# Youncy-Hu/MAGE

Hardware: AMD Instinct MI355X
Metric: generated frames/sec (64x64, 16-frame clips) (higher is better)
Workload: dtype bf16

## Files before the change

include/mage_hip_ext.h:

```cpp
#ifndef MAGE_HIP_EXT_H
#define MAGE_HIP_EXT_H

#include "mage_hip.h"

#ifdef __cplusplus
extern "C" {
#endif

int mage_token_stats(const float* logits, int64_t rows, int32_t K, int64_t ld, int64_t group, int64_t in_group_stride, int64_t in_off,
                     const int64_t* tokens, int64_t tok_group_stride, int64_t tok_off, float temperature, int32_t top_k, float top_p,
                     float* policy_logprob, float* policy_entropy, int32_t* kept, float* entropy, void* stream);

int mage_policy_loss(const float* logits, int64_t rows, int32_t K, int64_t ld, const int64_t* tokens, const float* advantage, int64_t adv_div,
                     const float* behaviour_logprob, float temperature, int32_t top_k, float top_p, float clip_lo, float clip_hi,
                     float entropy_coef, float* row_loss, float* logprob, float* entropy, uint32_t* cut, float* summary, void* stream);
int mage_policy_loss_bwd(const float* logits, int64_t rows, int32_t K, int64_t ld, const int64_t* tokens, const float* advantage,
                         int64_t adv_div, const float* behaviour_logprob, const uint32_t* cut, float temperature, float clip_lo,
                         float clip_hi, float entropy_coef, const float* grad_out, void* dlogits, int32_t dl_dtype, void* stream);

int mage_policy_loss_anchored(const float* logits, int64_t rows, int32_t K, int64_t ld, const int64_t* tokens, const float* advantage,
                              int64_t adv_div, const float* behaviour_logprob, const float* reference_logprob, float temperature,
                              int32_t top_k, float top_p, float clip_lo, float clip_hi, float entropy_coef, float kl_coef, float* row_loss,
                              float* logprob, float* entropy, uint32_t* cut, float* kl, float* summary, void* stream);
int mage_policy_loss_anchored_bwd(const float* logits, int64_t rows, int32_t K, int64_t ld, const int64_t* tokens, const float* advantage,
                                  int64_t adv_div, const float* behaviour_logprob, const float* reference_logprob, const uint32_t* cut,
                                  float temperature, float clip_lo, float clip_hi, float entropy_coef, float kl_coef, const float* grad_out,
                                  void* dlogits, int32_t dl_dtype, void* stream);

int mage_sumsq(const float* g, int64_t n, double* out, void* stream);
int mage_adam_clipped(float* p, const float* g, float* m, float* v, int64_t n, float lr, float beta1, float beta2, float eps, int32_t step,
                      float grad_scale, const double* sumsq, float max_norm, float* norm_out, void* stream);

int mage_video_metrics(const float* video, int64_t video_clip_stride, const float* target, int64_t target_clip_stride, int64_t clips, int32_t T,
                       int32_t C, int32_t H, int32_t W, int64_t tgt_div, float data_range, float* mse, float* psnr, float* ssim, void* stream);

int mage_group_advantages(const float* frame_reward, int64_t groups, int32_t N, int32_t T, int32_t mode, float eps, float* reward,
                          float* advantage, void* stream);

int mage_video_noise(const int64_t* seeds, int64_t B, int32_t C, int64_t hw, float* nchw, float* rows, void* stream);

int mage_guide_logits(const float* cond, const float* uncond, float* out, int64_t rows, int32_t K, int64_t ld, int64_t group,
                      int64_t in_group_stride, int64_t in_off, const float* scale, int64_t scale_div, void* stream);

int mage_preference_loss(const float* clip_logprob, const float* reference_logprob, int64_t clips, const int64_t* pairs, int64_t n_pairs,
                         float beta, float label_smoothing, int32_t mode, float* pair_loss, float* pair_margin, float* clip_coef,
                         float* summary, void* stream);

int mage_token_logprob_bwd(const float* logits, int64_t rows, int32_t K, int64_t ld, const int64_t* tokens, const float* weight,
                           int64_t weight_div, const float* grad_out, void* dlogits, int32_t dl_dtype, void* stream);

#ifdef __cplusplus
}
#endif
#endif
```

mage_amd/_lib.py:

```python
from __future__ import annotations

import ctypes as C
import os
from typing import Optional

_HERE = os.path.dirname(os.path.abspath(__file__))
LIB_PATH = os.environ.get("MAGE_HIP_LIB", os.path.join(_HERE, "lib", "libmage_hip.so"))

F32, BF16, BF16X3, F16X3, F16 = 0, 1, 2, 3, 4
ACT_NONE, ACT_RELU, ACT_QUICKGELU, ACT_GELU_ERF, ACT_TANH, ACT_QUICKGELU_GRAD = 0, 1, 2, 3, 4, 5
ABI_VERSION = 10

i32, i64, f32, vp = C.c_int32, C.c_int64, C.c_float, C.c_void_p


class GemmDesc(C.Structure):
    _fields_ = [
        ("dtype", i32), ("M", i32), ("N", i32), ("K", i32),
        ("A", vp), ("W", vp), ("Y", vp),
        ("lda", i32), ("ldy", i32), ("y_dtype", i32),
        ("out_h", i32), ("out_w", i32), ("in_h", i32), ("in_w", i32),
        ("a_img_stride", i32), ("a_off", i32),
        ("taps_h", i32), ("taps_w", i32), ("cin", i32), ("stride", i32),
        ("dy0", i32), ("dx0", i32), ("dys", i32), ("dxs", i32),
        ("y_img_stride", i32), ("y_mul_y", i32), ("y_mul_x", i32), ("y_off", i32),
        ("bias", vp), ("scale", vp), ("shift", vp),
        ("act", i32),
        ("rowadd", vp), ("rowadd_div", i32), ("rowadd_mod", i32),
        ("residual", vp), ("ldr", i32), ("res_dtype", i32),
        ("post_relu", i32), ("ldw", i32), ("n_split", i32),
        ("a_split_stride", i64), ("w_split_stride", i64), ("y_split_stride", i64),
        ("y2", vp), ("ldy2", i32), ("res_half", i32), ("ln_part", vp), ("ln_stats", vp), ("ln_colsum", vp), ("a_half", i32), ("ln_eps", C.c_float),
        ("head_w", vp), ("head_phases", i32), ("a_relu", i32), ("ln_part_rows", i64),
    ]


class AttnDesc(C.Structure):
    _fields_ = [
        ("dtype", i32), ("q", vp), ("k", vp), ("v", vp), ("out", vp),
        ("ldq", i32), ("ldk", i32), ("ldv", i32), ("ldo", i32),
        ("n_seq", i32), ("inner", i32), ("nq", i32), ("nk", i32), ("n_head", i32),
        ("q_outer_stride", i32), ("q_axis_stride", i32), ("kv_outer_stride", i32), ("kv_axis_stride", i32),
        ("causal", i32), ("kv_len", vp), ("kv_len_div", i32), ("scale", f32), ("out_split", i32), ("drop_p", f32), ("drop_seed", C.c_uint64),
        ("o_outer_stride", i32), ("o_axis_stride", i32),
    ]


SIGNATURES = {
    "mage_abi_version": (C.c_int, []),
    "mage_last_error": (C.c_char_p, []),
    "mage_init": (C.c_int, [C.c_int]),
    "mage_check_device_errors": (C.c_int, [vp]),
    "mage_set_option": (C.c_int, [C.c_char_p, i32]),
    "mage_get_option": (C.c_int, [C.c_char_p, C.POINTER(i32)]),
    "mage_gemm": (C.c_int, [C.POINTER(GemmDesc), vp]),
    "mage_gemm_kernel_name": (C.c_int, [C.POINTER(GemmDesc), C.c_char_p, i32]),
    "mage_gemm_is_small": (C.c_int, [i32, i32, i32]),
    "mage_ln_stats": (C.c_int, [vp, i64, i32, i32, f32, vp, vp]),
    "mage_row_stats": (C.c_int, [vp, i32, i64, i32, i64, f32, vp, vp]),
    "mage_groupnorm_bwd": (C.c_int, [vp, i64, i64, i32, i32, i32, i32, vp, vp, vp, vp, i32, vp, i64, i64, vp, vp, vp, vp, vp, vp]),
    "mage_adain_bwd": (C.c_int, [vp, vp, vp, vp, vp, i32, i32, i32, f32, vp]),
    "mage_reparam_kl_bwd": (C.c_int, [vp, vp, vp, vp, vp, vp, vp, i64, vp]),
    "mage_mse_bwd": (C.c_int, [vp, i64, vp, i64, i64, i32, vp, vp, i64, vp]),
    "mage_transpose_colsum": (C.c_int, [vp, i64, vp, i64, i64, i64, i32, i32, i64, i64, vp, i32, vp]),
    "mage_maxpool2_bwd": (C.c_int, [vp, vp, vp, i32, i32, i32, i32, vp]),
    "mage_upsample2_bwd": (C.c_int, [vp, vp, i32, i32, i32, i32, vp]),
    "mage_layernorm": (C.c_int, [vp, vp, vp, vp, i32, i64, i32, f32, vp]),
    "mage_split": (C.c_int, [vp, i64, vp, i64, i64, i32, i32, vp]),
    "mage_attention": (C.c_int, [C.POINTER(AttnDesc), vp]),
    "mage_embedding": (C.c_int, [vp, vp, vp, i32, i64, i32, i32, i32, i64, i64, i64, i64, i64, vp]),
    "mage_table_conv": (C.c_int, [vp, i64, i32, i32, i32, i32, vp, i32, i32, i32, vp, vp, i32, vp, i64, i32, vp, i32, i64, i64, i64, i64, vp]),
    "mage_resblock_table": (C.c_int, [vp, i64, i32, i32, vp, i32, i32, vp, vp, vp, vp, vp, vp, i32, vp, i64, i64, i64, i64, vp]),
    "mage_resblock_rows": (C.c_int, [vp, i64, vp, vp, vp, vp, vp, i64, i32, vp, i64, i64, i32, i32, i32, i64, i64, i64, vp]),
    "mage_vq_nearest": (C.c_int, [vp, vp, vp, i64, i32, i32, vp, vp, vp]),
    "mage_vq_prepare": (C.c_int, [vp, i32, i32, vp, vp, vp]),
    "mage_argmax": (C.c_int, [vp, i64, i32, i64, i64, i64, i64, vp, i64, i64, vp, vp]),
    "mage_sample_tokens": (C.c_int, [vp, i64, i32, i64, i64, i64, i64, vp, i64, i64, vp, i64, f32, i32, f32, vp]),
    "mage_token_logprob": (C.c_int, [vp, i64, i32, i64, i64, i64, i64, vp, vp, i64, i64, vp]),
    "mage_clip_scores": (C.c_int, [vp, i64, i32, i64, vp, vp, vp]),
    "mage_cross_entropy": (C.c_int, [vp, vp, i64, i32, vp, vp, vp]),
    "mage_conv_in": (C.c_int, [vp, vp, vp, vp, vp, vp, i32, i32, i32, i32, i32, i32, i32, i32, i32, i32, i32, i32, vp]),
    "mage_split_rows": (C.c_int, [vp, i64, vp, i64, i32, i32, i32, i64, i64, i64, i64, i64, vp, vp]),
    "mage_conv_out": (C.c_int, [vp, i32, vp, vp, vp, i32, i32, i32, i32, i32, i32, vp]),
    "mage_convt_fold_tanh": (C.c_int, [vp, vp, vp, i32, i32, i32, i32, vp]),
    "mage_maxpool2": (C.c_int, [vp, vp, i32, i32, i32, i32, i32, i32, vp]),
    "mage_upsample2": (C.c_int, [vp, vp, i32, i32, i32, i32, i32, vp]),
    "mage_relu": (C.c_int, [vp, vp, i32, i64, vp]),
    "mage_cast": (C.c_int, [vp, i32, vp, i32, i64, vp]),
    "mage_adain": (C.c_int, [vp, vp, vp, vp, i32, i32, i32, f32, vp]),
    "mage_add_scaled_rowvec": (C.c_int, [vp, vp, vp, i32, i32, i32, vp]),
    "mage_row_affine": (C.c_int, [vp, vp, vp, i64, i32, i32, i32, vp]),
    "mage_caption_mask": (C.c_int, [vp, i32, i32, i64, vp, vp, vp]),
    "mage_copy2d": (C.c_int, [vp, i64, vp, i64, i64, i64, vp]),
    "mage_groupnorm_silu": (C.c_int, [vp, i64, i64, i32, i32, i32, i32, vp, vp, f32, vp, vp, i32, vp]),
    "mage_groupnorm_act": (C.c_int, [vp, i64, i64, i32, i32, i32, i32, vp, vp, f32, vp, vp, i32, vp, i32, i64, i64, vp]),
    "mage_reparam_kl": (C.c_int, [vp, vp, vp, vp, vp, i32, i64, vp]),
    "mage_mse": (C.c_int, [vp, i64, vp, i64, i64, i32, vp, vp, vp]),
    "mage_transpose": (C.c_int, [vp, i32, i64, vp, i64, i64, i64, i64, i32, i32, i32, i32, i32, i64, i64, i32, i32, i32, vp]),
    "mage_bn_colreduce": (C.c_int, [i32, vp, vp, vp, vp, vp, i64, i32, vp, i32, vp]),
    "mage_bn_apply": (C.c_int, [vp, vp, vp, vp, vp, vp, vp, i32, i64, i32, i32, vp]),
    "mage_bn_bwd_apply": (C.c_int, [vp, vp, vp, vp, vp, vp, vp, vp, i64, i32, vp]),
    "mage_convt_unfold_tanh_bwd": (C.c_int, [vp, vp, vp, i32, i32, i32, i32, vp]),
    "mage_gemm_tn": (C.c_int, [vp, i64, vp, i64, i64, i32, i32, i32, i64, vp, vp, vp]),
    "mage_colsum": (C.c_int, [vp, i64, i64, i32, vp, i32, vp]),
    "mage_row_sum": (C.c_int, [vp, i32, i64, i64, i32, vp, i32, vp]),
    "mage_sum_partials": (C.c_int, [vp, i64, i32, i64, vp, i32, vp]),
    "mage_layernorm_bwd": (C.c_int, [vp, vp, vp, i32, vp, vp, i32, i64, i32, f32, i32, vp, f32, C.c_uint64, vp]),
    "mage_act": (C.c_int, [vp, vp, i32, i64, i32, vp]),
    "mage_act_bwd": (C.c_int, [vp, vp, vp, i32, i64, i32, vp]),
    "mage_cross_entropy_bwd": (C.c_int, [vp, vp, i64, i32, vp, vp, i32, vp]),
    "mage_embedding_bwd": (C.c_int, [vp, vp, i32, vp, i64, i32, i32, i64, i64, i64, i64, vp, i64, vp]),
    "mage_group_rowsum": (C.c_int, [vp, i32, i64, i32, i64, i64, vp, i64, vp, i32, vp]),
    "mage_attention_bwd": (C.c_int, [C.POINTER(AttnDesc), vp, vp, vp, vp, i32, i32, i32, vp]),
    "mage_dropout": (C.c_int, [vp, i32, vp, i32, i64, f32, C.c_uint64, i32, vp]),
    "mage_dropout_add": (C.c_int, [vp, i32, vp, vp, vp, i64, f32, C.c_uint64, vp]),
    "mage_dropout_add_layernorm": (C.c_int, [vp, i32, vp, vp, vp, vp, vp, i32, i64, i32, f32, f32, C.c_uint64, vp]),
    "mage_adam": (C.c_int, [vp, vp, vp, vp, i64, f32, f32, f32, f32, i32, f32, vp]),
}

EXT_SIGNATURES = {
    "mage_token_stats": (C.c_int, [vp, i64, i32, i64, i64, i64, i64, vp, i64, i64, f32, i32, f32, vp, vp, vp, vp, vp]),
    "mage_policy_loss": (C.c_int, [vp, i64, i32, i64, vp, vp, i64, vp, f32, i32, f32, f32, f32, f32, vp, vp, vp, vp, vp, vp]),
    "mage_policy_loss_bwd": (C.c_int, [vp, i64, i32, i64, vp, vp, i64, vp, vp, f32, f32, f32, f32, vp, vp, i32, vp]),
    "mage_policy_loss_anchored": (C.c_int, [vp, i64, i32, i64, vp, vp, i64, vp, vp, f32, i32, f32, f32, f32, f32, f32, vp, vp, vp, vp, vp, vp, vp]),
    "mage_policy_loss_anchored_bwd": (C.c_int, [vp, i64, i32, i64, vp, vp, i64, vp, vp, vp, f32, f32, f32, f32, f32, vp, vp, i32, vp]),
    "mage_sumsq": (C.c_int, [vp, i64, vp, vp]),
    "mage_adam_clipped": (C.c_int, [vp, vp, vp, vp, i64, f32, f32, f32, f32, i32, f32, vp, f32, vp, vp]),
    "mage_video_metrics": (C.c_int, [vp, i64, vp, i64, i64, i32, i32, i32, i32, i64, f32, vp, vp, vp, vp]),
    "mage_group_advantages": (C.c_int, [vp, i64, i32, i32, i32, f32, vp, vp, vp]),
    "mage_video_noise": (C.c_int, [vp, i64, i32, i64, vp, vp, vp]),
    "mage_guide_logits": (C.c_int, [vp, vp, vp, i64, i32, i64, i64, i64, i64, vp, i64, vp]),
    "mage_preference_loss": (C.c_int, [vp, vp, i64, vp, i64, f32, f32, i32, vp, vp, vp, vp, vp]),
    "mage_token_logprob_bwd": (C.c_int, [vp, i64, i32, i64, vp, vp, i64, vp, vp, i32, vp]),
}

_lib: Optional[C.CDLL] = None
_inited_devices = set()


class MageHipError(RuntimeError):
    pass


def load(path: str = LIB_PATH) -> C.CDLL:
    global _lib
    if _lib is not None:
        return _lib
    if not os.path.exists(path):
        raise MageHipError(
            f"{path} not found: the HIP extension is not built. Run `python -c 'import __graft_entry__ as g; g.build()'` "
            f"(or `make -C mage_amd/csrc`). There is no CPU/PyTorch fallback for the MAGE product path.")
    import torch
    lib = C.CDLL(path)
    for name, (res, args) in {**SIGNATURES, **EXT_SIGNATURES}.items():
        fn = getattr(lib, name)
        fn.restype, fn.argtypes = res, args
    if lib.mage_abi_version() != ABI_VERSION:
        raise MageHipError(f"libmage_hip.so ABI {lib.mage_abi_version()} != binding ABI {ABI_VERSION}: rebuild")
    _lib = lib
    return lib


def lib(device_index: int = 0) -> C.CDLL:
    l = load()
    if device_index not in _inited_devices:
        check(l.mage_init(int(device_index)), l)
        _inited_devices.add(device_index)
    return l


def check(code: int, l: Optional[C.CDLL] = None) -> None:
    if code == 0:
        return
    l = l or load()
    msg = (l.mage_last_error() or b"").decode(errors="replace")
    if code == -1:
        raise ValueError(f"mage_hip: {msg}")
    raise MageHipError(f"mage_hip error {code}: {msg}")
```

mage_amd/config.py:

```python
from __future__ import annotations

import contextlib
import dataclasses
import os
from typing import Iterator

__all__ = ["Config", "ENV", "get", "override", "lib_option", "lib_options", "lib_flag", "LIB_OPTIONS"]


@dataclasses.dataclass(frozen=True)
class Config:
    ln_fold: bool = True
    stream_16bit: bool = True
    attn_split: bool = True
    frame_table: bool = True
    auto_graph: bool = True
    encode_split: bool = True
    decode_table: bool = True
    decode_split: bool = True
    decode_taps8: bool = True
    decode_resblock_fusion: bool = True
    decode_head_fusion: bool = True
    decode_phase_merge: bool = True
    decode_relu_fold: bool = True
    train_f32_branch: bool = False
    train_wgrad_transpose: bool = False
    train_emit: bool = True
    train_dual: bool = True
    train_taps: bool = True
    train_enc_split: bool = True


ENV = {
    "ln_fold": ("MAGE_NO_LN_FOLD", False),
    "stream_16bit": ("MAGE_STREAM_FP32", False),
    "attn_split": ("MAGE_ATTN_SPLIT_FP32", False),
    "frame_table": ("MAGE_NO_FRAME_TABLE", False),
    "auto_graph": ("MAGE_NO_AUTO_GRAPH", False),
    "encode_split": ("MAGE_ENCODE_FP32", False),
    "decode_table": ("MAGE_NO_DECODE_TABLE", False),
    "decode_split": ("MAGE_DECODE_FP32", False),
    "decode_taps8": ("MAGE_DECODE_NO_TAPS8", False),
    "decode_resblock_fusion": ("MAGE_DECODE_NO_RESBLOCK_FUSION", False),
    "decode_head_fusion": ("MAGE_DECODE_NO_HEAD_FUSION", False),
    "decode_phase_merge": ("MAGE_DECODE_NO_PHASE_MERGE", False),
    "decode_relu_fold": ("MAGE_DECODE_NO_RELU_FOLD", False),
    "train_f32_branch": ("MAGE_TRAIN_F32_BRANCH", True),
    "train_wgrad_transpose": ("MAGE_WGRAD_TRANSPOSE", True),
    "train_emit": ("MAGE_TRAIN_NO_EMIT", False),
    "train_dual": ("MAGE_TRAIN_NO_DUAL", False),
    "train_taps": ("MAGE_TRAIN_NO_TAPS", False),
    "train_enc_split": ("MAGE_TRAIN_ENC_FP32", False),
}

LIB_OPTIONS = ("gemm_no_4w", "gemm_no_4h", "gemm_4h_plain", "gemm4_train_forms", "gemm_no_8phase", "gemm_no_taps8", "gemm_no_narrow", "gemm_no_narrow_few", "gemm_no_small",
               "gemm_small_m", "gemm_stagger_groups", "gemm_stagger_percent", "gemm_stagger_forced",
               "gemm4_stagger_groups", "gemm4_stagger_percent", "attn_no_mfma", "attn_no_fewq", "vq_no_mfma", "conv_no_tile")


def _set(v) -> bool:
    return bool(v) and v != "0"


def _from_env() -> Config:
    kw = {}
    for field, (var, when_set) in ENV.items():
        if _set(os.environ.get(var)):
            kw[field] = when_set
    return Config(**kw)


_CONFIG = _from_env()


def get() -> Config:
    return _CONFIG


@contextlib.contextmanager
def override(**kw) -> Iterator[Config]:
    global _CONFIG
    saved = _CONFIG
    _CONFIG = dataclasses.replace(saved, **kw)
    try:
        yield _CONFIG
    finally:
        _CONFIG = saved


_LIB_CACHE = None


def invalidate_lib_options() -> None:
    global _LIB_CACHE
    _LIB_CACHE = None


def _lib_cache() -> dict:
    global _LIB_CACHE
    if _LIB_CACHE is None:
        import ctypes as C
        from . import _lib
        l = _lib.load()
        out = {}
        for name in LIB_OPTIONS:
            v = C.c_int32(0)
            _lib.check(l.mage_get_option(name.encode(), C.byref(v)), l)
            out[name] = int(v.value)
        _LIB_CACHE = out
    return _LIB_CACHE


def lib_options() -> dict:
    return dict(_lib_cache())


def lib_flag(name: str) -> int:
    c = _lib_cache()
    if name not in c:
        raise KeyError(f"unknown library option '{name}' (mage_amd.config.LIB_OPTIONS)")
    return c[name]


def set_lib_option(name: str, value: int) -> None:
    from . import _lib
    l = _lib.load()
    try:
        _lib.check(l.mage_set_option(name.encode(), int(value)), l)
    finally:
        invalidate_lib_options()


@contextlib.contextmanager
def lib_option(name: str, value: int) -> Iterator[None]:
    old = lib_flag(name)
    set_lib_option(name, value)
    try:
        yield
    finally:
        set_lib_option(name, old)
```

mage_amd/csrc/common.h:

```cpp
#pragma once
#include <hip/hip_runtime.h>
#include <stdint.h>
#include <stdio.h>
#include <stdarg.h>
#include "../../include/mage_hip.h"

typedef __bf16 bf16_t;
typedef __attribute__((ext_vector_type(8))) __bf16 bf16x8;
typedef __attribute__((ext_vector_type(4))) __bf16 bf16x4;
typedef __attribute__((ext_vector_type(4))) float f32x4;
typedef __attribute__((ext_vector_type(4))) unsigned int u32x4;

#define MAGE_MAX_DEVICES 16
void mage_set_error(const char* fmt, ...);
int mage_device_index();
const void* mage_zero_page();
int* mage_error_word();
enum { MAGE_DEVERR_EMBEDDING_ID = 1, MAGE_DEVERR_CE_TARGET = 2, MAGE_DEVERR_TOKEN_ID = 3, MAGE_DEVERR_PAIR_ID = 4 };
struct MageOptions {
    int gemm_no_4w;
    int gemm_no_4h;
    int gemm_4h_plain;
    int gemm4_train_forms;
    int gemm_no_8phase;
    int gemm_no_taps8;
    int gemm_no_narrow;
    int gemm_no_narrow_few;
    int gemm_no_small;
    int gemm_small_m;
    int gemm_stagger_groups, gemm_stagger_percent, gemm_stagger_forced;
    int gemm4_stagger_groups, gemm4_stagger_percent;
    int attn_no_mfma;
    int attn_no_fewq;
    int vq_no_mfma;
    int conv_no_tile;
};
const MageOptions& mage_options();
__device__ __forceinline__ void mage_raise(int* word, int code, long value, int bound) {
    if (atomicCAS(word, 0, code) == 0) {
        word[1] = (int)value;
        word[2] = bound;
    }
}

#if defined(MAGE_DEBUG) && MAGE_DEBUG
#include <cassert>
#define MAGE_DASSERT(cond) assert(cond)
#else
#define MAGE_DASSERT(cond) ((void)0)
#endif

#define MAGE_CHECK_ARG(cond, ...)                                   \
    do {                                                            \
        if (!(cond)) {                                              \
            mage_set_error(__VA_ARGS__);                            \
            return MAGE_EINVAL;                                     \
        }                                                           \
    } while (0)

#define MAGE_CHECK_LAUNCH(name)                                                         \
    do {                                                                                \
        hipError_t e_ = hipGetLastError();                                              \
        if (e_ != hipSuccess) {                                                         \
            mage_set_error("%s: launch failed: %s", name, hipGetErrorString(e_));       \
            return MAGE_EHIP;                                                           \
        }                                                                               \
    } while (0)

int mage_gemm_cu_count();
extern thread_local const void** mage_gemm_plan;
template <auto KERNEL, typename Args>
int mage_gemm_launch(unsigned grid, unsigned block, unsigned lds, hipStream_t s, const Args& a) {
    if (mage_gemm_plan) {
        *mage_gemm_plan = (const void*)KERNEL;
        return MAGE_OK;
    }
    static bool attr[MAGE_MAX_DEVICES] = {false};
    const int dev = mage_device_index();
    MAGE_CHECK_ARG(dev >= 0, "mage_gemm: no current device");
    if (!attr[dev]) {
        (void)hipFuncSetAttribute((const void*)KERNEL, hipFuncAttributeMaxDynamicSharedMemorySize, lds);
        attr[dev] = true;
    }
    hipLaunchKernelGGL(KERNEL, dim3(grid), dim3(block), lds, s, a);
    MAGE_CHECK_LAUNCH("mage_gemm");
    return MAGE_OK;
}

__device__ __forceinline__ unsigned short f2bf_bits(float f) {
    unsigned int u = __float_as_uint(f);
    if ((u & 0x7fffffffu) > 0x7f800000u) return (unsigned short)((u >> 16) | 0x40);
    u += 0x7fffu + ((u >> 16) & 1u);
    return (unsigned short)(u >> 16);
}
__device__ __forceinline__ float bf_bits2f(unsigned short b) { return __uint_as_float(((unsigned int)b) << 16); }

template <typename T> __device__ __forceinline__ float to_f32(T v);
template <> __device__ __forceinline__ float to_f32<float>(float v) { return v; }
template <> __device__ __forceinline__ float to_f32<unsigned short>(unsigned short v) { return bf_bits2f(v); }

template <typename T> __device__ __forceinline__ T from_f32(float v);
template <> __device__ __forceinline__ float from_f32<float>(float v) { return v; }
template <> __device__ __forceinline__ unsigned short from_f32<unsigned short>(float v) { return f2bf_bits(v); }

typedef _Float16 f16_t;
template <> __device__ __forceinline__ float to_f32<f16_t>(f16_t v) { return (float)v; }
template <> __device__ __forceinline__ f16_t from_f32<f16_t>(float v) { return (f16_t)v; }

__device__ __forceinline__ f32x4 load4(const float* p) { return *(const f32x4*)p; }
__device__ __forceinline__ f32x4 load4(const unsigned short* p) {
    uint2 r = *(const uint2*)p;
    f32x4 o;
    o[0] = __uint_as_float(r.x << 16);
    o[1] = __uint_as_float(r.x & 0xffff0000u);
    o[2] = __uint_as_float(r.y << 16);
    o[3] = __uint_as_float(r.y & 0xffff0000u);
    return o;
}
__device__ __forceinline__ void store4(float* p, f32x4 v) { *(f32x4*)p = v; }
__device__ __forceinline__ void mage_ln_stats_row(const float2* __restrict__ p, long stride, int n_slices, float inv_c, float eps, float& mean, float& rstd) {
    float s1 = 0.f, s2 = 0.f;
    for (int i = 0; i < n_slices; ++i) {
        const float2 v = p[(long)i * stride];
        s1 = __fadd_rn(s1, v.x);
        s2 = __fadd_rn(s2, v.y);
    }
    mean = __fmul_rn(s1, inv_c);
    const float var = fmaxf(__fmaf_rn(-mean, mean, __fmul_rn(s2, inv_c)), 0.f);
    rstd = __fdiv_rn(1.0f, __fsqrt_rn(__fadd_rn(var, eps)));
}

typedef __attribute__((ext_vector_type(2))) __bf16 bf16x2_t;
__device__ __forceinline__ unsigned int pack_bf16x2(float a, float b) {
    bf16x2_t v = {(__bf16)a, (__bf16)b};
    return __builtin_bit_cast(unsigned int, v);
}
__device__ __forceinline__ void store4(unsigned short* p, f32x4 v) {
    uint2 r;
    r.x = pack_bf16x2(v[0], v[1]);
    r.y = pack_bf16x2(v[2], v[3]);
    *(uint2*)p = r;
}

__device__ __forceinline__ void store8(unsigned short* p, f32x4 a, f32x4 b) {
    uint4 r;
    r.x = pack_bf16x2(a[0], a[1]);
    r.y = pack_bf16x2(a[2], a[3]);
    r.z = pack_bf16x2(b[0], b[1]);
    r.w = pack_bf16x2(b[2], b[3]);
    *(uint4*)p = r;
}
__device__ __forceinline__ void store8(float* p, f32x4 a, f32x4 b) { *(f32x4*)p = a; *(f32x4*)(p + 4) = b; }

typedef __attribute__((ext_vector_type(2))) _Float16 f16x2_t;
typedef __attribute__((ext_vector_type(8))) _Float16 f16x8;
__device__ __forceinline__ unsigned int pack_f16x2(float a, float b) {
    const f16x2_t v = {(_Float16)a, (_Float16)b};
    return __builtin_bit_cast(unsigned int, v);
}
__device__ __forceinline__ float2 unpack_f16x2(unsigned int u) {
    const f16x2_t v = __builtin_bit_cast(f16x2_t, u);
    return float2{(float)v[0], (float)v[1]};
}
__device__ __forceinline__ float2 unpack_bf16x2(unsigned int u) { return float2{__uint_as_float(u << 16), __uint_as_float(u & 0xffff0000u)}; }
template <typename T> __device__ __forceinline__ unsigned int pack16x2(float a, float b) {
    if constexpr (sizeof(T) == 2 && !__is_same(T, unsigned short)) return pack_f16x2(a, b);
    else return pack_bf16x2(a, b);
}
template <typename T> __device__ __forceinline__ float2 unpack16x2(unsigned int u) {
    if constexpr (sizeof(T) == 2 && !__is_same(T, unsigned short)) return unpack_f16x2(u);
    else return unpack_bf16x2(u);
}
template <typename T> __device__ __forceinline__ f32x4 widen4(uint2 r) {
    const float2 a = unpack16x2<T>(r.x), b = unpack16x2<T>(r.y);
    return f32x4{a.x, a.y, b.x, b.y};
}
template <typename T> __device__ __forceinline__ f32x4 mfma16x16x32(const u32x4& a, const u32x4& b, const f32x4& c) {
    if constexpr (sizeof(T) == 2 && !__is_same(T, unsigned short))
        return __builtin_amdgcn_mfma_f32_16x16x32_f16(__builtin_bit_cast(f16x8, a), __builtin_bit_cast(f16x8, b), c, 0, 0, 0);
    else
        return __builtin_amdgcn_mfma_f32_16x16x32_bf16(__builtin_bit_cast(bf16x8, a), __builtin_bit_cast(bf16x8, b), c, 0, 0, 0);
}
__device__ __forceinline__ f32x4 load4(const f16_t* p) { return widen4<f16_t>(*(const uint2*)p); }
__device__ __forceinline__ void store4(f16_t* p, f32x4 v) { *(uint2*)p = uint2{pack_f16x2(v[0], v[1]), pack_f16x2(v[2], v[3])}; }
__device__ __forceinline__ void store8(f16_t* p, f32x4 a, f32x4 b) {
    *(uint4*)p = uint4{pack_f16x2(a[0], a[1]), pack_f16x2(a[2], a[3]), pack_f16x2(b[0], b[1]), pack_f16x2(b[2], b[3])};
}

typedef short mage_s16x2 __attribute__((ext_vector_type(2)));
__device__ __forceinline__ unsigned relu16x2(unsigned v) {
    const mage_s16x2 z = {0, 0};
    return __builtin_bit_cast(unsigned, __builtin_elementwise_max(__builtin_bit_cast(mage_s16x2, v), z));
}

struct split_bf16 { unsigned int pair; };
struct split_f16 { unsigned int pair; };
#define MAGE_F16_LO_SCALE 2048.0f
template <int KIND>
__device__ __forceinline__ void split_pack2(float a, float b, unsigned int& hi, unsigned int& lo) {
    if constexpr (KIND == 1) {
        hi = pack_bf16x2(a, b);
        lo = pack_bf16x2(a - __uint_as_float(hi << 16), b - __uint_as_float(hi & 0xffff0000u));
    } else {
        a = __builtin_amdgcn_fmed3f(a, -65504.f, 65504.f);
        b = __builtin_amdgcn_fmed3f(b, -65504.f, 65504.f);
        const f16x2_t h = {(_Float16)a, (_Float16)b};
        const f16x2_t l = {(_Float16)((a - (float)h[0]) * MAGE_F16_LO_SCALE), (_Float16)((b - (float)h[1]) * MAGE_F16_LO_SCALE)};
        hi = __builtin_bit_cast(unsigned int, h);
        lo = __builtin_bit_cast(unsigned int, l);
    }
}
template <int KIND>
__device__ __forceinline__ void split_store4(void* p, f32x4 v) {
    const uintptr_t a = (uintptr_t)p;
    char* q = (char*)((a & ~(uintptr_t)255) + ((a & 255) >> 1));
    uint2 h, l;
    split_pack2<KIND>(v[0], v[1], h.x, l.x);
    split_pack2<KIND>(v[2], v[3], h.y, l.y);
    *(uint2*)q = h;
    *(uint2*)(q + 128) = l;
}
__device__ __forceinline__ void store4(split_bf16* p, f32x4 v) { split_store4<1>(p, v); }
__device__ __forceinline__ void store4(split_f16* p, f32x4 v) { split_store4<2>(p, v); }
// ... 35 lines not shown
```

mage_amd/csrc/gemm.hip:

```cpp
#include <cxxabi.h>
#include <cstring>
#include <mutex>
#include <string>
#include <unordered_map>
#include "gemm_impl.h"

int mage_gemm_f16(const mage_gemm_desc* d, hipStream_t s);

#ifdef MAGE_PROBE
extern "C" int mage_debug_read_waves(void* dst, size_t bytes) {
    return hipMemcpyFromSymbol(dst, HIP_SYMBOL(mage_probe_wave), bytes < sizeof(mage_probe_wave) ? bytes : sizeof(mage_probe_wave)) ==
                   hipSuccess
               ? 0
               : -1;
}
extern "C" int mage_debug_read_seg(void* dst, size_t bytes) {
    return hipMemcpyFromSymbol(dst, HIP_SYMBOL(mage_probe_seg), bytes < sizeof(mage_probe_seg) ? bytes : sizeof(mage_probe_seg)) ==
                   hipSuccess
               ? 0
               : -1;
}
extern "C" int mage_debug_read(void* dst, size_t bytes) {
    return hipMemcpyFromSymbol(dst, HIP_SYMBOL(mage_probe_buf), bytes < sizeof(mage_probe_buf) ? bytes : sizeof(mage_probe_buf)) ==
                   hipSuccess
               ? 0
               : -1;
}
#endif


extern "C" int mage_gemm_is_small(int32_t M, int32_t N, int32_t K) {
    MAGE_CHECK_ARG(mage_device_index() >= 0 && M > 0 && N > 0 && K > 0, "mage_gemm_is_small: no current device / bad sizes");
    return small_shape(M, N, K, mage_gemm_cu_count()) ? 1 : 0;
}

extern "C" int mage_gemm(const mage_gemm_desc* d_in, void* stream) {
    MAGE_CHECK_ARG(d_in != nullptr, "mage_gemm: null descriptor");
    mage_gemm_desc dn = *d_in;
    const bool spl = dn.dtype == MAGE_BF16X3 || dn.dtype == MAGE_F16X3;
    if (dn.ldw == 0) dn.ldw = spl ? 2 * dn.K : dn.K;
    if (dn.n_split <= 0) dn.n_split = 1;
    const mage_gemm_desc* d = &dn;
    MAGE_CHECK_ARG(d->ldw >= (spl ? 2 * d->K : d->K), "mage_gemm: ldw=%d < K=%d", d->ldw, d->K);
    MAGE_CHECK_ARG(d->ldw == d->K || d->n_split > 1 || spl,
                   "mage_gemm: ldw=%d != K=%d: a W row stride other than K is read only by the split-K (n_split > 1) and split-precision forms", d->ldw, d->K);
    MAGE_CHECK_ARG(mage_zero_page() != nullptr, "mage_gemm: mage_init() has not been called");
    const bool h16 = d->dtype == MAGE_F16;
    MAGE_CHECK_ARG(d->dtype == MAGE_F32 || d->dtype == MAGE_BF16 || h16 || spl, "mage_gemm: bad dtype %d", d->dtype);
    MAGE_CHECK_ARG(d->y_dtype == MAGE_F32 || (d->y_dtype == MAGE_BF16 && !h16) || ((spl || h16) && d->y_dtype == d->dtype),
                   "mage_gemm: bad y_dtype %d for dtype %d (fp32, or the operands' 16-bit / split type; fp32 operands may write bf16)", d->y_dtype, d->dtype);
    MAGE_CHECK_ARG(!d->residual || d->res_dtype == MAGE_F32 || (d->res_dtype == MAGE_BF16 && !h16) || (h16 && d->res_dtype == MAGE_F16),
                   "mage_gemm: bad res_dtype %d for dtype %d", d->res_dtype, d->dtype);
    MAGE_CHECK_ARG(!spl || (d->K % 64 == 0 && d->cin % 64 == 0 && d->lda >= 2 * d->cin && d->y_dtype != MAGE_BF16),
                   "mage_gemm: split-precision operands need K and cin multiples of 64, lda >= 2 cin (16-bit elements), fp32 or split output");
    MAGE_CHECK_ARG(!spl || d->y_dtype == MAGE_F32 || (d->N % 64 == 0 && d->ldy % 8 == 0 && d->ldy >= 2 * d->N && (((uintptr_t)d->Y) & 255) == 0),
                   "mage_gemm: split output needs N %% 64 == 0, ldy >= 2N (16-bit elements), Y 256-byte aligned");
    MAGE_CHECK_ARG(d->M > 0 && d->N > 0 && d->K > 0, "mage_gemm: empty problem M=%d N=%d K=%d", d->M, d->N, d->K);
    MAGE_CHECK_ARG(d->A && d->W && d->Y, "mage_gemm: null operand");
    const int ch = d->dtype == MAGE_F32 ? 4 : 8;
    MAGE_CHECK_ARG(d->N % 8 == 0, "mage_gemm: N=%d must be a multiple of 8", d->N);
    MAGE_CHECK_ARG(d->K % ch == 0 && d->lda % ch == 0 && d->cin % ch == 0,
                   "mage_gemm: K=%d, lda=%d, cin=%d must be multiples of %d", d->K, d->lda, d->cin, ch);
    MAGE_CHECK_ARG(d->ldy % 4 == 0 && (!d->residual || d->ldr % 4 == 0), "mage_gemm: ldy/ldr must be multiples of 4");
    MAGE_CHECK_ARG((d->y_dtype != MAGE_BF16 && d->y_dtype != MAGE_F16) || d->ldy % 8 == 0, "mage_gemm: 16-bit output needs ldy a multiple of 8 (16-byte accesses)");
    MAGE_CHECK_ARG(!d->residual || d->res_dtype == MAGE_F32 || d->ldr % 8 == 0, "mage_gemm: a 16-bit residual needs ldr a multiple of 8 (16-byte accesses)");
    MAGE_CHECK_ARG(d->taps_h >= 1 && d->taps_w >= 1 && d->K == d->taps_h * d->taps_w * d->cin,
                   "mage_gemm: K=%d != taps_h*taps_w*cin = %d*%d*%d", d->K, d->taps_h, d->taps_w, d->cin);
    MAGE_CHECK_ARG(d->out_h >= 1 && d->out_w >= 1 && d->in_h >= 1 && d->in_w >= 1, "mage_gemm: bad geometry");
    MAGE_CHECK_ARG(!d->scale == !d->shift, "mage_gemm: scale and shift must be given together");
    MAGE_CHECK_ARG(!d->rowadd || (d->rowadd_div >= 1 && d->rowadd_mod >= 1), "mage_gemm: bad rowadd div/mod");
    MAGE_CHECK_ARG((((uintptr_t)d->A | (uintptr_t)d->W | (uintptr_t)d->Y) & 15) == 0, "mage_gemm: operands must be 16-byte aligned");
    const bool gather_ = d->taps_h * d->taps_w > 1 || d->stride != 1 || d->dy0 != 0 || d->dx0 != 0 || d->in_h != d->out_h || d->in_w != d->out_w;
    MAGE_CHECK_ARG(d->n_split == 1 || (!gather_ && !d->residual && !d->rowadd && !d->scale && !d->post_relu && !d->bias &&
                                       d->out_h == 1 && d->out_w >= d->M && d->act == MAGE_ACT_NONE),
                   "mage_gemm: n_split > 1 is the plain split-K form (no gather, no epilogue extras, rows not regrouped)");
    MAGE_CHECK_ARG(d->n_split == 1 || ((d->a_split_stride | d->w_split_stride) % ch == 0 && d->y_split_stride % 4 == 0 && d->ldw % ch == 0),
                   "mage_gemm: split strides / ldw must keep 16-byte alignment");
    hipStream_t s = (hipStream_t)stream;
    MAGE_CHECK_ARG(!d->a_half || (d->in_h % 2 == 0 && d->in_w % 2 == 0 && d->n_split == 1), "mage_gemm: a_half needs an even in_h x in_w grid");
    MAGE_CHECK_ARG(!d->res_half || (d->residual && d->out_h > 1 && d->out_h % 2 == 0 && d->out_w % 2 == 0 && d->n_split == 1),
                   "mage_gemm: res_half needs a residual and an even out_h x out_w output plane");
    MAGE_CHECK_ARG(!d->ln_part || d->ln_part_rows > (d->ln_colsum ? (int64_t)d->M - 1 : (int64_t)(d->M - 1) * d->y_mul_x + d->y_off),
                   "mage_gemm: ln_part needs ln_part_rows (rows of the slice-major partial-sum buffer) > the largest row it is indexed with");
    MAGE_CHECK_ARG(!d->a_relu || (d->dtype == MAGE_BF16 && !gather_ && !d->a_half && d->N <= 128 && d->n_split == 1 && !d->residual && !d->rowadd && !d->scale &&
                                  !d->post_relu && !d->y2 && !d->ln_part && !d->ln_stats && !d->ln_colsum && !d->head_w),
                   "mage_gemm: a_relu is a form of the bf16 plain GEMM with N <= 128 (epilogue act(acc + bias) only)");
    if (spl) {
        const bool tapsform = gather_ || d->rowadd;
        MAGE_CHECK_ARG(!d->head_w, "mage_gemm: head_w is a fusion of the bf16 padded-taps form");
        if (tapsform) {
            const int r = d->dtype == MAGE_BF16X3 ? try_taps8<1>(d, s) : try_taps8<2>(d, s);
            if (r) return r < 0 ? r : MAGE_OK;
            mage_set_error("mage_gemm: split-precision form: this convolution / row-table geometry is not eligible for the padded-taps kernel");
            return MAGE_EUNSUPPORTED;
        }
        return d->dtype == MAGE_BF16X3 ? launch_spl<1>(d, s) : launch_spl<2>(d, s);
    }
    if (h16) {
        MAGE_CHECK_ARG(!d->head_w && d->n_split == 1 && !d->scale && !d->post_relu && !d->res_half && !d->a_half,
                       "mage_gemm: MAGE_F16 operands do not take head_w / n_split / scale+shift / post_relu / res_half / a_half");
        return mage_gemm_f16(d, s);
    }
    if (const int r = try_taps8(d, s)) return r < 0 ? r : MAGE_OK;
    MAGE_CHECK_ARG(!d->head_w, "mage_gemm: head_w is a fusion of the bf16 padded-taps form; this geometry does not run there");
    if (const int r = mage_conv3x3_c64_try(d, s)) return r < 0 ? r : MAGE_OK;
    if (const int r = mage_gemm4_try(d, s)) return r < 0 ? r : MAGE_OK;
    const bool gather = d->taps_h * d->taps_w > 1 || d->stride != 1 || d->dy0 != 0 || d->dx0 != 0 || d->in_h != d->out_h ||
                        d->in_w != d->out_w || d->a_half;
    if (d->dtype == MAGE_BF16) return gather ? launch<MAGE_BF16, true>(d, s) : launch<MAGE_BF16, false>(d, s);
    return gather ? launch<MAGE_F32, true>(d, s) : launch<MAGE_F32, false>(d, s);
}

thread_local const void** mage_gemm_plan = nullptr;

extern "C" int mage_gemm_kernel_name(const mage_gemm_desc* desc, char* buf, int32_t len) {
    MAGE_CHECK_ARG(buf != nullptr && len > 0, "mage_gemm_kernel_name: no buffer");
    const void* kernel = nullptr;
    mage_gemm_plan = &kernel;
    const int r = mage_gemm(desc, nullptr);
    mage_gemm_plan = nullptr;
    if (r != MAGE_OK) return r;
    static std::mutex mu;
    static std::unordered_map<const void*, std::string> names;
    std::string name;
    {
        std::lock_guard<std::mutex> lock(mu);
        auto it = names.find(kernel);
        if (it == names.end()) {
            hipFunction_t f = nullptr;
            const char* raw = hipGetFuncBySymbol(&f, kernel) == hipSuccess ? hipKernelNameRef(f) : nullptr;
            if (!raw) {
                mage_set_error("mage_gemm_kernel_name: the runtime has no name for the selected kernel");
                return MAGE_EHIP;
            }
            std::string n = raw;
            int status = -1;
            if (char* dm = n.compare(0, 2, "_Z") == 0 ? abi::__cxa_demangle(raw, nullptr, nullptr, &status) : nullptr) {
                if (status == 0) n = dm;
                free(dm);
            }
            for (const char* drop : {"void ", "(anonymous namespace)::"})
                for (size_t at; (at = n.find(drop)) != std::string::npos;) n.erase(at, strlen(drop));
            n = n.substr(0, n.find('('));
            it = names.emplace(kernel, n).first;
        }
        name = it->second;
    }
    MAGE_CHECK_ARG((int32_t)name.size() < len, "mage_gemm_kernel_name: %d bytes are too few for '%s'", (int)len, name.c_str());
    memcpy(buf, name.c_str(), name.size() + 1);
    return MAGE_OK;
}
```

mage_amd/csrc/gemm4.hip:

```cpp
#include <cstdio>
#include <cstdlib>
#include <utility>

#include "gemm_shared.h"
#include "gemm4_regs.h"

namespace {

struct Gemm4Args {
    const void* A;
    const void* W;
    void* Y;
    const float* bias;
    const float* ln_stats;
    const float* ln_colsum;
    const void* residual;
    float* ln_part;
    void* y2;
    int M, N, K, lda, ldw, ldy, ldr, ldy2, y_dtype, a_off, y_off;
    int ntiles_n, ntiles;
    int stagger_groups, stagger_sleeps;
};

#ifndef MAGE4_ABL
#define MAGE4_ABL 0
#endif

#ifdef MAGE4_STAMP
__device__ unsigned long long g4_stamps[256 * 32 * 4 * 8];
#define G4_STAMP(it, p)                                                                                                   \
    do {                                                                                                                  \
        if (lane == 0 && (it) < 32 && blockIdx.x < 256) {                                                                 \
            g4_stamps[((blockIdx.x * 32 + (it)) * 4 + wave) * 8 + (p)] = __builtin_readcyclecounter();                    \
            if ((p) == 1) g4_stamps[((blockIdx.x * 32 + (it)) * 4 + wave) * 8 + 3] = __builtin_amdgcn_s_memrealtime();    \
            if ((p) == 0) g4_stamps[((blockIdx.x * 32 + (it)) * 4 + wave) * 8 + 4] = __builtin_amdgcn_s_memrealtime();    \
        }                                                                                                                 \
    } while (0)
#else
#define G4_STAMP(it, p)
#endif

constexpr int G4_STAGE = 65536, G4_WOFF = 32768, G4_RING = 2 * G4_STAGE, G4_LDS = G4_RING + 4 * 4096;

#ifdef MAGE4_MFMA32
template <int B, bool ZERO, bool CLOB>
__device__ __forceinline__ void g4_mfma32(const u32x4& w, const u32x4& x) {
    if constexpr (ZERO && CLOB) asm volatile("v_mfma_f32_32x32x16_bf16 a[%c2:%c3], %0, %1, 0" ::"v"(w), "v"(x), "i"(16 * B), "i"(16 * B + 15) : G4_ALL_ACC);
    else if constexpr (ZERO) asm volatile("v_mfma_f32_32x32x16_bf16 a[%c2:%c3], %0, %1, 0" ::"v"(w), "v"(x), "i"(16 * B), "i"(16 * B + 15));
    else if constexpr (CLOB) asm volatile("v_mfma_f32_32x32x16_bf16 a[%c2:%c3], %0, %1, a[%c2:%c3]" ::"v"(w), "v"(x), "i"(16 * B), "i"(16 * B + 15) : G4_ALL_ACC);
    else asm volatile("v_mfma_f32_32x32x16_bf16 a[%c2:%c3], %0, %1, a[%c2:%c3]" ::"v"(w), "v"(x), "i"(16 * B), "i"(16 * B + 15));
}
#endif
template <int ACT, int EK, int LN, bool RB, bool HF = false>
__global__ __launch_bounds__(256) void gemm4_kernel(const Gemm4Args g) {
    static_assert(EK != EK_GENERAL, "lean epilogue kinds");
    static_assert(!HF || (LN != LN_DUAL && LN != LN_GELUBWD), "f16 form: the generation path's epilogues");
    typedef std::conditional_t<HF, f16_t, unsigned short> H16;
    extern __shared__ __attribute__((aligned(16))) char smem[];
    g4_claim_accumulators();
    const int tid = threadIdx.x;
    const int lane = tid & 63;
    const int wave = __builtin_amdgcn_readfirstlane(tid >> 6);
    const int nwg8 = gridDim.x >> 3;
    const int xcd = blockIdx.x & 7, li = blockIdx.x >> 3;
    const int q8 = g.ntiles >> 3, r8 = g.ntiles & 7;
    const int chunk0 = xcd < r8 ? xcd * (q8 + 1) : r8 * (q8 + 1) + (xcd - r8) * q8;
    const int chunk1 = chunk0 + q8 + (xcd < r8 ? 1 : 0);
    const int nk = g.K >> 6;
    int c_tile = chunk0 + li;
    if (c_tile >= chunk1) return;
    const int last_tile = c_tile + ((chunk1 - 1 - c_tile) / nwg8) * nwg8;

    const int lr = lane >> 3, lp = lane & 7;
    unsigned voffA[8], voffW[8];
#pragma unroll
    for (int u = 0; u < 8; ++u) {
        const int r = u * 8 + lr;
        const int ch = lp ^ ((r >> 1) & 7);
        voffA[u] = (unsigned)(r * g.lda * 2 + ch * 16 + 8192 - u * 1024);
        voffW[u] = (unsigned)(r * g.ldw * 2 + ch * 16 + 8192 - u * 1024);
    }
    auto a_base = [&](int tile) { return (const char*)g.A + ((long)((tile / g.ntiles_n) * 256 + wave * 64) + g.a_off) * g.lda * 2 - 4096; };
    auto w_base = [&](int tile) { return (const char*)g.W + (long)((tile % g.ntiles_n) * 256 + wave * 64) * g.ldw * 2 - 4096; };
    const char* a_src = a_base(c_tile);
    const char* w_src = w_base(c_tile);
    const char* a_next = a_src;
    const char* w_next = w_src;
    const unsigned lds0 = (unsigned)(uintptr_t)(__attribute__((address_space(3))) char*)smem + wave * 8192 + 4096;
    auto dma_m0 = [&](unsigned lds_group) __attribute__((always_inline)) {
        asm volatile("s_mov_b32 m0, %0\n\ts_nop 0" ::"s"(lds0 + lds_group) : "memory");
    };

    const int wm = wave >> 1, wn = wave & 1;
    const int l15 = lane & 15, grp = lane >> 4;
    const int rsw = (l15 >> 1) & 7;
    const int pc[2] = {((grp + 0) ^ rsw) * 16, ((grp + 4) ^ rsw) * 16};
    const int x_off = (wm * 128 + l15) * 128;
    const int w_off = G4_WOFF + (wn * 128 + l15) * 128;
    u32x4 wf[2][8], xf[2][4];
    auto rd_w1 = [&](int buf, int stage, int t, int nt) __attribute__((always_inline)) {
        wf[buf][nt] = *(const u32x4*)(smem + stage * G4_STAGE + w_off + nt * 2048 + pc[t]);
    };
    auto rd_x1 = [&](int buf, int stage, int t, int mt) __attribute__((always_inline)) {
        xf[buf][mt & 3] = *(const u32x4*)(smem + stage * G4_STAGE + x_off + mt * 2048 + pc[t]);
    };

#ifdef MAGE4_MFMA32
    const int l31 = lane & 31, hi5 = lane >> 5;
    const int rsw32 = (l31 >> 1) & 7;
    const int x32_off = (wm * 128 + l31) * 128, w32_off = G4_WOFF + (wn * 128 + l31) * 128;
    u32x4 wq[2][4], xq[2][4];
    auto rd_w32 = [&](int buf, int stage, int ks, int nb) __attribute__((always_inline)) {
        wq[buf][nb] = *(const u32x4*)(smem + stage * G4_STAGE + w32_off + nb * 4096 + (((2 * ks + hi5) ^ rsw32) << 4));
    };
    auto rd_x32 = [&](int buf, int stage, int ks, int mb) __attribute__((always_inline)) {
        xq[buf][mb] = *(const u32x4*)(smem + stage * G4_STAGE + x32_off + mb * 4096 + (((2 * ks + hi5) ^ rsw32) << 4));
    };
#endif
    if (g.stagger_groups > 1) {
        for (int w = (li % g.stagger_groups) * g.stagger_sleeps; w > 0; --w) __builtin_amdgcn_s_sleep(16);
    }
    dma_m0(0);
    g4_for<8>([&](auto u_) { g4_dma<decltype(u_)::value>(voffA[decltype(u_)::value], a_src); });
    dma_m0(G4_WOFF);
    g4_for<8>([&](auto u_) { g4_dma<decltype(u_)::value>(voffW[decltype(u_)::value], w_src); });
    a_src += 128;
    w_src += 128;
    dma_m0(G4_STAGE);
    g4_for<8>([&](auto u_) { g4_dma<decltype(u_)::value>(voffA[decltype(u_)::value], a_src); });
    dma_m0(G4_STAGE + G4_WOFF);
    g4_for<8>([&](auto u_) { g4_dma<decltype(u_)::value>(voffW[decltype(u_)::value], w_src); });
    a_src += 128;
    w_src += 128;
    __builtin_amdgcn_s_waitcnt(0x0F70);
    ring_barrier();
#ifdef MAGE4_MFMA32
#pragma unroll
    for (int b = 0; b < 4; ++b) { rd_w32(0, 0, 0, b); rd_x32(0, 0, 0, b); }
#else
#pragma unroll
    for (int nt = 0; nt < 8; ++nt) rd_w1(0, 0, 0, nt);
#pragma unroll
    for (int m = 0; m < 4; ++m) rd_x1(0, 0, 0, m);
#endif

    [[maybe_unused]] int it = 0;
    for (; c_tile < chunk1; c_tile += nwg8, ++it) {
        G4_STAMP(it, 0);
        const int tm = c_tile / g.ntiles_n, tn = c_tile - tm * g.ntiles_n;
        MAGE_DASSERT(c_tile >= 0 && c_tile < g.ntiles && tm * 256 < g.M && tn * 256 < g.N);
        const int m0 = ((MAGE4_ABL & 32) ? (int)blockIdx.x : tm) * 256 + wm * 128, n0 = ((MAGE4_ABL & 32) ? 0 : tn) * 256 + wn * 128;
        {
            const int nt_tile = c_tile + nwg8 > last_tile ? last_tile : c_tile + nwg8;
            a_next = a_base(nt_tile);
            w_next = w_base(nt_tile);
        }
        f32x4 biasm[2][4];
        [[maybe_unused]] float ln_mean[8], ln_rstd[8];
        [[maybe_unused]] f32x4 lns[2][4];
        auto slab = [&](auto S_, auto FIRST_, auto LAST_, int j) __attribute__((always_inline)) {
            constexpr int S = decltype(S_)::value;
            constexpr bool FIRST = decltype(FIRST_)::value, LAST = decltype(LAST_)::value;
            g4_for<32>([&](auto i_) {
                constexpr int i = decltype(i_)::value, m = i >> 3, nt = i & 7;
                g4_mfma<((nt >> 2) * 8 + m) * 4 + (nt & 3), FIRST, i == 0, HF>(wf[0][nt], xf[0][m]);
                __builtin_amdgcn_sched_barrier(0);
                if constexpr (!(MAGE4_ABL & 4) && i < 4) {
                    rd_x1(1, S, 0, 4 + i);
                    __builtin_amdgcn_sched_barrier(0);
                }
                if constexpr (!(MAGE4_ABL & 2) && !FIRST && i == 4) {
                    dma_m0((S ^ 1) * G4_STAGE + G4_WOFF);
                    __builtin_amdgcn_sched_barrier(0);
                }
                if constexpr (!(MAGE4_ABL & 2) && !FIRST && (i & 3) == 1 && i > 4) {
                    g4_dma<(i >> 2) - 1>(voffW[(i >> 2) - 1], w_src);
                    __builtin_amdgcn_sched_barrier(0);
                }
            });
            if constexpr (!(MAGE4_ABL & 2) && !FIRST) {
                g4_dma<7>(voffW[7], w_src);
                __builtin_amdgcn_sched_barrier(0);
            }
            if constexpr (!(MAGE4_ABL & 8) && !FIRST) w_src = (j == nk - 2) ? w_next : w_src + 128;
            g4_for<32>([&](auto i_) {
                constexpr int i = decltype(i_)::value, m = i >> 3, nt = i & 7;
                g4_mfma<((nt >> 2) * 8 + 4 + m) * 4 + (nt & 3), FIRST, i == 0, HF>(wf[0][nt], xf[1][m]);
                __builtin_amdgcn_sched_barrier(0);
                if constexpr (!(MAGE4_ABL & 4) && i < 12) {
                    if constexpr (i < 4) rd_x1(0, S, 1, i);
                    else rd_w1(1, S, 1, i - 4);
                    __builtin_amdgcn_sched_barrier(0);
                }
            });
            if constexpr (LAST) {
#pragma unroll
                for (int b = 0; b < 4; ++b) {
                    const int n = n0 + b * 16 + grp * 4;
                    biasm[0][b] = *(const f32x4*)(g.bias + n);
                    if constexpr (LN == LN_CONSUME) lns[0][b] = *(const f32x4*)(g.ln_colsum + n);
                }
                if constexpr (LN == LN_CONSUME) {
#pragma unroll
                    for (int a = 0; a < 8; ++a) {
                        const float2 st = *(const float2*)(g.ln_stats + 2 * (long)(m0 + a * 16 + l15));
                        ln_mean[a] = st.x;
                        ln_rstd[a] = st.y;
                    }
                }
                __builtin_amdgcn_sched_barrier(0);
            }
            g4_for<32>([&](auto i_) {
                constexpr int i = decltype(i_)::value, m = i >> 3, nt = i & 7;
                g4_mfma<((nt >> 2) * 8 + m) * 4 + (nt & 3), false, i == 0, HF>(wf[1][nt], xf[0][m]);
                __builtin_amdgcn_sched_barrier(0);
                if constexpr (!(MAGE4_ABL & 4) && i < 4) {
                    rd_x1(1, S, 1, 4 + i);
                    __builtin_amdgcn_sched_barrier(0);
                }
            });
            if constexpr (MAGE4_ABL & 16) __builtin_amdgcn_s_waitcnt(0xC07F);
            else if constexpr (FIRST) __builtin_amdgcn_s_waitcnt(LN == LN_CONSUME ? 0x8074 : 0x8070);
            else __builtin_amdgcn_s_waitcnt(0x0070);
            ring_barrier();
            __builtin_amdgcn_sched_barrier(0);
            g4_for<32>([&](auto i_) {
                constexpr int i = decltype(i_)::value, m = i >> 3, nt = i & 7;
                g4_mfma<((nt >> 2) * 8 + 4 + m) * 4 + (nt & 3), false, i == 0, HF>(wf[1][nt], xf[1][m]);
                __builtin_amdgcn_sched_barrier(0);
                if constexpr (!(MAGE4_ABL & 4) && i < 12 && !LAST) {
                    if constexpr (i < 4) rd_x1(0, S ^ 1, 0, i);
                    else rd_w1(0, S ^ 1, 0, i - 4);
                    __builtin_amdgcn_sched_barrier(0);
                }
                if constexpr (!(MAGE4_ABL & 2) && !LAST) {
                    if constexpr (i == 2) dma_m0(S * G4_STAGE);
                    if constexpr ((i & 3) == 3) g4_dma<(i >> 2)>(voffA[i >> 2], a_src);
                    if constexpr (i == 2 || (i & 3) == 3) __builtin_amdgcn_sched_barrier(0);
                }
                if constexpr (!(MAGE4_ABL & 2) && LAST) {
                    if constexpr (i == 0) dma_m0(S * G4_STAGE);
                    if constexpr (i == 16) dma_m0(S * G4_STAGE + G4_WOFF);
                    if constexpr ((i & 1) == 1 && i < 16) g4_dma<(i >> 1)>(voffA[i >> 1], a_src);
                    if constexpr ((i & 1) == 1 && i > 16) g4_dma<((i - 16) >> 1)>(voffW[(i - 16) >> 1], w_src);
                    if constexpr (i == 0 || i == 16 || (i & 1) == 1) __builtin_amdgcn_sched_barrier(0);
                }
            });
            if constexpr (!(MAGE4_ABL & 8)) a_src = (j == nk - 3) ? a_next : a_src + 128;
            if constexpr (!(MAGE4_ABL & 8) && LAST) w_src += 128;
        };
#ifdef MAGE4_MFMA32
        auto slab32 = [&](auto S_, auto FIRST_, auto LAST_, int j) __attribute__((always_inline)) {
            constexpr int S = decltype(S_)::value;
            constexpr bool FIRST = decltype(FIRST_)::value, LAST = decltype(LAST_)::value;
            auto quarter = [&](auto Q_) __attribute__((always_inline)) {
                constexpr int Q = decltype(Q_)::value, buf = Q & 1;
                g4_for<16>([&](auto i_) {
                    constexpr int i = decltype(i_)::value, mb = i >> 2, nb = i & 3;
                    g4_mfma32<mb * 4 + nb, FIRST && Q == 0, i == 0>(wq[buf][nb], xq[buf][mb]);
                    __builtin_amdgcn_sched_barrier(0);
                    if constexpr (!(MAGE4_ABL & 4) && i < 8 && !(Q == 3 && LAST)) {
                        constexpr int st = Q == 3 ? (S ^ 1) : S, ks = (Q + 1) & 3;
                        if constexpr (i < 4) rd_x32(buf ^ 1, st, ks, i);
                        else rd_w32(buf ^ 1, st, ks, i - 4);
                        __builtin_amdgcn_sched_barrier(0);
                    }
                    if constexpr (Q == 0 && !(MAGE4_ABL & 2) && !FIRST) {
                        if constexpr (i == 4) dma_m0((S ^ 1) * G4_STAGE + G4_WOFF);
                        if constexpr (i >= 5 && i < 13) g4_dma<i - 5>(voffW[i - 5], w_src);
                        if constexpr (i >= 4 && i < 13) __builtin_amdgcn_sched_barrier(0);
                    }
                    if constexpr (Q == 3 && !(MAGE4_ABL & 2) && !LAST) {
                        if constexpr (i == 1) dma_m0(S * G4_STAGE);
                        if constexpr (i >= 2 && i < 10) g4_dma<i - 2>(voffA[i - 2], a_src);
                        if constexpr (i >= 1 && i < 10) __builtin_amdgcn_sched_barrier(0);
                    }
                });
            };
            quarter(std::integral_constant<int, 0>{});
            if constexpr (!(MAGE4_ABL & 8) && !FIRST) w_src = (j == nk - 2) ? w_next : w_src + 128;
            quarter(std::integral_constant<int, 1>{});
            quarter(std::integral_constant<int, 2>{});
            if constexpr (FIRST) __builtin_amdgcn_s_waitcnt(0x8070);
            else __builtin_amdgcn_s_waitcnt(0x0070);
            ring_barrier();
            __builtin_amdgcn_sched_barrier(0);
            quarter(std::integral_constant<int, 3>{});
            if constexpr (LAST && !(MAGE4_ABL & 2)) {
                dma_m0(S * G4_STAGE);
                g4_for<8>([&](auto u_) { g4_dma<decltype(u_)::value>(voffA[decltype(u_)::value], a_src); });
                dma_m0(S * G4_STAGE + G4_WOFF);
                g4_for<8>([&](auto u_) { g4_dma<decltype(u_)::value>(voffW[decltype(u_)::value], w_src); });
            }
            if constexpr (!(MAGE4_ABL & 8)) a_src = (j == nk - 3) ? a_next : a_src + 128;
            if constexpr (!(MAGE4_ABL & 8) && LAST) w_src += 128;
        };
#define slab slab32
#endif
        typedef std::integral_constant<int, 0> S0;
        typedef std::integral_constant<int, 1> S1;
        slab(S0{}, std::true_type{}, std::false_type{}, 0);
        slab(S1{}, std::false_type{}, std::false_type{}, 1);
        for (int j = 2; j < nk - 2; j += 2) {
            slab(S0{}, std::false_type{}, std::false_type{}, j);
            slab(S1{}, std::false_type{}, std::false_type{}, j + 1);
        }
        slab(S0{}, std::false_type{}, std::false_type{}, nk - 2);
        slab(S1{}, std::false_type{}, std::true_type{}, nk - 1);
#ifdef MAGE4_MFMA32
#undef slab
#endif
        asm volatile("s_nop 15\n\ts_nop 7" ::: "memory");
        G4_STAMP(it, 1);
#if MAGE4_ABL & 1
        {
            f32x4 t = g4_acc_read<0>() + g4_acc_read<17>() + g4_acc_read<63>();
            if (t[0] + t[1] + t[2] + t[3] == 123456.789f) ((float*)g.Y)[0] = t[0] + biasm[0][0][0];
        }
#else
        char* win = smem + G4_RING + wave * 4096;
#pragma unroll
        for (int b = 0; b < 4; ++b) {
            const int n = n0 + 64 + b * 16 + grp * 4;
            biasm[1][b] = *(const f32x4*)(g.bias + n);
            if constexpr (LN == LN_CONSUME) lns[1][b] = *(const f32x4*)(g.ln_colsum + n);
        }
        mage_gemm_desc e = {};
        e.M = 0x7fffffff;
        e.N = LN == LN_PRODUCE ? g.N : 0x7fffffff;
        e.K = g.K;
        e.Y = g.Y;
        e.ldy = g.ldy;
        e.y_dtype = g.y_dtype;
        e.out_h = 1;
        e.out_w = 0x7fffffff;
        e.y_mul_x = 1;
        e.y_off = g.y_off;
        e.y2 = g.y2;
        e.ldy2 = g.ldy2;
        e.ln_part = g.ln_part;
        g4_for<4>([&](auto c_) {
            constexpr int c = decltype(c_)::value, h = c >> 1, mh = c & 1;
            __builtin_amdgcn_sched_barrier(0);
            f32x4 t[4][4];
            g4_for<16>([&](auto q_) {
                constexpr int q = decltype(q_)::value;
                t[q >> 2][q & 3] = g4_acc_read<(h * 8 + mh * 4 + (q >> 2)) * 4 + (q & 3), q == 0>();
            });
            [[maybe_unused]] LnConsume lnc;
            if constexpr (LN == LN_CONSUME) {
#pragma unroll
                for (int a = 0; a < 4; ++a) {
                    lnc.mean[a] = ln_mean[mh * 4 + a];
                    lnc.rstd[a] = ln_rstd[mh * 4 + a];
                }
#pragma unroll
                for (int b = 0; b < 4; ++b) lnc.s[b] = lns[h][b];
                if (g.y_dtype == MAGE_F32) epilogue_lean<ACT, float, 4, false, LN>(e, biasm[h], t, m0 + mh * 64, n0 + h * 64, lane, 1, win, 0, &lnc);
                else epilogue_lean<ACT, H16, 4, false, LN>(e, biasm[h], t, m0 + mh * 64, n0 + h * 64, lane, 1, win, 0, &lnc);
            } else if constexpr (LN == LN_DUAL || LN == LN_GELUBWD) {
                epilogue_lean<ACT, unsigned short, 4, false, LN>(e, biasm[h], t, m0 + mh * 64, n0 + h * 64, lane, 1, win, 0);
            } else {
                if (g.y_dtype == MAGE_F32) epilogue_lean<ACT, float, 4, false, LN>(e, biasm[h], t, m0 + mh * 64, n0 + h * 64, lane, 1, win, 0);
                else epilogue_lean<ACT, H16, 4, false, LN>(e, biasm[h], t, m0 + mh * 64, n0 + h * 64, lane, 1, win, 0);
            }
        });
#endif
        G4_STAMP(it, 2);
        __builtin_amdgcn_sched_barrier(0);
        if (c_tile + nwg8 < chunk1) {
#ifdef MAGE4_MFMA32
#pragma unroll
            for (int b = 0; b < 4; ++b) { rd_w32(0, 0, 0, b); rd_x32(0, 0, 0, b); }
#else
#pragma unroll
            for (int nt = 0; nt < 8; ++nt) rd_w1(0, 0, 0, nt);
#pragma unroll
            for (int m = 0; m < 4; ++m) rd_x1(0, 0, 0, m);
#endif
        }
    }
}

template <int ACT, int EK, int LN, bool RB, bool HF = false>
int launch4(const mage_gemm_desc* d, hipStream_t s, int n_cu) {
    Gemm4Args a;
    a.A = d->A;
    a.W = d->W;
    a.Y = d->Y;
    a.bias = d->bias ? d->bias : (const float*)mage_zero_page();
    a.ln_stats = d->ln_stats;
    a.ln_colsum = d->ln_colsum;
    a.residual = d->residual;
    a.ln_part = d->ln_part;
    a.y2 = d->y2;
    a.M = d->M;
    a.N = d->N;
    a.K = d->K;
    a.lda = d->lda;
    a.ldw = d->ldw ? d->ldw : d->K;
    a.ldy = d->ldy;
    a.ldr = d->ldr;
    a.ldy2 = d->ldy2;
    a.y_dtype = d->y_dtype;
    a.a_off = d->a_off;
    a.y_off = d->y_off;
    a.ntiles_n = d->N / 256;
    a.ntiles = (d->M / 256) * a.ntiles_n;
    const int st_groups = mage_options().gemm4_stagger_groups, st_percent = mage_options().gemm4_stagger_percent;
    a.stagger_groups = 0;
    a.stagger_sleeps = 0;
    const int grid = a.ntiles >= n_cu ? n_cu : ((a.ntiles + 7) & ~7);
    if (st_groups > 1 && a.ntiles / grid >= 6) {
        const long period = (long)(d->K / 64) * 3100 + 9000;
        a.stagger_groups = st_groups;
        a.stagger_sleeps = (int)(period * st_percent / 100 / st_groups / 1024);
    }
    const int r = mage_gemm_launch<gemm4_kernel<ACT, EK, LN, RB, HF>>(grid, 256, G4_LDS, s, a);
    return r < 0 ? r : 1;
}

}

namespace {

struct Tn4Args {
    const unsigned short* A;
    const unsigned short* B;
    float* P;
    float* DB;
    long lda, ldb, T, tps;
    int N, K, n_split, ntk;
};
typedef short g4_tr4 __attribute__((ext_vector_type(4)));
__device__ __forceinline__ g4_tr4 g4_lds_tr(const char* p) { return __builtin_amdgcn_ds_read_tr16_b64_v4i16((__attribute__((address_space(3))) g4_tr4*)p); }

template <bool DB>
__global__ __launch_bounds__(256) void gemm_tn4_kernel(const Tn4Args g) {
    constexpr int PART = 32768, STAGE = 2 * PART;
    extern __shared__ __attribute__((aligned(16))) char smem[];
    g4_claim_accumulators();
    const int lane = threadIdx.x & 63;
    const int wave = __builtin_amdgcn_readfirstlane(threadIdx.x >> 6);
    const int tile = blockIdx.x / g.n_split, s = blockIdx.x - tile * g.n_split;
    const int tm = tile / g.ntk, tk = tile - tm * g.ntk;
    const long t_begin = (long)s * g.tps;
    const long t_end = t_begin + g.tps < g.T ? t_begin + g.tps : g.T;
    const int nslab = (int)((t_end - t_begin) >> 6);
    const int rr = lane >> 3, pc = lane & 7;
    unsigned voffA[8], voffB[8];
#pragma unroll
    for (int u = 0; u < 8; ++u) {
        const int col_in_strip = (((pc >> 1) ^ (rr & 3) ^ (u & 1)) << 4) + ((pc & 1) << 3);
        voffA[u] = (unsigned)(((long)(u * 8 + rr) * g.lda + wave * 64 + col_in_strip) * 2 + 8192 - u * 1024);
        voffB[u] = (unsigned)(((long)(u * 8 + rr) * g.ldb + wave * 64 + col_in_strip) * 2 + 8192 - u * 1024);
    }
    const char* a_src = (const char*)(g.A + t_begin * g.lda + (long)tm * 256) - 4096;
    const char* b_src = (const char*)(g.B + t_begin * g.ldb + (long)tk * 256) - 4096;
    const long da = 64 * g.lda * 2, db_ = 64 * g.ldb * 2;
    int a_slab = 0, b_slab = 0;
    const unsigned lds0 = (unsigned)(uintptr_t)(__attribute__((address_space(3))) char*)smem + wave * 8192 + 4096;
    auto dma_m0 = [&](unsigned lds_group) __attribute__((always_inline)) {
        asm volatile("s_mov_b32 m0, %0\n\ts_nop 0" ::"s"(lds0 + lds_group) : "memory");
    };
    auto a_advance = [&]() __attribute__((always_inline)) {
        const bool more = a_slab + 1 < nslab;
        a_src = more ? a_src + da : a_src;
        a_slab = more ? a_slab + 1 : a_slab;
    };
    auto b_advance = [&]() __attribute__((always_inline)) {
        const bool more = b_slab + 1 < nslab;
        b_src = more ? b_src + db_ : b_src;
        b_slab = more ? b_slab + 1 : b_slab;
    };
    const int wm = wave >> 1, wn = wave & 1;
    const int i15 = lane & 15, grp = lane >> 4;
    const int lane_off = grp * 1024 + (i15 >> 2) * 128 + (i15 & 3) * 8;
    const int sw = (i15 >> 2) ^ (grp & 1);
    g4_tr4 bfh[2][8][2], afh[2][4][2];
    auto rd_b = [&](int buf, int stage, int t, int nt, int h) __attribute__((always_inline)) {
        bfh[buf][nt][h] = g4_lds_tr(smem + stage * STAGE + PART + ((wn * 2 + (nt >> 2)) * 8 + t * 4) * 1024 + lane_off + (((nt & 3) ^ sw) << 5) + h * 512);
    };
    auto rd_a = [&](int buf, int stage, int t, int mt, int h) __attribute__((always_inline)) {
        afh[buf][mt & 3][h] = g4_lds_tr(smem + stage * STAGE + ((wm * 2 + (mt >> 2)) * 8 + t * 4) * 1024 + lane_off + (((mt & 3) ^ sw) << 5) + h * 512);
    };
    auto frag = [](const g4_tr4 (&h)[2]) __attribute__((always_inline)) {
        return __builtin_bit_cast(u32x4, __builtin_shufflevector(h[0], h[1], 0, 1, 2, 3, 4, 5, 6, 7));
    };
    typedef __attribute__((ext_vector_type(2))) __bf16 bf16x2v;
    const bf16x2v ones2 = {(__bf16)1.0f, (__bf16)1.0f};
    [[maybe_unused]] float dbs[8] = {0.f, 0.f, 0.f, 0.f, 0.f, 0.f, 0.f, 0.f};
    [[maybe_unused]] auto db_acc = [&](int mt, const g4_tr4 (&h)[2]) __attribute__((always_inline)) {
        const uint2 w0 = __builtin_bit_cast(uint2, h[0]), w1 = __builtin_bit_cast(uint2, h[1]);
        float d = dbs[mt];
        d = __builtin_amdgcn_fdot2_f32_bf16(__builtin_bit_cast(bf16x2v, w0.x), ones2, d, false);
        d = __builtin_amdgcn_fdot2_f32_bf16(__builtin_bit_cast(bf16x2v, w0.y), ones2, d, false);
        d = __builtin_amdgcn_fdot2_f32_bf16(__builtin_bit_cast(bf16x2v, w1.x), ones2, d, false);
        d = __builtin_amdgcn_fdot2_f32_bf16(__builtin_bit_cast(bf16x2v, w1.y), ones2, d, false);
        dbs[mt] = d;
    };

    dma_m0(0);
    g4_for<8>([&](auto u_) { g4_dma<decltype(u_)::value>(voffA[decltype(u_)::value], a_src); });
    dma_m0(PART);
    g4_for<8>([&](auto u_) { g4_dma<decltype(u_)::value>(voffB[decltype(u_)::value], b_src); });
    a_advance();
    b_advance();
    dma_m0(STAGE);
    g4_for<8>([&](auto u_) { g4_dma<decltype(u_)::value>(voffA[decltype(u_)::value], a_src); });
    dma_m0(STAGE + PART);
    g4_for<8>([&](auto u_) { g4_dma<decltype(u_)::value>(voffB[decltype(u_)::value], b_src); });
    a_advance();
    b_advance();
    __builtin_amdgcn_s_waitcnt(0x0F70);
    ring_barrier();
#pragma unroll
    for (int nt = 0; nt < 8; ++nt) { rd_b(0, 0, 0, nt, 0); rd_b(0, 0, 0, nt, 1); }
#pragma unroll
    for (int m = 0; m < 4; ++m) { rd_a(0, 0, 0, m, 0); rd_a(0, 0, 0, m, 1); }

    auto slab = [&](auto S_, auto FIRST_) __attribute__((always_inline)) {
        constexpr int S = decltype(S_)::value;
        constexpr bool FIRST = decltype(FIRST_)::value;
        g4_for<32>([&](auto i_) {
            constexpr int i = decltype(i_)::value, m = i >> 3, nt = i & 7;
            g4_mfma<m * 8 + nt, FIRST, i == 0>(frag(bfh[0][nt]), frag(afh[0][m]));
            __builtin_amdgcn_sched_barrier(0);
            if constexpr (i < 8) {
                rd_a(1, S, 0, 4 + (i >> 1), i & 1);
                __builtin_amdgcn_sched_barrier(0);
            }
            if constexpr (DB && nt == 7) {
                db_acc(m, afh[0][m]);
                __builtin_amdgcn_sched_barrier(0);
            }
            if constexpr (!FIRST && i == 8) {
                dma_m0((S ^ 1) * STAGE + PART);
                __builtin_amdgcn_sched_barrier(0);
            }
            if constexpr (!FIRST && i > 8 && (i & 1) == 1 && i < 25) {
                g4_dma<((i - 9) >> 1)>(voffB[(i - 9) >> 1], b_src);
                __builtin_amdgcn_sched_barrier(0);
            }
        });
        if constexpr (!FIRST) b_advance();
        g4_for<32>([&](auto i_) {
            constexpr int i = decltype(i_)::value, m = i >> 3, nt = i & 7;
            g4_mfma<(4 + m) * 8 + nt, FIRST, i == 0>(frag(bfh[0][nt]), frag(afh[1][m]));
            __builtin_amdgcn_sched_barrier(0);
            if constexpr (i < 24) {
                if constexpr (i < 8) rd_a(0, S, 1, i >> 1, i & 1);
                else rd_b(1, S, 1, (i - 8) >> 1, i & 1);
                __builtin_amdgcn_sched_barrier(0);
            }
            if constexpr (DB && nt == 7) {
                db_acc(4 + m, afh[1][m]);
                __builtin_amdgcn_sched_barrier(0);
            }
        });
        g4_for<32>([&](auto i_) {
            constexpr int i = decltype(i_)::value, m = i >> 3, nt = i & 7;
            g4_mfma<m * 8 + nt, false, i == 0>(frag(bfh[1][nt]), frag(afh[0][m]));
            __builtin_amdgcn_sched_barrier(0);
            if constexpr (i < 8) {
                rd_a(1, S, 1, 4 + (i >> 1), i & 1);
                __builtin_amdgcn_sched_barrier(0);
            }
            if constexpr (DB && nt == 7) {
                db_acc(m, afh[0][m]);
                __builtin_amdgcn_sched_barrier(0);
            }
        });
        __builtin_amdgcn_s_waitcnt(0x0070);
        ring_barrier();
        __builtin_amdgcn_sched_barrier(0);
        g4_for<32>([&](auto i_) {
            constexpr int i = decltype(i_)::value, m = i >> 3, nt = i & 7;
            g4_mfma<(4 + m) * 8 + nt, false, i == 0>(frag(bfh[1][nt]), frag(afh[1][m]));
            __builtin_amdgcn_sched_barrier(0);
            if constexpr (i < 24) {
                if constexpr (i < 8) rd_a(0, S ^ 1, 0, i >> 1, i & 1);
                else rd_b(0, S ^ 1, 0, (i - 8) >> 1, i & 1);
                __builtin_amdgcn_sched_barrier(0);
            }
            if constexpr (DB && nt == 7) {
                db_acc(4 + m, afh[1][m]);
                __builtin_amdgcn_sched_barrier(0);
            }
            if constexpr (i == 24) {
                dma_m0(S * STAGE);
                __builtin_amdgcn_sched_barrier(0);
            }
        });
        g4_for<8>([&](auto u_) { g4_dma<decltype(u_)::value>(voffA[decltype(u_)::value], a_src); });
        __builtin_amdgcn_sched_barrier(0);
        a_advance();
    };
    typedef std::integral_constant<int, 0> S0;
    typedef std::integral_constant<int, 1> S1;
    slab(S0{}, std::true_type{});
    int j = 1;
    for (; j + 1 < nslab; j += 2) {
        slab(S1{}, std::false_type{});
        slab(S0{}, std::false_type{});
    }
    if (j < nslab) slab(S1{}, std::false_type{});
    asm volatile("s_nop 15\n\ts_nop 7" ::: "memory");
    float* out = g.P + ((long)s * g.N + (long)tm * 256 + wm * 128) * g.K + (long)tk * 256 + wn * 128;
    g4_for<64>([&](auto q_) {
        constexpr int q = decltype(q_)::value, mt = q >> 3, nt = q & 7;
        *(f32x4*)(out + (long)(mt * 16 + i15) * g.K + nt * 16 + grp * 4) = g4_acc_read<q, (q & 15) == 0>();
    });
    if constexpr (DB) {
#pragma unroll
        for (int mt = 0; mt < 8; ++mt) {
            float v = dbs[mt];
            v += __shfl_xor(v, 16);
            v += __shfl_xor(v, 32);
            if (grp == 0) g.DB[(long)s * g.N + (long)tm * 256 + wm * 128 + mt * 16 + i15] = v;
        }
    }
}

}

int mage_gemm4h_try(const mage_gemm_desc* d, hipStream_t s, int n_cu);

int mage_gemm4_try(const mage_gemm_desc* d, hipStream_t s) {
    const bool hf = d->dtype == MAGE_F16;
    if ((d->dtype != MAGE_BF16 && !hf) || d->n_split > 1) return 0;
    if (mage_options().gemm_no_4w) return 0;
    if (d->M % 256 || d->N % 256 || d->K % 128 || d->K < 256 || d->K > 1024) return 0;
    if (d->taps_h * d->taps_w != 1 || d->stride != 1 || d->dy0 || d->dx0 || d->in_h != d->out_h || d->in_w != d->out_w || d->a_half) return 0;
    if (d->out_h != 1 || d->out_w < d->M || d->y_mul_x != 1) return 0;
    if (d->scale || d->rowadd || d->post_relu || d->res_half) return 0;
    if (d->residual || d->ln_part || d->rowadd) return 0;
    if (!d->bias && (d->N > 4096 || d->ln_stats || mage_zero_page() == nullptr)) return 0;
    if ((d->ln_colsum != nullptr) != (d->ln_stats != nullptr)) return 0;
    const bool dual = d->y2 && d->act == MAGE_ACT_QUICKGELU && !d->ln_stats;
    const bool gbwd = d->y2 && d->act == MAGE_ACT_QUICKGELU_GRAD && !d->ln_stats;
    if (d->y2 && !dual && !gbwd) return 0;
    if ((dual || gbwd) && !mage_options().gemm4_train_forms) return 0;
    if ((dual || gbwd) && (d->y_dtype != MAGE_BF16 || d->ldy2 % 8 || (((uintptr_t)d->y2) & 15))) return 0;
    if (!dual && !gbwd && d->act != MAGE_ACT_NONE && d->act != MAGE_ACT_QUICKGELU) return 0;
    if (d->y_dtype != MAGE_F32 && d->y_dtype != d->dtype) return 0;
    if (hf && (dual || gbwd)) return 0;
    if (d->ldy % 8 || d->lda % 8 || (((uintptr_t)d->bias | (uintptr_t)d->ln_colsum) & 15) || (((uintptr_t)d->ln_stats) & 7)) return 0;
    const int n_cu = mage_gemm_cu_count();
    const long ntiles = (long)(d->M / 256) * (d->N / 256);
    const bool few_tiles = ntiles < 4L * n_cu;
    const int ldw = d->ldw ? d->ldw : d->K;
    if (((long)d->M + d->a_off) * d->lda * 2 + 16384 >= (1L << 32) || (long)d->N * ldw * 2 + 16384 >= (1L << 32)) return 0;
    if (!dual && !gbwd)
        if (const int r = mage_gemm4h_try(d, s, n_cu)) return r;
    if (few_tiles) return 0;
    if (dual) return launch4<MAGE_ACT_QUICKGELU, EK_BIAS, LN_DUAL, false>(d, s, n_cu);
    if (gbwd) return launch4<MAGE_ACT_NONE, EK_BIAS, LN_GELUBWD, false>(d, s, n_cu);
    if (hf) {
        if (d->ln_stats) {
            if (d->act == MAGE_ACT_NONE) return launch4<MAGE_ACT_NONE, EK_BIAS, LN_CONSUME, false, true>(d, s, n_cu);
            return launch4<MAGE_ACT_QUICKGELU, EK_BIAS, LN_CONSUME, false, true>(d, s, n_cu);
        }
        if (d->act == MAGE_ACT_NONE) return launch4<MAGE_ACT_NONE, EK_BIAS, LN_NONE, false, true>(d, s, n_cu);
        return launch4<MAGE_ACT_QUICKGELU, EK_BIAS, LN_NONE, false, true>(d, s, n_cu);
    }
    if (d->ln_stats) {
        if (d->act == MAGE_ACT_NONE) return launch4<MAGE_ACT_NONE, EK_BIAS, LN_CONSUME, false>(d, s, n_cu);
        return launch4<MAGE_ACT_QUICKGELU, EK_BIAS, LN_CONSUME, false>(d, s, n_cu);
    }
    if (d->act == MAGE_ACT_NONE) return launch4<MAGE_ACT_NONE, EK_BIAS, LN_NONE, false>(d, s, n_cu);
    return launch4<MAGE_ACT_QUICKGELU, EK_BIAS, LN_NONE, false>(d, s, n_cu);
}

int mage_gemm_tn4_try(const void* dY, int64_t lda, const void* X, int64_t ldb, int64_t T, int32_t N, int32_t K, int32_t n_split, int64_t tps,
                      float* partials, float* db_partials, hipStream_t stream) {
    if (mage_options().gemm_no_4w) return 0;
    if (T % 64 || tps % 64 || tps < 128 || (T - (int64_t)(n_split - 1) * tps) < 128) return 0;
    if (lda * 2 * 64 + 16384 >= (1L << 31) || ldb * 2 * 64 + 16384 >= (1L << 31)) return 0;
    const int dev = mage_device_index();
    if (dev < 0) return 0;
    static bool attr[MAGE_MAX_DEVICES] = {false};
    if (!attr[dev]) {
        (void)hipFuncSetAttribute((const void*)gemm_tn4_kernel<false>, hipFuncAttributeMaxDynamicSharedMemorySize, 128 * 1024);
        (void)hipFuncSetAttribute((const void*)gemm_tn4_kernel<true>, hipFuncAttributeMaxDynamicSharedMemorySize, 128 * 1024);
        attr[dev] = true;
    }
    Tn4Args a;
    a.A = (const unsigned short*)dY;
    a.B = (const unsigned short*)X;
    a.P = partials;
    a.DB = db_partials;
    a.lda = lda;
    a.ldb = ldb;
    a.T = T;
    a.tps = tps;
    a.N = N;
    a.K = K;
    a.n_split = n_split;
    a.ntk = K / 256;
    const long grid = (long)(N / 256) * (K / 256) * n_split;
    if (db_partials) hipLaunchKernelGGL(gemm_tn4_kernel<true>, dim3((unsigned)grid), dim3(256), 128 * 1024, stream, a);
    else hipLaunchKernelGGL(gemm_tn4_kernel<false>, dim3((unsigned)grid), dim3(256), 128 * 1024, stream, a);
    MAGE_CHECK_LAUNCH("mage_gemm_tn");
    return 1;
}
```

mage_amd/csrc/norm_attn.hip:

```cpp
#include <cstdlib>
#include <type_traits>

#include "common.h"

namespace {

template <typename OT, int VPL>
__global__ __launch_bounds__(256) void layernorm_kernel(const float* __restrict__ x, const float* __restrict__ gamma,
                                                        const float* __restrict__ beta, OT* __restrict__ y, long rows,
                                                        int C, float eps) {
    const int lane = threadIdx.x & 63;
    const long row = (long)blockIdx.x * 4 + (threadIdx.x >> 6);
    if (row >= rows) return;
    const float* xr = x + row * C;
    f32x4 v[VPL];
    float s = 0.f;
#pragma unroll
    for (int j = 0; j < VPL; ++j) {
        const int c = j * 256 + lane * 4;
        v[j] = (c < C) ? *(const f32x4*)(xr + c) : f32x4{0.f, 0.f, 0.f, 0.f};
        s += (v[j][0] + v[j][1]) + (v[j][2] + v[j][3]);
    }
    const float mean = wave_sum(s) / (float)C;
    float q = 0.f;
#pragma unroll
    for (int j = 0; j < VPL; ++j) {
        const int c = j * 256 + lane * 4;
        if (c < C) {
#pragma unroll
            for (int e = 0; e < 4; ++e) {
                const float dlt = v[j][e] - mean;
                q += dlt * dlt;
            }
        }
    }
    const float rstd = 1.0f / sqrtf(wave_sum(q) / (float)C + eps);
    OT* yr = y + row * C;
#pragma unroll
    for (int j = 0; j < VPL; ++j) {
        const int c = j * 256 + lane * 4;
        if (c < C) {
            const f32x4 gm = *(const f32x4*)(gamma + c), bt = *(const f32x4*)(beta + c);
            f32x4 o;
#pragma unroll
            for (int e = 0; e < 4; ++e) o[e] = (v[j][e] - mean) * rstd * gm[e] + bt[e];
            store4(yr + c, o);
        }
    }
}

__device__ __forceinline__ void load8f(const float* p, f32x4& a, f32x4& b) {
    a = *(const f32x4*)p;
    b = *(const f32x4*)(p + 4);
}
__device__ __forceinline__ void load8f(const unsigned short* p, f32x4& a, f32x4& b) {
    const uint4 r = *(const uint4*)p;
    a = f32x4{__uint_as_float(r.x << 16), __uint_as_float(r.x & 0xffff0000u), __uint_as_float(r.y << 16), __uint_as_float(r.y & 0xffff0000u)};
    b = f32x4{__uint_as_float(r.z << 16), __uint_as_float(r.z & 0xffff0000u), __uint_as_float(r.w << 16), __uint_as_float(r.w & 0xffff0000u)};
}
__device__ __forceinline__ void copy8(const float* src, float* dst) {
    *(f32x4*)dst = *(const f32x4*)src;
    *(f32x4*)(dst + 4) = *(const f32x4*)(src + 4);
}
__device__ __forceinline__ void copy8(const unsigned short* src, unsigned short* dst) { *(uint4*)dst = *(const uint4*)src; }
__device__ __forceinline__ void load8f(const f16_t* p, f32x4& a, f32x4& b) {
    const uint4 r = *(const uint4*)p;
    a = widen4<f16_t>(uint2{r.x, r.y});
    b = widen4<f16_t>(uint2{r.z, r.w});
}
__device__ __forceinline__ void copy8(const f16_t* src, f16_t* dst) { *(uint4*)dst = *(const uint4*)src; }

template <typename T, int NK_MAX, typename OT = T>
__global__ __launch_bounds__(256) void attention_kernel(const mage_attn_desc d, int hg) {
    extern __shared__ __attribute__((aligned(16))) char smem_raw[];
    T* ks = (T*)smem_raw;
    const int rowf = hg * 32;
    T* vs = ks + (long)d.nk * rowf;
    const int s = blockIdx.x;
    const int h0 = blockIdx.y * hg;
    const int outer = s / d.inner, in = s - outer * d.inner;
    const long q_base = (long)outer * d.q_outer_stride + in;
    const long o_base = d.o_axis_stride ? (long)outer * d.o_outer_stride + in : q_base;
    const long o_step = d.o_axis_stride ? d.o_axis_stride : d.q_axis_stride;
    const long kv_base = (long)outer * d.kv_outer_stride + in;
    const T* kp = (const T*)d.k;
    const T* vp = (const T*)d.v;
    const int vec_per_row = rowf / 8;
    for (int e = threadIdx.x; e < d.nk * vec_per_row; e += 256) {
        const int j = e / vec_per_row, c = (e - j * vec_per_row) * 8;
        const long row = kv_base + (long)j * d.kv_axis_stride;
        copy8(kp + row * d.ldk + h0 * 32 + c, ks + j * rowf + c);
        copy8(vp + row * d.ldv + h0 * 32 + c, vs + j * rowf + c);
    }
    __syncthreads();
    int klen = d.nk;
    if (d.kv_len) klen = min(klen, d.kv_len[s / d.kv_len_div]);
    const unsigned drop_thresh = d.drop_p > 0.f ? (unsigned)((double)d.drop_p * 4294967296.0) : 0u;
    const float inv_keep = 1.0f / (1.0f - d.drop_p);
    const T* qp = (const T*)d.q;
    OT* op = (OT*)d.out;
    const int ldo = std::is_same<OT, T>::value ? d.ldo : d.ldo >> 1;
    for (int p = threadIdx.x; p < d.nq * hg; p += 256) {
        const int hl = p / d.nq, i = p - hl * d.nq;
        const long row = q_base + (long)i * d.q_axis_stride;
        f32x4 q[8];
#pragma unroll
        for (int c = 0; c < 4; ++c) {
            load8f(qp + row * d.ldq + (h0 + hl) * 32 + c * 8, q[2 * c], q[2 * c + 1]);
            q[2 * c] *= d.scale;
            q[2 * c + 1] *= d.scale;
        }
        const int jmax = d.causal ? min(klen, i + 1 + (d.nk - d.nq)) : klen;
        float sc[NK_MAX];
        float mx = -INFINITY;
#pragma unroll
        for (int j = 0; j < NK_MAX; ++j) {
            float a = -INFINITY;
            if (j < jmax) {
                const T* kr = ks + j * rowf + hl * 32;
                float a0 = 0.f, a1 = 0.f;
#pragma unroll
                for (int c = 0; c < 4; ++c) {
                    f32x4 k0, k1;
                    load8f(kr + c * 8, k0, k1);
                    a0 += q[2 * c][0] * k0[0] + q[2 * c][1] * k0[1] + q[2 * c][2] * k0[2] + q[2 * c][3] * k0[3];
                    a1 += q[2 * c + 1][0] * k1[0] + q[2 * c + 1][1] * k1[1] + q[2 * c + 1][2] * k1[2] + q[2 * c + 1][3] * k1[3];
                }
                a = a0 + a1;
            }
            sc[j] = a;
            mx = fmaxf(mx, a);
        }
        float den = 0.f;
        f32x4 o[8];
#pragma unroll
        for (int c = 0; c < 8; ++c) o[c] = f32x4{0.f, 0.f, 0.f, 0.f};
#pragma unroll
        for (int j = 0; j < NK_MAX; ++j) {
            if (j < jmax) {
                float pj = expf(sc[j] - mx);
                den += pj;
                if (drop_thresh) {
                    const unsigned long long idx = (((unsigned long long)s * d.n_head + (h0 + hl)) * d.nq + i) * d.nk + j;
                    pj = hash32(d.drop_seed * 0x9e3779b97f4a7c15ULL + idx) >= drop_thresh ? pj * inv_keep : 0.f;
                }
                const T* vr = vs + j * rowf + hl * 32;
#pragma unroll
                for (int c = 0; c < 4; ++c) {
                    f32x4 v0, v1;
                    load8f(vr + c * 8, v0, v1);
                    o[2 * c] += pj * v0;
                    o[2 * c + 1] += pj * v1;
                }
            }
        }
        const float inv = 1.0f / den;
        OT* orow = op + (o_base + (long)i * o_step) * ldo + (h0 + hl) * 32;
#pragma unroll
        for (int c = 0; c < 4; ++c) store8(orow + c * 8, o[2 * c] * inv, o[2 * c + 1] * inv);
    }
}

typedef __attribute__((ext_vector_type(8))) __bf16 abf16x8;
typedef __attribute__((ext_vector_type(4))) short ashort4;
typedef __attribute__((ext_vector_type(4))) _Float16 ahalf4;
template <typename HT> __device__ __forceinline__ void attn_p_split(float p, short& hi, short& lo) {
    if constexpr (std::is_same<HT, f16_t>::value) {
        const _Float16 h = (_Float16)p;
        hi = __builtin_bit_cast(short, h);
        lo = __builtin_bit_cast(short, (_Float16)(p - (float)h));
    } else {
        const unsigned hb = __float_as_uint(p) & 0xffff0000u;
        hi = (short)(hb >> 16);
        lo = (short)(__float_as_uint(p - __uint_as_float(hb)) >> 16);
    }
}
template <typename HT> __device__ __forceinline__ f32x4 attn_mfma_pv(const ashort4& vt, const ashort4& p, const f32x4& o) {
    if constexpr (std::is_same<HT, f16_t>::value)
        return __builtin_amdgcn_mfma_f32_16x16x16f16(__builtin_bit_cast(ahalf4, vt), __builtin_bit_cast(ahalf4, p), o, 0, 0, 0);
    else
        return __builtin_amdgcn_mfma_f32_16x16x16bf16_1k(vt, p, o, 0, 0, 0);
}
template <typename HT> __device__ __forceinline__ f32x4 attn_mfma_qk(const uint4& k, const uint4& q) {
    return mfma16x16x32<HT>(__builtin_bit_cast(u32x4, k), __builtin_bit_cast(u32x4, q), f32x4{0.f, 0.f, 0.f, 0.f});
}

template <int NKB, int MAXH, typename HT = unsigned short>
__global__ __launch_bounds__(256) void attention_mfma_kernel(const mage_attn_desc d) {
    extern __shared__ __attribute__((aligned(16))) char smem_raw[];
    unsigned short* vs = (unsigned short*)smem_raw;
    const int rowf = d.n_head * 32, vpitch = rowf + 16;
    const int s = blockIdx.x;
    const int outer = s / d.inner, in = s - outer * d.inner;
    const long q_base = (long)outer * d.q_outer_stride + in;
    const long o_base = d.o_axis_stride ? (long)outer * d.o_outer_stride + in : q_base;
    const long o_step = d.o_axis_stride ? d.o_axis_stride : d.q_axis_stride;
    const long kv_base = (long)outer * d.kv_outer_stride + in;
    const unsigned short* qp = (const unsigned short*)d.q;
    const unsigned short* kp = (const unsigned short*)d.k;
    const unsigned short* vp = (const unsigned short*)d.v;
    HT* op = (HT*)d.out;
    const int vec_per_row = rowf / 8;
    for (int e = threadIdx.x; e < 16 * NKB * vec_per_row; e += 256) {
        const int j = e / vec_per_row, c = (e - j * vec_per_row) * 8;
        uint4 val = uint4{0u, 0u, 0u, 0u};
        if (j < d.nk) val = *(const uint4*)(vp + (kv_base + (long)j * d.kv_axis_stride) * d.ldv + c);
        *(uint4*)(vs + j * vpitch + c) = val;
    }
    int klen = d.nk;
    if (d.kv_len) klen = min(klen, d.kv_len[s / d.kv_len_div]);
    const int lane = threadIdx.x & 63, wave = threadIdx.x >> 6;
    const int r = lane & 15, g = lane >> 4;
    uint4 kf[MAXH][NKB];
#pragma unroll
    for (int t = 0; t < MAXH; ++t) {
        const int h = wave + 4 * t;
        if (h < d.n_head) {
#pragma unroll
            for (int kb = 0; kb < NKB; ++kb) {
                const long krow = kv_base + (long)min(kb * 16 + r, d.nk - 1) * d.kv_axis_stride;
                kf[t][kb] = *(const uint4*)(kp + krow * d.ldk + h * 32 + g * 8);
            }
        }
    }
    __syncthreads();
    const int nqb = (d.nq + 15) >> 4;
    for (int qb = 0; qb < nqb; ++qb) {
        const int qi = qb * 16 + r;
        const long qrow = q_base + (long)min(qi, d.nq - 1) * d.q_axis_stride;
        const int jmax = d.causal ? min(klen, qi + 1 + (d.nk - d.nq)) : klen;
        uint4 qf[MAXH];
#pragma unroll
        for (int t = 0; t < MAXH; ++t) {
            const int h = wave + 4 * t;
            if (h < d.n_head) qf[t] = *(const uint4*)(qp + qrow * d.ldq + h * 32 + g * 8);
        }
#pragma unroll
        for (int t = 0; t < MAXH; ++t) {
            const int h = wave + 4 * t;
            if (h >= d.n_head) break;
            f32x4 st[NKB];
            float mx = -INFINITY;
#pragma unroll
            for (int kb = 0; kb < NKB; ++kb) {
                st[kb] = attn_mfma_qk<HT>(kf[t][kb], qf[t]);
#pragma unroll
                for (int e = 0; e < 4; ++e) {
                    st[kb][e] = (kb * 16 + 4 * g + e < jmax) ? st[kb][e] * d.scale : -INFINITY;
                    mx = fmaxf(mx, st[kb][e]);
                }
            }
            mx = fmaxf(mx, __shfl_xor(mx, 16));
            mx = fmaxf(mx, __shfl_xor(mx, 32));
            float den = 0.f;
            ashort4 phi[NKB], plo[NKB];
#pragma unroll
            for (int kb = 0; kb < NKB; ++kb)
#pragma unroll
                for (int e = 0; e < 4; ++e) {
                    const float p = (kb * 16 + 4 * g + e < jmax) ? expf(st[kb][e] - mx) : 0.f;
                    den += p;
                    short ph, pl;
                    attn_p_split<HT>(p, ph, pl);
                    phi[kb][e] = ph;
                    plo[kb][e] = pl;
                }
            den += __shfl_xor(den, 16);
            den += __shfl_xor(den, 32);
            f32x4 o[2];
#pragma unroll
            for (int b = 0; b < 2; ++b) {
                o[b] = f32x4{0.f, 0.f, 0.f, 0.f};
#pragma unroll
                for (int kb = 0; kb < NKB; ++kb) {
                    const unsigned short* vr = vs + (kb * 16 + 4 * g) * vpitch + h * 32 + b * 16 + r;
                    ashort4 vt;
#pragma unroll
                    for (int e = 0; e < 4; ++e) vt[e] = (short)vr[e * vpitch];
                    o[b] = attn_mfma_pv<HT>(vt, phi[kb], o[b]);
                    o[b] = attn_mfma_pv<HT>(vt, plo[kb], o[b]);
                }
            }
            const float inv = 1.0f / den;
            f32x4 v0, v1;
#pragma unroll
            for (int e = 0; e < 4; ++e) {
                const auto sw = __builtin_amdgcn_permlane16_swap(__float_as_uint(o[0][e]), __float_as_uint(o[1][e]), false, false);
                v0[e] = __uint_as_float(sw[0]) * inv;
                v1[e] = __uint_as_float(sw[1]) * inv;
            }
            if (qi < d.nq) {
                const int col = h * 32 + 16 * (g & 1) + 8 * (g >> 1);
                store8(op + (o_base + (long)qi * o_step) * d.ldo + col, v0, v1);
            }
        }
    }
}

template <int N> __device__ __forceinline__ float row_shr_f(float old, float src) {
    if constexpr (N == 0) return src;
    else return __uint_as_float(__builtin_amdgcn_update_dpp(__float_as_uint(old), __float_as_uint(src), 0x110 + N, 0xf, 0xf, false));
}
template <int N> __device__ __forceinline__ unsigned row_shl_u(unsigned src) {
    if constexpr (N == 0) return src;
    else return __builtin_amdgcn_update_dpp(src, src, 0x100 + N, 0xf, 0xf, false);
}
template <int N> __device__ __forceinline__ float row_shl_f(float src) { return __uint_as_float(row_shl_u<N>(__float_as_uint(src))); }
template <int N> __device__ __forceinline__ ashort4 row_shl_s4(ashort4 src) {
    const uint2 u = __builtin_bit_cast(uint2, src);
    return __builtin_bit_cast(ashort4, uint2{row_shl_u<N>(u.x), row_shl_u<N>(u.y)});
}

template <int NKB, typename HT = unsigned short>
__global__ __launch_bounds__(256) void attention_mfma_fewq_kernel(const mage_attn_desc d) {
    const int lane = threadIdx.x & 63;
    const int s = blockIdx.x * 4 + (threadIdx.x >> 6);
    if (s >= d.n_seq) return;
    const int outer = s / d.inner, in = s - outer * d.inner;
    const long q_base = (long)outer * d.q_outer_stride + in;
    const long o_base = d.o_axis_stride ? (long)outer * d.o_outer_stride + in : q_base;
    const long o_step = d.o_axis_stride ? d.o_axis_stride : d.q_axis_stride;
    const long kv_base = (long)outer * d.kv_outer_stride + in;
    const unsigned short* qp = (const unsigned short*)d.q;
    const unsigned short* kp = (const unsigned short*)d.k;
    const unsigned short* vp = (const unsigned short*)d.v;
    HT* op = (HT*)d.out;
    int klen = d.nk;
    if (d.kv_len) klen = min(klen, d.kv_len[s / d.kv_len_div]);
    const int r = lane & 15, g = lane >> 4;
    const int qi = r;
    const long qrow = q_base + (long)min(qi, d.nq - 1) * d.q_axis_stride;
    long krow[NKB], krow_v[NKB];
#pragma unroll
    for (int kb = 0; kb < NKB; ++kb) {
        krow[kb] = (kv_base + (long)min(kb * 16 + r, d.nk - 1) * d.kv_axis_stride) * d.ldk;
        krow_v[kb] = (kv_base + (long)min(kb * 16 + r, d.nk - 1) * d.kv_axis_stride) * d.ldv;
    }
// ... 945 lines not shown
```

mage_amd/modules/mage_model.py:

```python
from __future__ import annotations

import contextlib
import ctypes
import gc
import math
from collections import OrderedDict
from math import exp
from typing import Dict, Optional, Tuple

import torch
from torch import nn

from .. import config, ops
from ..utils.util import default, instantiate_from_config, zero_module
from .vqvae_model import VectorQuantizedVAE, _Derived, _conv_w, _no_torch_forward, weights_frozen

__all__ = ["QuickGELU", "AxialAttentionBlock", "TransformerBlock", "MAEncoder", "TransformerTextEncoder", "BasicBlock",
           "ADAIN2D", "FlatAxialDecoder", "PIDControl", "MAGE"]

F32 = torch.float32
BF16 = torch.bfloat16
F16 = torch.float16
HALF_TYPES = (BF16, F16)

# ... 197 lines not shown
        self.layer_norm = nn.LayerNorm(transformer_width, eps=1e-8, elementwise_affine=True)
        self.dropout = nn.Dropout(p=dropout)
        self.ln_text_final = nn.LayerNorm(transformer_width)
        self.text_projection = nn.Linear(transformer_width, output_dim)
        self.apply(self._init_weights)
        self._derived = _Derived(self)

    @staticmethod
    def _init_weights(module):
        if isinstance(module, nn.Linear):
            module.weight.data.normal_(mean=0.0, std=0.02)
        elif isinstance(module, nn.MultiheadAttention):
            module.in_proj_weight.data.normal_(mean=0.0, std=0.02)
            module.out_proj.weight.data.normal_(mean=0.0, std=0.02)
        elif isinstance(module, nn.Embedding):
            module.weight.data.normal_(mean=0.0, std=0.02)
            if module.padding_idx is not None:
                module.weight.data[module.padding_idx].zero_()

    def _build(self):
        d: Dict[str, torch.Tensor] = {"tok": self.token_embedding.weight.float().contiguous(),
                                      "pos": self.positions.weight.float().contiguous()}
        for n in ("layer_norm", "ln_text_final"):
            d[n + ".w"], d[n + ".b"] = getattr(self, n).weight.float().contiguous(), getattr(self, n).bias.float().contiguous()
        _pack_linear(d, "proj", self.text_projection.weight, self.text_projection.bias)
        for i, l in enumerate(self.transformer.layers):
            _pack_linear(d, f"l{i}.in_proj", l.self_attn.in_proj_weight, l.self_attn.in_proj_bias)
            _pack_linear(d, f"l{i}.out_proj", l.self_attn.out_proj.weight, l.self_attn.out_proj.bias)
            _pack_linear(d, f"l{i}.fc1", l.linear1.weight, l.linear1.bias)
            _pack_linear(d, f"l{i}.fc2", l.linear2.weight, l.linear2.bias)
            for n in ("norm1", "norm2"):
                d[f"l{i}.{n}.w"], d[f"l{i}.{n}.b"] = getattr(l, n).weight.float().contiguous(), getattr(l, n).bias.float().contiguous()
                d[f"l{i}.{n}.eps"] = getattr(l, n).eps
        return d

    @torch.no_grad()
    def forward(self, text: torch.Tensor) -> torch.Tensor:
        _need_gpu(text, "TransformerTextEncoder")
        d = self._derived.get(self._build)
        B, S = text.shape
        if S > 64 or S > self.context_length:
            raise ValueError(f"caption length {S} exceeds context_length {self.context_length} (kernel limit 64)")
        Wd, dev, H = self.transformer_width, text.device, self.transformer_width // 32
        ids = text.to(torch.int64).contiguous()
        kv_len, keep = ops.caption_mask(ids, self.padding_idx)
        x = ops.embedding(ids, d["tok"], torch.empty(B * S, Wd, device=dev, dtype=F32))
        ops.row_affine(x, None, d["pos"], div=1, mod=S)
        ops.layernorm(x, d["layer_norm.w"], d["layer_norm.b"], x, self.layer_norm.eps)
        ops.row_affine(x, keep, None)
        sk = getattr(self, "split_kind", 0) if Wd % 64 == 0 else 0
        for i in range(self.transformer_layers):
            p = f"l{i}"
            qkv = _lin_fp32(x, d, p + ".in_proj", torch.empty(B * S, 3 * Wd, device=dev, dtype=F32), M=B * S, N=3 * Wd, K=Wd, sk=sk)
            ao = ops.split_empty(B * S, Wd, sk, dev) if sk else torch.empty(B * S, Wd, device=dev, dtype=F32)
            ops.attention(qkv, qkv[:, Wd:], qkv[:, 2 * Wd:], ao, ldq=3 * Wd, ldk=3 * Wd, ldv=3 * Wd, ldo=2 * Wd if sk else Wd, n_seq=B, inner=1,
                          nq=S, nk=S, n_head=H, q_outer_stride=S, q_axis_stride=1, kv_outer_stride=S, kv_axis_stride=1,
                          kv_len=kv_len, kv_len_div=1, out_split=sk)
            _lin_fp32(ao, d, p + ".out_proj", x, M=B * S, N=Wd, K=Wd, sk=sk, a_split=ao if sk else None, residual=x, ldr=Wd)
            ops.layernorm(x, d[p + ".norm1.w"], d[p + ".norm1.b"], x, d[p + ".norm1.eps"])
            hdn = _linear(x, d, p + ".fc1", torch.empty(B * S, 4 * Wd, device=dev, dtype=F32), F32, M=B * S, N=4 * Wd, K=Wd,
                          act=ops.ACT_GELU_ERF)
            _lin_fp32(hdn, d, p + ".fc2", x, M=B * S, N=Wd, K=4 * Wd, sk=sk, residual=x, ldr=Wd)
            ops.layernorm(x, d[p + ".norm2.w"], d[p + ".norm2.b"], x, d[p + ".norm2.eps"])
        ops.layernorm(x, d["ln_text_final.w"], d["ln_text_final.b"], x, self.ln_text_final.eps)
        out = _lin_fp32(x, d, "proj", torch.empty(B * S, self.output_dim, device=dev, dtype=F32), M=B * S, N=self.output_dim, K=Wd, sk=sk)
        return out.view(B, S, self.output_dim)


class BasicBlock(nn.Module):

    def __init__(self, in_planes, out_planes, stride=1, stride_t=1, downsample=False, spectral=False):
        super().__init__()
        st = [stride_t, stride, stride]
        self.conv1 = nn.Conv3d(in_planes, out_planes, kernel_size=(3, 3, 3), stride=st, padding=1, bias=False)
        self.bn1 = nn.GroupNorm(num_groups=16, num_channels=out_planes)
        self.relu = nn.ReLU(inplace=True)
        self.conv2 = nn.Conv3d(out_planes, out_planes, kernel_size=(3, 3, 3), stride=[1, 1, 1], padding=1, bias=False)
        self.bn2 = nn.GroupNorm(num_groups=16, num_channels=out_planes)
        self.downsample = nn.Sequential(nn.Conv3d(in_planes, out_planes, kernel_size=(3, 3, 3), stride=st, padding=[1, 1, 1],
                                                  bias=False),
                                        nn.GroupNorm(num_channels=out_planes, num_groups=16)) if downsample else None
        self.stride = stride
        if spectral:
            self.conv1 = torch.nn.utils.spectral_norm(self.conv1)
            self.conv2 = torch.nn.utils.spectral_norm(self.conv2)

    forward = _no_torch_forward


class ADAIN2D(nn.Module):

    def __init__(self, num_features, z_dim):
        super().__init__()
        self.num_features = num_features
        self.norm = nn.InstanceNorm2d(num_features, affine=False, track_running_stats=False)
        self.conv_mu = nn.Sequential(nn.Conv2d(z_dim, num_features, 3, 1, 1), nn.Conv2d(num_features, num_features, 3, 1, 1))
        self.conv_var = nn.Sequential(nn.Conv2d(z_dim, num_features, 3, 1, 1), nn.Conv2d(num_features, num_features, 3, 1, 1))
        self._derived = _Derived(self)

    def _build(self):
        d: Dict[str, torch.Tensor] = {}
        for n, seq in (("mu", self.conv_mu), ("var", self.conv_var)):
            for j in range(2):
                d[f"{n}{j}.w"] = _conv_w(seq[j])
                d[f"{n}{j}.b"] = seq[j].bias.float().contiguous()
        return d

    @torch.no_grad()
    def _run(self, x_rows: torch.Tensor, y_rows: torch.Tensor, B: int, H: int, W: int) -> torch.Tensor:
        d = self._derived.get(self._build)
        Cc, z, dev = self.num_features, y_rows.shape[1], x_rows.device
        outs = []
        for n in ("mu", "var"):
            t = VectorQuantizedVAE._conv(y_rows, d[n + "0.w"], torch.empty(B * H * W, Cc, device=dev, dtype=F32), n_img=B, H=H,
                                         W=W, cin=z, cout=Cc, k=3, bias=d[n + "0.b"])
            outs.append(VectorQuantizedVAE._conv(t, d[n + "1.w"], torch.empty(B * H * W, Cc, device=dev, dtype=F32), n_img=B,
                                                 H=H, W=W, cin=Cc, cout=Cc, k=3, bias=d[n + "1.b"]))
        return ops.adain(x_rows, outs[0], outs[1], torch.empty_like(x_rows), B=B, P=H * W, Cc=Cc, eps=self.norm.eps)

    def forward(self, x: torch.Tensor, y: torch.Tensor) -> torch.Tensor:
        _need_gpu(x, "ADAIN2D")
        B, Cc, H, W = x.shape
        xr = x.permute(0, 2, 3, 1).reshape(B * H * W, Cc).float().contiguous()
        yr = y.permute(0, 2, 3, 1).reshape(B * H * W, -1).float().contiguous()
        return self._run(xr, yr, B, H, W).view(B, H, W, Cc).permute(0, 3, 1, 2)


class FlatAxialDecoder(nn.Module):

    def __init__(self, in_channels, model_channels, out_channels, frames_length, layers, context_channels=None, use_cids=True,
                 dropout=0.1):
        super().__init__()
        self.in_channels, self.model_channels, self.out_channels = in_channels, model_channels, out_channels
        self.frames_length, self.layers = frames_length, layers
        self.in_linear = nn.Linear(in_channels, model_channels)
        context_channels = default(context_channels, in_channels)
        self.context_channels = context_channels
        self.context_linear = nn.Linear(context_channels, model_channels)
        scale = model_channels ** -0.5
        self.T_positional_embedding = nn.Parameter(scale * torch.randn(frames_length, 1, 1, model_channels))
        num_heads = model_channels // 32
        self.blocks = nn.ModuleList([AxialAttentionBlock(model_channels, num_heads, axial_dim=i % 3 + 1, dropout=dropout)
                                     for i in range(layers)])
        self.use_cids = use_cids
        if use_cids:
            self.out = nn.Linear(model_channels, out_channels)
        else:
            self.out = nn.Sequential(nn.GroupNorm(32, model_channels), nn.SiLU(),
                                     zero_module(nn.Conv3d(model_channels, out_channels, 1)))
        self.initialize_parameters()
        self.compute_dtype = F32
        self.split_kind = 0
        self.stream_bf16 = True
        self._derived = _Derived(self)

    def initialize_parameters(self):
        proj_std = (self.model_channels ** -0.5) * ((2 * self.layers) ** -0.5)
        attn_std = self.model_channels ** -0.5
        fc_std = (2 * self.model_channels) ** -0.5
        for block in self.blocks:
            nn.init.normal_(block.attn.in_proj_weight, std=attn_std)
            nn.init.normal_(block.attn.out_proj.weight, std=proj_std)
            nn.init.normal_(block.mlp.c_fc.weight, std=fc_std)
            nn.init.normal_(block.mlp.c_proj.weight, std=proj_std)

    def build_casual_attention_mask(self):
        mask = torch.empty(self.frames_length, self.frames_length)
        mask.fill_(float("-inf"))
        mask.triu_(1)
        return mask

    def _build(self):
        d: Dict[str, torch.Tensor] = {}
        _pack_linear(d, "in_linear", self.in_linear.weight, self.in_linear.bias)
        _pack_linear(d, "context_linear", self.context_linear.weight, self.context_linear.bias)
        if self.use_cids:
            _pack_linear(d, "out", self.out.weight, self.out.bias)
        else:
            d["gn.w"], d["gn.b"] = self.out[0].weight.float().contiguous(), self.out[0].bias.float().contiguous()
            w = self.out[2].weight.float().reshape(self.out_channels, self.model_channels)
            n8 = (self.out_channels + 7) // 8 * 8
            wp = torch.zeros(n8, self.model_channels, device=w.device)
            wp[:self.out_channels] = w
            bp = torch.zeros(n8, device=w.device)
            bp[:self.out_channels] = self.out[2].bias.float()
            _pack_linear(d, "out", wp, bp)
        d["tpos"] = self.T_positional_embedding.float().reshape(self.frames_length, self.model_channels).contiguous()
        for i, blk in enumerate(self.blocks):
            _pack_block(d, f"b{i}", blk)
            for ln, lin in (("ln_1", "in_proj"), ("ln_2", "c_fc")):
                w, g, bt = d[f"b{i}.{lin}.f32"], d[f"b{i}.{ln}.w"], d[f"b{i}.{ln}.b"]
                wq = (w * g[None, :]).to(BF16)
                d[f"b{i}.{lin}.lnw"] = wq
                d[f"b{i}.{lin}.lns"] = wq.float().sum(dim=1).contiguous()
                d[f"b{i}.{lin}.lnc"] = ((w.double() * bt.double()[None, :]).sum(1) + d[f"b{i}.{lin}.b"].double()).float().contiguous()
        return d

    def _fold(self, dt, B: int, hw: int) -> bool:
        return (dt in HALF_TYPES and (B * hw) % 256 == 0 and self.model_channels % 256 == 0 and config.get().ln_fold)

    def _stream_bf16(self) -> bool:
        return getattr(self, "stream_bf16", True) and config.get().stream_16bit

    def _ln_linear(self, d, p, lin, xn, xb, ln, y, *, M, N, **kw):
        Cc, name = self.model_channels, f"{p}.{lin}"
        if ln is None:
            return ops.gemm(xn, _wdt(d, name, self.compute_dtype), y, M=M, N=N, K=Cc, lda=Cc, ldy=N, bias=d[name + ".b"], **kw)
        lnw, lns = self._ln_fold_w(d, p, lin, xb.dtype)
        return ops.gemm(xb, lnw, y, M=M, N=N, K=Cc, lda=Cc, ldy=N, bias=d[name + ".lnc"], ln_colsum=lns, **ln, **kw)

    @staticmethod
    def _ln_fold_w(d, p, lin, dt):
        if dt == BF16:
            return d[f"{p}.{lin}.lnw"], d[f"{p}.{lin}.lns"]
        kw_, ks_ = f"{p}.{lin}.lnw.f16", f"{p}.{lin}.lns.f16"
        if kw_ not in d:
            ln = "ln_1" if lin == "in_proj" else "ln_2"
            wq = (d[f"{p}.{lin}.f32"] * d[f"{p}.{ln}.w"][None, :]).to(F16)
            d[kw_], d[ks_] = wq, wq.float().sum(dim=1).contiguous()
        return d[kw_], d[ks_]

    def _stats_inline(self, xb, M: int) -> bool:
        Cc = self.model_channels
        return all(ops.gemm_is_small(xb, M, n, Cc) for n in (Cc, 2 * Cc, 3 * Cc, 4 * Cc))

    @torch.no_grad()
    def _run(self, motion: torch.Tensor, imgs: torch.Tensor, *, B: int, hh: int, ww: int) -> torch.Tensor:
        L = self.frames_length
        run = self._pass_split if self._split_on() else self._pass
        return run(motion, imgs, B=B, hh=hh, ww=ww, p0=0, P=L, nf=L - 1, cache=None)

    def _inc_begin(self, B: int, hh: int, ww: int) -> dict:
        return {"B": B, "hh": hh, "ww": ww, "kv": {}, "p": 0}

    @torch.no_grad()
    def _inc_step(self, st: dict, motion: Optional[torch.Tensor], imgs: torch.Tensor) -> torch.Tensor:
        p0 = st["p"]
        P = 2 if motion is not None else 1
        assert self.use_cids and (p0 == 0) == (motion is not None) and p0 + P <= self.frames_length
        run = self._pass_split if self._split_on() else self._pass
        logits = run(motion, imgs, B=st["B"], hh=st["hh"], ww=st["ww"], p0=p0, P=P, nf=1, cache=st["kv"])
        st["p"] = p0 + P
        return logits

    def _axial_geo(self, axis: int, B: int, hh: int, ww: int, P: int, p0: int = 0, *, cached: bool = False,
                   q_cached: bool = False) -> dict:
        hw, H = hh * ww, self.model_channels // 32
        if axis == 1:
            return dict(n_seq=B * P * ww, inner=ww, nq=hh, nk=hh, q_outer_stride=hw, q_axis_stride=ww, causal=False,
                        kv_outer_stride=hw, kv_axis_stride=ww, n_head=H)
        if axis == 2:
            return dict(n_seq=B * P * hh, inner=1, nq=ww, nk=ww, q_outer_stride=ww, q_axis_stride=1, causal=False,
                        kv_outer_stride=ww, kv_axis_stride=1, n_head=H)
        kvo = (self.frames_length if cached else P) * hw
        geo = dict(n_seq=B * hw, inner=hw, nq=P, nk=p0 + P, q_outer_stride=kvo if q_cached else P * hw, q_axis_stride=hw, causal=True,
                   kv_outer_stride=kvo, kv_axis_stride=hw, n_head=H)
        if q_cached:
            geo.update(o_outer_stride=P * hw, o_axis_stride=hw)
        return geo

    def _embed(self, d, x, motion, imgs, *, B: int, hw: int, P: int, nf: int, tp: torch.Tensor, sk: int = 0) -> None:
        dt, Cc = self.compute_dtype, self.model_channels
        if motion is not None:
            if sk and self._taps_ok(B * hw):
                self._lin_s(ops.split(motion, sk), d, "context_linear", x, M=B * hw, N=Cc, K=self.context_channels, out_w=hw,
                            y_img_stride=P * hw, rowadd=tp, rowadd_div=hw, rowadd_mod=P)
            else:
                _linear(motion, d, "context_linear", x, dt, M=B * hw, N=Cc, K=self.context_channels, out_w=hw, y_img_stride=P * hw,
                        rowadd=tp, rowadd_div=hw, rowadd_mod=P)
        off = (P - nf) * hw
        if isinstance(imgs, FrameTokens):
            imgs.fill(x, n_img=B * nf, per_clip=nf, P=P, y_off=off, tp=tp)
        elif sk and imgs.dtype != F32:
            self._lin_s(imgs, d, "in_linear", x, M=B * nf * hw, N=Cc, K=self.in_channels, out_w=nf * hw, y_img_stride=P * hw, y_off=off,
                        rowadd=tp, rowadd_div=hw, rowadd_mod=P)
        else:
            _linear(imgs, d, "in_linear", x, dt, M=B * nf * hw, N=Cc, K=self.in_channels, out_w=nf * hw, y_img_stride=P * hw, y_off=off,
                    rowadd=tp, rowadd_div=hw, rowadd_mod=P)

    def _head(self, d, xa, *, B: int, hw: int, P: int, nf: int, split: bool = False) -> torch.Tensor:
        dt, Cc, rows = self.compute_dtype, self.model_channels, B * nf * hw
        if not self.use_cids:
            y = ops.groupnorm_silu(xa, d["gn.w"], d["gn.b"], torch.empty(rows, Cc, device=xa.device, dtype=dt), n_samples=B,
                                   rows_per_sample=nf * hw, sample_stride_rows=P * hw, row_off=(P - nf) * hw, groups=32, eps=self.out[0].eps)
            n8 = d["out.f32"].shape[0]
            return _linear(y, d, "out", torch.empty(rows, n8, device=xa.device, dtype=F32), dt, M=rows, N=n8, K=Cc)
        logits = torch.empty(rows, self.out_channels, device=xa.device, dtype=F32)
        if split:
            return self._lin_s(xa, d, "out", logits, M=rows, N=self.out_channels, K=Cc, out_w=nf * hw, a_img_stride=P * hw, a_off=(P - nf) * hw)
        return _linear(xa, d, "out", logits, dt, M=rows, N=self.out_channels, K=Cc, out_w=nf * hw, a_img_stride=P * hw, a_off=(P - nf) * hw)

    def _pass(self, motion, imgs, *, B: int, hh: int, ww: int, p0: int, P: int, nf: int, cache: Optional[dict]) -> torch.Tensor:
        d = self._derived.get(self._build)
        dt, Cc, L = self.compute_dtype, self.model_channels, self.frames_length
        dev = (imgs.tokens if isinstance(imgs, FrameTokens) else imgs).device
        hw = hh * ww
        M = B * P * hw
        fold = self._fold(dt, B, hw)
        sb = fold and self._stream_bf16()
        xb = part = stats = None
        if fold:
            xb = torch.empty(M, Cc, device=dev, dtype=dt)
            part = torch.empty(Cc // 64, M, 2, device=dev, dtype=F32)
            stats = torch.empty(M, 2, device=dev, dtype=F32)
        inl = fold and self._stats_inline(xb, M)
        ln = None if not fold else dict(ln_part=part, ln_eps=1e-5) if inl else dict(ln_stats=stats)
        ln0 = dict(ln_stats=stats) if sb else None
        x = xb if sb else torch.empty(M, Cc, device=dev, dtype=F32)
        res = dict(residual=x, ldr=Cc)
        if fold:
            res["ln_part"] = part
            if not sb:
                res.update(y2=xb, ldy2=Cc)
        self._embed(d, x, motion, imgs, B=B, hw=hw, P=P, nf=nf, tp=d["tpos"][p0:])
        if sb:
            ops.row_stats(xb, 1e-5, stats)
        xn = torch.empty(M, Cc, device=dev, dtype=dt)
        qkv = torch.empty(M, 3 * Cc, device=dev, dtype=dt)
        ao = torch.empty(M, Cc, device=dev, dtype=dt)
        hdn = torch.empty(M, 4 * Cc, device=dev, dtype=dt)
        geo = [self._axial_geo(a, B, hh, ww, P, p0, cached=cache is not None, q_cached=cache is not None) for a in range(3)]
        for i in range(self.layers):
            p = f"b{i}"
            ln1 = ln if i else ln0
            if ln1 is None:
                ops.layernorm(x, d[p + ".ln_1.w"], d[p + ".ln_1.b"], xn, 1e-5)
            if i % 3 == 0 and cache is not None:
                if p0 == 0:
                    cache[i] = torch.empty(B * L * hw, 3 * Cc, device=dev, dtype=dt)
                kv = cache[i]
                self._ln_linear(d, p, "in_proj", xn, xb, ln1, kv, M=M, N=3 * Cc, out_w=P * hw, y_img_stride=L * hw, y_off=p0 * hw)
                q = kv[p0 * hw:]
            else:
                q = kv = qkv
                self._ln_linear(d, p, "in_proj", xn, xb, ln1, qkv, M=M, N=3 * Cc)
            ops.attention(q, kv[:, Cc:], kv[:, 2 * Cc:], ao, ldq=3 * Cc, ldk=3 * Cc, ldv=3 * Cc, ldo=Cc, **geo[i % 3])
            _linear(ao, d, p + ".out_proj", x, dt, M=M, N=Cc, K=Cc, **res)
            if fold and not inl:
                ops.ln_stats(part, Cc, 1e-5, stats)
            if ln is None:
                ops.layernorm(x, d[p + ".ln_2.w"], d[p + ".ln_2.b"], xn, 1e-5)
            self._ln_linear(d, p, "c_fc", xn, xb, ln, hdn, M=M, N=4 * Cc, act=ops.ACT_QUICKGELU)
            if i < self.layers - 1:
                _linear(hdn, d, p + ".c_proj", x, dt, M=M, N=Cc, K=4 * Cc, **res)
                if fold and not inl:
                    ops.ln_stats(part, Cc, 1e-5, stats)
            else:
                if self.use_cids and dt != F32:
                    xa = xn
                else:
                    xa = torch.empty(M, Cc, device=dev, dtype=F32) if sb else x
                _linear(hdn, d, p + ".c_proj", xa, dt, M=M, N=Cc, K=4 * Cc, residual=x, ldr=Cc)
        return self._head(d, xa, B=B, hw=hw, P=P, nf=nf)

    def _split_on(self) -> bool:
        return bool(self.split_kind) and self.compute_dtype == F32 and self.model_channels % 64 == 0

    def _warm_split(self) -> None:
        if not self._split_on():
            return
        d = self._derived.get(self._build)
        names = ["in_linear", "context_linear"] + (["out"] if self.use_cids else [])
        for i in range(self.layers):
            names += [f"b{i}.in_proj", f"b{i}.out_proj", f"b{i}.c_fc", f"b{i}.c_proj"]
        for n in names:
            _wsplit(d, n, self.split_kind)

    def _attn_split(self) -> bool:
        return (self.split_kind == ops.F16X3 and self.frames_length <= 32 and (self.model_channels // 32) % 2 == 0
                and config.get().attn_split)

    def _taps_ok(self, rows: int) -> bool:
        return self.model_channels % 256 == 0 and rows % 256 == 0 and self.in_channels % 64 == 0 and self.context_channels % 64 == 0

    def _lin_s(self, a, d, name, y, *, M, N, K, lo=0, hi=None, **kw):
        sk = self.split_kind
        w, b = _wsplit(d, name, sk), d.get(name + ".b")
        if hi is not None or lo:
            w, b = w[lo:hi], (None if b is None else b[lo:hi])
        y_split = kw.pop("y_split", False)
        return ops.gemm(a, w, y, M=M, N=N, K=K, lda=kw.pop("lda", 2 * K), ldy=kw.pop("ldy", 2 * N if y_split else N), bias=b,
                        split_kind=sk, y_split=y_split, **kw)

    def _pass_split(self, motion, imgs, *, B: int, hh: int, ww: int, p0: int, P: int, nf: int, cache: Optional[dict]) -> torch.Tensor:
        d = self._derived.get(self._build)
        sk, Cc, L = self.split_kind, self.model_channels, self.frames_length
        dev = (imgs.tokens if isinstance(imgs, FrameTokens) else imgs).device
        hw = hh * ww
        M = B * P * hw
        x = torch.empty(M, Cc, device=dev, dtype=F32)
        self._embed(d, x, motion, imgs, B=B, hw=hw, P=P, nf=nf, tp=d["tpos"][p0:], sk=sk)
        xn = ops.split_empty(M, Cc, sk, dev)
        qs = self._attn_split()
        m_ = 2 if qs else 1
        qkv = ops.split_empty(M, 3 * Cc, sk, dev) if qs else torch.empty(M, 3 * Cc, device=dev, dtype=F32)
        ao = ops.split_empty(M, Cc, sk, dev)
        hdn = ops.split_empty(M, 4 * Cc, sk, dev)
        geo = [self._axial_geo(a, B, hh, ww, P, p0, cached=cache is not None) for a in range(3)]
        for i in range(self.layers):
            p = f"b{i}"
            ops.layernorm(x, d[p + ".ln_1.w"], d[p + ".ln_1.b"], xn, 1e-5, split_kind=sk)
            if i % 3 == 0 and cache is not None:
                if p0 == 0:
                    cache[i] = ops.split_empty(B * L * hw, 2 * Cc, sk, dev) if qs else torch.empty(B * L * hw, 2 * Cc, device=dev, dtype=F32)
                kv = cache[i]
                q = qkv.view(-1)[:M * m_ * Cc].view(M, m_ * Cc)
                self._lin_s(xn, d, p + ".in_proj", q, M=M, N=Cc, K=Cc, lo=0, hi=Cc, ldy=m_ * Cc, y_split=qs)
                self._lin_s(xn, d, p + ".in_proj", kv, M=M, N=2 * Cc, K=Cc, lo=Cc, hi=3 * Cc, ldy=m_ * 2 * Cc, out_w=P * hw,
                            y_img_stride=L * hw, y_off=p0 * hw, y_split=qs)
                k, v, ldq, ldkv = kv, kv[:, m_ * Cc:], m_ * Cc, m_ * 2 * Cc
            else:
                self._lin_s(xn, d, p + ".in_proj", qkv, M=M, N=3 * Cc, K=Cc, y_split=qs)
                q, k, v, ldq, ldkv = qkv, qkv[:, m_ * Cc:], qkv[:, m_ * 2 * Cc:], m_ * 3 * Cc, m_ * 3 * Cc
            ops.attention(q, k, v, ao, ldq=ldq, ldk=ldkv, ldv=ldkv, ldo=2 * Cc, out_split=sk, split_kind=sk if qs else 0, **geo[i % 3])
            self._lin_s(ao, d, p + ".out_proj", x, M=M, N=Cc, K=Cc, residual=x, ldr=Cc)
            ops.layernorm(x, d[p + ".ln_2.w"], d[p + ".ln_2.b"], xn, 1e-5, split_kind=sk)
            self._lin_s(xn, d, p + ".c_fc", hdn, M=M, N=4 * Cc, K=Cc, act=ops.ACT_QUICKGELU, y_split=True)
            if i == self.layers - 1 and self.use_cids:
                self._lin_s(hdn, d, p + ".c_proj", xn, M=M, N=Cc, K=4 * Cc, residual=x, ldr=Cc, y_split=True)
            else:
                self._lin_s(hdn, d, p + ".c_proj", x, M=M, N=Cc, K=4 * Cc, residual=x, ldr=Cc)
        return self._head(d, xn if self.use_cids else x, B=B, hw=hw, P=P, nf=nf, split=True)

    def forward(self, motion: torch.Tensor, imgs: torch.Tensor) -> torch.Tensor:
        _need_gpu(motion, "FlatAxialDecoder")
        B, hh, ww, _ = motion.shape
        dt = self.compute_dtype
        m = motion.reshape(B * hh * ww, -1).to(dt).contiguous()
        im = imgs.reshape(-1, imgs.shape[-1]).to(dt).contiguous()
        out = self._run(m, im, B=B, hh=hh, ww=ww)
        return out.view(B, self.frames_length - 1, hh, ww, -1)[..., :self.out_channels]


class PIDControl:

    def __init__(self):
        self.I_k1 = 0.0
        self.W_k1 = 0.0
        self.e_k1 = 0.0

    def _Kp_fun(self, Err, scale=1):
        return 1.0 / (1.0 + float(scale) * exp(Err))

    def pid(self, exp_KL, KL_loss, Kp=0.01, Ki=-0.0001, Kd=0.0):
        error_k = exp_KL - KL_loss
        Pk = Kp * self._Kp_fun(error_k)
        Ik = self.I_k1 + Ki * error_k
        if self.W_k1 < 0 and self.W_k1 >= 1:
            Ik = self.I_k1
        Wk = Pk + Ik
        self.W_k1, self.I_k1, self.e_k1 = Wk, Ik, error_k
        return min(max(Wk, 0.0), 1.0), error_k


def disabled_train(self, mode=True):
    return self


class MAGE(nn.Module):
    def __init__(self, first_stage_config, text_encoder_config, ma_config, generate_decoder_config, codebook_size: int,
                 frames_length: int, image_resolution: int, vision_width: int, dropout: float = 0.1, use_cids=False,
                 randomness=False, alpha=0., beta=1., v_kl=0., auto_beta=False):
        super().__init__()
        self.instantiate_first_stage(first_stage_config)
        self.frames_length, self.image_resolution, self.vision_width = frames_length, image_resolution, vision_width
        self.dropout, self.use_cids, self.auto_beta = dropout, use_cids, auto_beta
        self.text_encoder = instantiate_from_config(text_encoder_config)
        self.ma_encoder = instantiate_from_config(ma_config, {"dropout": dropout})
        if hasattr(self.ma_encoder, "mage_plus"):
            self.ma_encoder.mage_plus = not use_cids
        self.generate_model = instantiate_from_config(
            generate_decoder_config, {"use_cids": use_cids, "dropout": dropout, "context_channels": ma_config["params"]["d_model"]})
        self.codebook_size = codebook_size
        if use_cids:
            self.visual_token_embedding = nn.Embedding(codebook_size, vision_width)
        else:
            self.visual_token_embedding = nn.Linear(self.first_stage_model.embed_dim, vision_width)
        self.conv = nn.Sequential(nn.Conv2d(vision_width, vision_width, kernel_size=3, stride=1, padding=1, bias=False))
        scale = vision_width ** -0.5
        self.speed_embedding = nn.Parameter(scale * torch.randn(1, vision_width))
        self.H_positional_embedding = nn.Parameter(scale * torch.randn(1, image_resolution, 1, vision_width))
        self.W_positional_embedding = nn.Parameter(scale * torch.randn(1, 1, image_resolution, vision_width))
        self.randomness = randomness
        if randomness:
            dm = ma_config["params"]["d_model"]
            self.conv3d = nn.Sequential(*[BasicBlock(vision_width, vision_width if i < 3 else dm, stride=1, stride_t=2,
                                                     downsample=True) for i in range(4)])
            self.conv_mu2 = nn.Conv2d(vision_width, 64, 3, 1, 1)
            self.conv_var2 = nn.Conv2d(vision_width, 64, 3, 1, 1)
# ... 1220 lines not shown
```

mage_amd/ops.py:

```python
from __future__ import annotations

import ctypes as C
from typing import Optional

import torch

from . import _lib
from ._lib import ACT_GELU_ERF, ACT_NONE, ACT_QUICKGELU, ACT_QUICKGELU_GRAD, ACT_RELU, ACT_TANH, BF16, BF16X3, F16, F16X3, F32, AttnDesc, GemmDesc

__all__ = ["gemm", "layernorm", "attention", "embedding", "table_conv", "split_rows", "vq_prepare", "vq_nearest", "argmax", "cross_entropy",
           "conv_in", "conv_out", "convt_fold_tanh", "row_affine", "groupnorm_silu", "groupnorm_act", "reparam_kl", "mse", "check_device_errors", "graph_events_supported", "transpose", "row_sum", "sum_partials", "layernorm_bwd", "dropout_add_layernorm", "act", "act_bwd", "cross_entropy_bwd", "embedding_bwd", "group_rowsum", "attention_bwd", "dropout", "adam", "adam_clipped", "sumsq", "bn_train_stats", "bn_apply", "bn_backward", "convt_unfold_tanh_bwd", "maxpool2", "upsample2", "relu", "cast", "adain", "add_scaled_rowvec",
           "token_logprob", "clip_scores", "video_metrics", "group_advantages", "policy_loss", "policy_loss_bwd", "preference_loss", "token_logprob_bwd", "split", "split_empty", "split_dtype", "PROFILE", "F32", "BF16", "F16", "BF16X3", "F16X3", "ACT_NONE", "ACT_RELU", "ACT_QUICKGELU", "ACT_GELU_ERF", "ACT_TANH", "tdtype", "code"]


def code(t: torch.Tensor) -> int:
    if t.dtype == torch.float32:
        return F32
    if t.dtype == torch.bfloat16:
        return BF16
    if t.dtype == torch.float16:
        return F16
    raise TypeError(f"unsupported dtype {t.dtype}")


# ... 89 lines not shown
        self.records = []
        self.only = None
        self.external = False
        self.acc = {}

    def reset(self, enabled: bool = False, only=None):
        self.enabled, self.records, self.only = enabled, [], (set(only) if only is not None else None)
        self.acc = {}

    def clear(self):
        self.records, self.acc = [], {}

    def mode_key(self):
        if not self.enabled:
            return "off"
        return "all" if self.only is None else tuple(sorted(self.only))

    def wants(self, key: str) -> bool:
        return self.enabled and (self.only is None or key in self.only)

    def begin(self):
        e = torch.cuda.Event(enable_timing=True, external=True) if self.external else torch.cuda.Event(enable_timing=True)
        e.record()
        return e

    def end(self, key: str, start, flops: float = 0.0, nbytes: float = 0.0):
        e = torch.cuda.Event(enable_timing=True, external=True) if self.external else torch.cuda.Event(enable_timing=True)
        e.record()
        self.records.append((key, start, e, flops, nbytes))

    def capture_begin(self):
        saved = (self.records, self.external)
        self.records, self.external = [], True
        return saved

    def capture_end(self, saved):
        recs = self.records
        self.records, self.external = saved
        return recs

    def _add(self, out, recs):
        for key, s, e, fl, nb in recs:
            d = out.setdefault(key, {"ms": 0.0, "calls": 0, "flops": 0.0, "bytes": 0.0})
            d["ms"] += s.elapsed_time(e)
            d["calls"] += 1
            d["flops"] += fl
            d["bytes"] += nb

    def absorb(self, recs):
        if self.enabled and recs:
            self._add(self.acc, recs)

    def summary(self):
        torch.cuda.synchronize()
        out = {k: dict(v) for k, v in self.acc.items()}
        self._add(out, self.records)
        return out


PROFILE = _Profile()


def gemm(a: torch.Tensor, w: torch.Tensor, y: torch.Tensor, *, M: int, N: int, K: int, lda: int, ldy: int,
         out_h: int = 1, out_w: Optional[int] = None, in_h: Optional[int] = None, in_w: Optional[int] = None,
         a_img_stride: Optional[int] = None, a_off: int = 0, taps_h: int = 1, taps_w: int = 1, cin: Optional[int] = None,
         stride: int = 1, dy0: int = 0, dx0: int = 0, dys: int = 1, dxs: int = 1,
         y_img_stride: Optional[int] = None, y_mul_y: Optional[int] = None, y_mul_x: int = 1, y_off: int = 0,
         bias=None, scale=None, shift=None, act: int = ACT_NONE, rowadd=None, rowadd_div: int = 1, rowadd_mod: int = 1,
         residual=None, ldr: int = 0, post_relu: bool = False, ldw: int = 0, n_split: int = 1, a_split_stride: int = 0,
         w_split_stride: int = 0, y_split_stride: int = 0, y2=None, ldy2: int = 0, ln_part=None, ln_stats=None,
         ln_colsum=None, res_half: bool = False, a_half: bool = False, split_kind: int = 0, y_split: bool = False,
         ln_eps: float = 0.0, head_w=None, head_phases: int = 0, a_relu: bool = False) -> torch.Tensor:
    l, s = _dev(a)
    if split_kind and a_relu:
        raise ValueError("ops.gemm: split-precision operands (split_kind) do not take a_relu")
    if split_kind:
        unsupported = dict(scale=scale, shift=shift, y2=y2, ln_part=ln_part, ln_stats=ln_stats, ln_colsum=ln_colsum, head_w=head_w)
        bad = [k for k, v_ in unsupported.items() if v_ is not None]
        bad += [k for k, v_ in dict(post_relu=post_relu, res_half=res_half, a_half=a_half).items() if v_]
        bad += [k for k, v_ in dict(n_split=n_split).items() if v_ not in (0, 1)]
        bad += [k for k, v_ in dict(a_split_stride=a_split_stride, w_split_stride=w_split_stride, y_split_stride=y_split_stride, ldy2=ldy2,
                                    stride=stride - 1, dy0=dy0, dx0=dx0, dys=dys - 1, dxs=dxs - 1).items() if v_]
        if ln_eps:
            bad.append("ln_eps")
        if bad:
            raise ValueError(f"ops.gemm: split-precision operands (split_kind) do not take {', '.join(bad)}")
        if residual is not None and residual.dtype != torch.float32:
            raise ValueError(f"ops.gemm: the split-precision x + Linear(.) form adds an fp32 residual, got {residual.dtype}")
        return _gemm_split(l, s, a, w, y, M=M, N=N, K=K, lda=lda, ldy=ldy, out_h=out_h, out_w=out_w, in_h=in_h, in_w=in_w,
                           a_img_stride=a_img_stride, a_off=a_off, taps_h=taps_h, taps_w=taps_w, cin=cin, y_img_stride=y_img_stride,
                           y_mul_y=y_mul_y, y_mul_x=y_mul_x, y_off=y_off, bias=bias, act=act, rowadd=rowadd, rowadd_div=rowadd_div,
                           rowadd_mod=rowadd_mod, residual=residual, ldr=ldr, ldw=ldw, split_kind=split_kind, y_split=y_split)
    out_w = M if out_w is None else out_w
    in_h = out_h if in_h is None else in_h
    in_w = out_w if in_w is None else in_w
    d = GemmDesc()
    d.dtype, d.M, d.N, d.K = code(a), M, N, K
    assert w.dtype == a.dtype, (w.dtype, a.dtype)
    d.A, d.W, d.Y = a.data_ptr(), w.data_ptr(), y.data_ptr()
    d.lda, d.ldy, d.y_dtype = lda, ldy, code(y)
    d.out_h, d.out_w, d.in_h, d.in_w = out_h, out_w, in_h, in_w
    d.a_img_stride = in_h * in_w if a_img_stride is None else a_img_stride
    d.a_off = a_off
    d.taps_h, d.taps_w, d.cin, d.stride = taps_h, taps_w, (K // (taps_h * taps_w) if cin is None else cin), stride
    d.dy0, d.dx0, d.dys, d.dxs = dy0, dx0, dys, dxs
    d.y_img_stride = out_h * out_w if y_img_stride is None else y_img_stride
    d.y_mul_y = out_w if y_mul_y is None else y_mul_y
    d.y_mul_x, d.y_off = y_mul_x, y_off
    d.bias, d.scale, d.shift = _p(bias), _p(scale), _p(shift)
    d.act = act
    d.rowadd, d.rowadd_div, d.rowadd_mod = _p(rowadd), rowadd_div, rowadd_mod
    d.residual, d.ldr, d.res_dtype = _p(residual), ldr, (code(residual) if residual is not None else 0)
    d.post_relu = int(post_relu)
    d.ldw, d.n_split = ldw, n_split
    d.a_split_stride, d.w_split_stride, d.y_split_stride = a_split_stride, w_split_stride, y_split_stride
    d.y2, d.ldy2, d.ln_part, d.ln_stats, d.ln_colsum = _p(y2), ldy2, _p(ln_part), _p(ln_stats), _p(ln_colsum)
    d.ln_eps = float(ln_eps)
    if ln_part is not None:
        assert ln_part.dtype == torch.float32 and ln_part.dim() == 3 and ln_part.shape[2] == 2 and ln_part.is_contiguous(), tuple(ln_part.shape)
        d.ln_part_rows = ln_part.shape[1]
    if head_w is not None:
        assert head_w.dtype == torch.bfloat16 and head_w.is_contiguous() and tuple(head_w.shape) == (16, N // (head_phases or 1)) \
            and y.dtype == torch.float32, (head_w.dtype, tuple(head_w.shape), y.dtype)
    d.head_w = _p(head_w)
    d.head_phases = head_phases if head_w is not None else 0
    d.res_half = int(res_half)
    d.a_half = int(a_half)
    d.a_relu = int(a_relu)
    if PROFILE.enabled:
        key = _kernel_name(l, d)
        if PROFILE.wants(key):
            ev = PROFILE.begin()
            _lib.check(l.mage_gemm(C.byref(d), s), l)
            es, ys = a.element_size(), y.element_size()
            nb = float(M) * K * es + float(N) * K * es + float(M) * N * ys
            if key == "conv3x3_c64_kernel":
                nb = float(M) * 64 * es * (0.25 if a_half else 1.0) + float(N) * K * es + float(M) * N * ys
            if residual is not None:
                nb += float(M) * N * residual.element_size()
            if y2 is not None:
                nb += float(M) * N * 2
            if ln_part is not None:
                nb += float(M) * (N // 64) * 8
            fl = 2.0 * M * N * K
            if head_w is not None:
                nb += float(M) * 16 * 4 * (head_phases or 1) - float(M) * N * ys
                fl += 2.0 * M * N * 16
            PROFILE.end(key, ev, fl, nb)
            return y
    _lib.check(l.mage_gemm(C.byref(d), s), l)
    return y


def gemm_is_small(a: torch.Tensor, M: int, N: int, K: int) -> bool:
    l, _ = _dev(a)
    r = l.mage_gemm_is_small(M, N, K)
    if r < 0:
        _lib.check(r, l)
    return r == 1


def _gemm_split(l, s, a, w, y, *, M, N, K, lda, ldy, out_h, out_w, in_h, in_w, a_img_stride, a_off, taps_h, taps_w, cin, y_img_stride, y_mul_y,
                y_mul_x, y_off, bias, act, rowadd, rowadd_div, rowadd_mod, residual, ldr, ldw, split_kind, y_split):
    sd = split_dtype(split_kind)
    assert a.dtype == sd and w.dtype == sd and (y.dtype == sd if y_split else y.dtype == torch.float32), (a.dtype, w.dtype, y.dtype)
    out_w = M if out_w is None else out_w
    in_h = out_h if in_h is None else in_h
    in_w = out_w if in_w is None else in_w
    d = GemmDesc()
    d.dtype, d.M, d.N, d.K = split_kind, M, N, K
    d.A, d.W, d.Y = a.data_ptr(), w.data_ptr(), y.data_ptr()
    d.lda, d.ldy, d.y_dtype = lda, ldy, (split_kind if y_split else F32)
    d.out_h, d.out_w, d.in_h, d.in_w = out_h, out_w, in_h, in_w
    d.a_img_stride = in_h * in_w if a_img_stride is None else a_img_stride
    d.a_off = a_off
    d.taps_h, d.taps_w, d.cin, d.stride = taps_h, taps_w, (K // (taps_h * taps_w) if cin is None else cin), 1
    d.dy0, d.dx0, d.dys, d.dxs = 0, 0, 1, 1
    d.y_img_stride = out_h * out_w if y_img_stride is None else y_img_stride
    d.y_mul_y = out_w if y_mul_y is None else y_mul_y
    d.y_mul_x, d.y_off = y_mul_x, y_off
    d.bias, d.act = _p(bias), act
    d.rowadd, d.rowadd_div, d.rowadd_mod = _p(rowadd), rowadd_div, rowadd_mod
    d.residual, d.ldr, d.res_dtype = _p(residual), ldr, F32
    d.ldw, d.n_split = ldw, 1
    if PROFILE.enabled:
        key = _kernel_name(l, d)
        if PROFILE.wants(key):
            ev = PROFILE.begin()
            _lib.check(l.mage_gemm(C.byref(d), s), l)
            nb = 4.0 * M * K + 4.0 * N * K + float(M) * N * 4 * (2 if residual is not None else 1)
            PROFILE.end(key, ev, 2.0 * M * N * K, nb)
            return y
    _lib.check(l.mage_gemm(C.byref(d), s), l)
    return y


def row_stats(x: torch.Tensor, eps: float, stats: torch.Tensor) -> torch.Tensor:
    l, s = _dev(x)
    assert x.dtype in (torch.bfloat16, torch.float16) and x.dim() == 2 and x.stride(1) == 1 and stats.is_contiguous() and stats.numel() >= 2 * x.shape[0]
    ev = PROFILE.begin() if PROFILE.wants("layernorm") else None
    _lib.check(l.mage_row_stats(x.data_ptr(), code(x), x.shape[0], x.shape[1], x.stride(0), float(eps), stats.data_ptr(), s), l)
    if ev is not None:
        PROFILE.end("layernorm", ev, 0.0, float(x.numel()) * 2)
    return stats


def ln_stats(part: torch.Tensor, C_: int, eps: float, stats: torch.Tensor) -> torch.Tensor:
    l, s = _dev(part)
    n_slices, rows = part.shape[0], part.shape[1]
    assert part.dtype == torch.float32 and part.is_contiguous() and stats.is_contiguous() and stats.numel() >= 2 * rows
    if PROFILE.wants("ln_stats_kernel"):
        ev = PROFILE.begin()
        _lib.check(l.mage_ln_stats(part.data_ptr(), rows, n_slices, C_, eps, stats.data_ptr(), s), l)
        PROFILE.end("ln_stats_kernel", ev, 0.0)
        return stats
    _lib.check(l.mage_ln_stats(part.data_ptr(), rows, n_slices, C_, eps, stats.data_ptr(), s), l)
    return stats


def layernorm(x: torch.Tensor, gamma: torch.Tensor, beta: torch.Tensor, y: torch.Tensor, eps: float, split_kind: int = 0) -> torch.Tensor:
    l, s = _dev(x)
    assert x.dtype == torch.float32 and x.is_contiguous() and y.is_contiguous()
    Cc = x.shape[-1]
    assert not split_kind or (y.dtype == split_dtype(split_kind) and y.numel() == 2 * x.numel())
    ev = PROFILE.begin() if PROFILE.wants("layernorm") else None
    _lib.check(l.mage_layernorm(x.data_ptr(), gamma.data_ptr(), beta.data_ptr(), y.data_ptr(), split_kind or code(y),
                                x.numel() // Cc, Cc, float(eps), s), l)
    if ev is not None:
        PROFILE.end("layernorm", ev, 0.0, float(x.numel()) * (4 + y.element_size()))
    return y


def attention(q, k, v, out, *, ldq, ldk, ldv, ldo, n_seq, inner, nq, nk, n_head, q_outer_stride, q_axis_stride,
              kv_outer_stride, kv_axis_stride, causal=False, kv_len=None, kv_len_div=1, scale=None, out_split: int = 0,
              drop_p: float = 0.0, drop_seed: int = 0, split_kind: int = 0, o_outer_stride: int = 0, o_axis_stride: int = 0):
    l, s = _dev(q)
    d = AttnDesc()
    d.dtype = split_kind or code(q)
    d.q, d.k, d.v, d.out = q.data_ptr(), k.data_ptr(), v.data_ptr(), out.data_ptr()
    d.ldq, d.ldk, d.ldv, d.ldo = ldq, ldk, ldv, ldo
    d.n_seq, d.inner, d.nq, d.nk, d.n_head = n_seq, inner, nq, nk, n_head
    d.q_outer_stride, d.q_axis_stride = q_outer_stride, q_axis_stride
    d.kv_outer_stride, d.kv_axis_stride = kv_outer_stride, kv_axis_stride
    d.causal = int(causal)
    d.kv_len, d.kv_len_div = _p(kv_len), kv_len_div
    d.scale = float(32 ** -0.5 if scale is None else scale)
    d.out_split = out_split
    d.drop_p, d.drop_seed = float(drop_p), int(drop_seed) & (2 ** 64 - 1)
    d.o_outer_stride, d.o_axis_stride = o_outer_stride, o_axis_stride
    ev = PROFILE.begin() if PROFILE.wants("attention") else None
    _lib.check(l.mage_attention(C.byref(d), s), l)
    if ev is not None:
        es = q.element_size()
        PROFILE.end("attention", ev, 4.0 * n_seq * nq * nk * n_head * 32, float(n_seq) * n_head * 32 * es * (2 * nq + 2 * nk))
    return out


def embedding(ids: torch.Tensor, table: torch.Tensor, out: torch.Tensor, *, relu: bool = False, group: Optional[int] = None,
              group_stride: Optional[int] = None, off: int = 0, inner: int = 0, inner_stride: int = 0, split_kind: int = 0) -> torch.Tensor:
    l, s = _dev(table)
    assert ids.dtype == torch.int64 and ids.is_contiguous() and table.dtype == torch.float32 and table.is_contiguous()
    n = ids.numel()
    group = n if group is None else group
    group_stride = group if group_stride is None else group_stride
    _lib.check(l.mage_embedding(ids.data_ptr(), table.data_ptr(), out.data_ptr(), split_kind or code(out), n, table.shape[1],
                                table.shape[0], int(relu), group, group_stride, off, inner, inner_stride, s), l)
    return out


def table_conv(ids: torch.Tensor, table: torch.Tensor, y: torch.Tensor, *, n_img: int, H: int, W: int, taps: int = 3, pos=None, bias=None,
               relu: bool = False, rowadd=None, split_kind: int = 0,
               rowadd_div: int = 1, rowadd_mod: int = 1, ldy: Optional[int] = None, group: Optional[int] = None,
               y_group_stride: Optional[int] = None, y_off: int = 0) -> torch.Tensor:
    l, s = _dev(table)
    assert ids.dtype == torch.int64 and ids.is_contiguous() and ids.numel() == n_img * H * W
    assert table.dim() == 3 and table.shape[0] == taps * taps and table.is_contiguous()
    Cc = table.shape[2]
    group = n_img * H * W if group is None else group
    y_group_stride = group if y_group_stride is None else y_group_stride
    ev = PROFILE.begin() if PROFILE.wants("table_conv") else None
    _lib.check(l.mage_table_conv(ids.data_ptr(), n_img, H, W, taps, taps, table.data_ptr(), code(table), table.shape[1], Cc, _p(pos), _p(bias),
                                 int(relu), _p(rowadd), rowadd_div, rowadd_mod, y.data_ptr(), split_kind or code(y), Cc if ldy is None else ldy, group,
                                 y_group_stride, y_off, s), l)
    if ev is not None:
        PROFILE.end("table_conv", ev, 0.0, float(n_img) * H * W * Cc * (taps * taps * table.element_size() + 4))
    return y


def resblock_table(ids: torch.Tensor, table: torch.Tensor, codebook: torch.Tensor, w1: torch.Tensor, y: torch.Tensor, *, n_img: int, H: int, W: int,
                   bias3: torch.Tensor, b1: torch.Tensor, scale1=None, shift1=None, post_relu: bool = False, ldy: int, y_img_stride: int,
                   y_row_pitch: int, y_off: int = 0) -> torch.Tensor:
    l, s = _dev(table)
    Cc = table.shape[2]
    assert ids.dtype == torch.int64 and ids.is_contiguous() and ids.numel() == n_img * H * W
    assert table.dtype == torch.bfloat16 and table.dim() == 3 and table.shape[0] == 9 and table.is_contiguous()
    assert codebook.dtype == torch.float32 and codebook.is_contiguous() and tuple(codebook.shape) == (table.shape[1], Cc)
    assert w1.dtype == torch.bfloat16 and w1.is_contiguous() and tuple(w1.shape) == (Cc, Cc) and y.dtype == torch.bfloat16
    ev = PROFILE.begin() if PROFILE.wants("resblock_table") else None
    _lib.check(l.mage_resblock_table(ids.data_ptr(), n_img, H, W, table.data_ptr(), table.shape[1], Cc, bias3.data_ptr(), codebook.data_ptr(),
                                     w1.data_ptr(), b1.data_ptr(), _p(scale1), _p(shift1), int(post_relu), y.data_ptr(), ldy, y_img_stride,
                                     y_row_pitch, y_off, s), l)
    if ev is not None:
        npix = float(n_img) * H * W
        PROFILE.end("resblock_table", ev, 2.0 * npix * Cc * Cc, npix * (8 + 2 * Cc))
    return y

# ... 755 lines not shown
```

Baseline: 5827.

## Fuse axial attention into the in_proj GEMM epilogue for 16-token axes

```diff
diff --git a/include/mage_hip_ext.h b/include/mage_hip_ext.h
--- a/include/mage_hip_ext.h
+++ b/include/mage_hip_ext.h
@@ -49,6 +49,9 @@
 int mage_token_logprob_bwd(const float* logits, int64_t rows, int32_t K, int64_t ld, const int64_t* tokens, const float* weight,
                            int64_t weight_div, const float* grad_out, void* dlogits, int32_t dl_dtype, void* stream);
 
+int mage_gemm_attn_fused(const mage_gemm_desc* desc, int32_t phase, int32_t axis, float scale, float* p, void* stream);
+int mage_gemm_attn_fused_kernel_name(const mage_gemm_desc* desc, int32_t phase, int32_t axis, char* buf, int32_t len);
+
 #ifdef __cplusplus
 }
 #endif
diff --git a/mage_amd/_lib.py b/mage_amd/_lib.py
--- a/mage_amd/_lib.py
+++ b/mage_amd/_lib.py
@@ -132,6 +132,8 @@
     "mage_guide_logits": (C.c_int, [vp, vp, vp, i64, i32, i64, i64, i64, i64, vp, i64, vp]),
     "mage_preference_loss": (C.c_int, [vp, vp, i64, vp, i64, f32, f32, i32, vp, vp, vp, vp, vp]),
     "mage_token_logprob_bwd": (C.c_int, [vp, i64, i32, i64, vp, vp, i64, vp, vp, i32, vp]),
+    "mage_gemm_attn_fused": (C.c_int, [C.POINTER(GemmDesc), i32, i32, f32, vp, vp]),
+    "mage_gemm_attn_fused_kernel_name": (C.c_int, [C.POINTER(GemmDesc), i32, i32, C.c_char_p, i32]),
 }
 
 _lib: Optional[C.CDLL] = None
diff --git a/mage_amd/config.py b/mage_amd/config.py
--- a/mage_amd/config.py
+++ b/mage_amd/config.py
@@ -10,6 +10,7 @@
 
 @dataclasses.dataclass(frozen=True)
 class Config:
+    qk_fuse: bool = True
     ln_fold: bool = True
     stream_16bit: bool = True
     attn_split: bool = True
@@ -33,6 +34,7 @@
 
 ENV = {
     "ln_fold": ("MAGE_NO_LN_FOLD", False),
+    "qk_fuse": ("MAGE_NO_QK_FUSE", False),
     "stream_16bit": ("MAGE_STREAM_FP32", False),
     "attn_split": ("MAGE_ATTN_SPLIT_FP32", False),
     "frame_table": ("MAGE_NO_FRAME_TABLE", False),
diff --git a/mage_amd/csrc/attn_mfma.h b/mage_amd/csrc/attn_mfma.h
--- /dev/null
+++ b/mage_amd/csrc/attn_mfma.h
@@ -0,0 +1,31 @@
+#pragma once
+#include <type_traits>
+#include "common.h"
+
+namespace {
+
+typedef __attribute__((ext_vector_type(8))) __bf16 abf16x8;
+typedef __attribute__((ext_vector_type(4))) short ashort4;
+typedef __attribute__((ext_vector_type(4))) _Float16 ahalf4;
+template <typename HT> __device__ __forceinline__ void attn_p_split(float p, short& hi, short& lo) {
+    if constexpr (std::is_same<HT, f16_t>::value) {
+        const _Float16 h = (_Float16)p;
+        hi = __builtin_bit_cast(short, h);
+        lo = __builtin_bit_cast(short, (_Float16)(p - (float)h));
+    } else {
+        const unsigned hb = __float_as_uint(p) & 0xffff0000u;
+        hi = (short)(hb >> 16);
+        lo = (short)(__float_as_uint(p - __uint_as_float(hb)) >> 16);
+    }
+}
+template <typename HT> __device__ __forceinline__ f32x4 attn_mfma_pv(const ashort4& vt, const ashort4& p, const f32x4& o) {
+    if constexpr (std::is_same<HT, f16_t>::value)
+        return __builtin_amdgcn_mfma_f32_16x16x16f16(__builtin_bit_cast(ahalf4, vt), __builtin_bit_cast(ahalf4, p), o, 0, 0, 0);
+    else
+        return __builtin_amdgcn_mfma_f32_16x16x16bf16_1k(vt, p, o, 0, 0, 0);
+}
+template <typename HT> __device__ __forceinline__ f32x4 attn_mfma_qk(const uint4& k, const uint4& q) {
+    return mfma16x16x32<HT>(__builtin_bit_cast(u32x4, k), __builtin_bit_cast(u32x4, q), f32x4{0.f, 0.f, 0.f, 0.f});
+}
+
+}
diff --git a/mage_amd/csrc/common.h b/mage_amd/csrc/common.h
--- a/mage_amd/csrc/common.h
+++ b/mage_amd/csrc/common.h
@@ -69,6 +69,7 @@
 
 int mage_gemm_cu_count();
 extern thread_local const void** mage_gemm_plan;
+int mage_kernel_symbol_name(const void* kernel, char* buf, int32_t len, const char* who);
 template <auto KERNEL, typename Args>
 int mage_gemm_launch(unsigned grid, unsigned block, unsigned lds, hipStream_t s, const Args& a) {
     if (mage_gemm_plan) {
diff --git a/mage_amd/csrc/gemm.hip b/mage_amd/csrc/gemm.hip
--- a/mage_amd/csrc/gemm.hip
+++ b/mage_amd/csrc/gemm.hip
@@ -113,13 +113,7 @@
 
 thread_local const void** mage_gemm_plan = nullptr;
 
-extern "C" int mage_gemm_kernel_name(const mage_gemm_desc* desc, char* buf, int32_t len) {
-    MAGE_CHECK_ARG(buf != nullptr && len > 0, "mage_gemm_kernel_name: no buffer");
-    const void* kernel = nullptr;
-    mage_gemm_plan = &kernel;
-    const int r = mage_gemm(desc, nullptr);
-    mage_gemm_plan = nullptr;
-    if (r != MAGE_OK) return r;
+int mage_kernel_symbol_name(const void* kernel, char* buf, int32_t len, const char* who) {
     static std::mutex mu;
     static std::unordered_map<const void*, std::string> names;
     std::string name;
@@ -130,7 +124,7 @@
             hipFunction_t f = nullptr;
             const char* raw = hipGetFuncBySymbol(&f, kernel) == hipSuccess ? hipKernelNameRef(f) : nullptr;
             if (!raw) {
-                mage_set_error("mage_gemm_kernel_name: the runtime has no name for the selected kernel");
+                mage_set_error("%s: the runtime has no name for the selected kernel", who);
                 return MAGE_EHIP;
             }
             std::string n = raw;
@@ -146,7 +140,17 @@
         }
         name = it->second;
     }
-    MAGE_CHECK_ARG((int32_t)name.size() < len, "mage_gemm_kernel_name: %d bytes are too few for '%s'", (int)len, name.c_str());
+    MAGE_CHECK_ARG((int32_t)name.size() < len, "%s: %d bytes are too few for '%s'", who, (int)len, name.c_str());
     memcpy(buf, name.c_str(), name.size() + 1);
     return MAGE_OK;
 }
+
+extern "C" int mage_gemm_kernel_name(const mage_gemm_desc* desc, char* buf, int32_t len) {
+    MAGE_CHECK_ARG(buf != nullptr && len > 0, "mage_gemm_kernel_name: no buffer");
+    const void* kernel = nullptr;
+    mage_gemm_plan = &kernel;
+    const int r = mage_gemm(desc, nullptr);
+    mage_gemm_plan = nullptr;
+    if (r != MAGE_OK) return r;
+    return mage_kernel_symbol_name(kernel, buf, len, "mage_gemm_kernel_name");
+}
diff --git a/mage_amd/csrc/gemm4.hip b/mage_amd/csrc/gemm4.hip
--- a/mage_amd/csrc/gemm4.hip
+++ b/mage_amd/csrc/gemm4.hip
@@ -4,6 +4,7 @@
 
 #include "gemm_shared.h"
 #include "gemm4_regs.h"
+#include "attn_mfma.h"
 
 namespace {
 
@@ -20,6 +21,10 @@
     int M, N, K, lda, ldw, ldy, ldr, ldy2, y_dtype, a_off, y_off;
     int ntiles_n, ntiles;
     int stagger_groups, stagger_sleeps;
+    float* attn_p;
+    int attn_axis;
+    float attn_scale;
+    int out_w, y_img_stride;
 };
 
 #ifndef MAGE4_ABL
@@ -51,9 +56,34 @@
     else asm volatile("v_mfma_f32_32x32x16_bf16 a[%c2:%c3], %0, %1, a[%c2:%c3]" ::"v"(w), "v"(x), "i"(16 * B), "i"(16 * B + 15));
 }
 #endif
-template <int ACT, int EK, int LN, bool RB, bool HF = false>
-__global__ __launch_bounds__(256) void gemm4_kernel(const Gemm4Args g) {
+typedef unsigned g4_u32x2 __attribute__((ext_vector_type(2)));
+template <bool HF>
+__device__ __forceinline__ f32x4 g4_epi_qk(const u32x4& k, const u32x4& q) {
+    f32x4 d;
+    if constexpr (HF) asm volatile("s_nop 1\n\tv_mfma_f32_16x16x32_f16 %0, %1, %2, 0\n\ts_nop 15" : "=&v"(d) : "v"(k), "v"(q));
+    else asm volatile("s_nop 1\n\tv_mfma_f32_16x16x32_bf16 %0, %1, %2, 0\n\ts_nop 15" : "=&v"(d) : "v"(k), "v"(q));
+    return d;
+}
+#define G4_EPI_PV(OP)                                                                                                                               \
+    asm volatile("s_nop 1\n\t" OP " %0, %2, %4, 0\n\t" OP " %1, %3, %4, 0\n\t" OP " %0, %2, %5, %0\n\t" OP " %1, %3, %5, %1\n\ts_nop 15"           \
+                 : "=&v"(o0), "=&v"(o1)                                                                                                             \
+                 : "v"(__builtin_bit_cast(g4_u32x2, vt0)), "v"(__builtin_bit_cast(g4_u32x2, vt1)), "v"(__builtin_bit_cast(g4_u32x2, phi)),          \
+                   "v"(__builtin_bit_cast(g4_u32x2, plo)))
+template <bool HF>
+__device__ __forceinline__ void g4_epi_pv(const ashort4& vt0, const ashort4& vt1, const ashort4& phi, const ashort4& plo, f32x4& o0, f32x4& o1) {
+    if constexpr (HF) G4_EPI_PV("v_mfma_f32_16x16x16_f16");
+    else G4_EPI_PV("v_mfma_f32_16x16x16_bf16");
+}
+
+template <bool SWAP, int I, bool ZERO, bool CLOB, bool HF>
+__device__ __forceinline__ void g4_mm(const u32x4& w, const u32x4& x) {
+    if constexpr (SWAP) g4_mfma<I, ZERO, CLOB, HF>(x, w);
+    else g4_mfma<I, ZERO, CLOB, HF>(w, x);
+}
+template <int ACT, int EK, int LN, bool RB, bool HF, int QF>
+__device__ __forceinline__ void gemm4_body(const Gemm4Args& g) {
     static_assert(EK != EK_GENERAL, "lean epilogue kinds");
+    static_assert(QF == 0 || (LN == LN_CONSUME && ACT == MAGE_ACT_NONE), "fused attention pair: the LayerNorm-consuming in_proj");
     static_assert(!HF || (LN != LN_DUAL && LN != LN_GELUBWD), "f16 form: the generation path's epilogues");
     typedef std::conditional_t<HF, f16_t, unsigned short> H16;
     extern __shared__ __attribute__((aligned(16))) char smem[];
@@ -73,14 +103,15 @@
 
     const int lr = lane >> 3, lp = lane & 7;
     unsigned voffA[8], voffW[8];
+    [[maybe_unused]] auto frame_row = [&](int R) { return g.attn_axis == 1 ? ((R & 15) << 4) + (R >> 4) : R; };
 #pragma unroll
     for (int u = 0; u < 8; ++u) {
         const int r = u * 8 + lr;
         const int ch = lp ^ ((r >> 1) & 7);
-        voffA[u] = (unsigned)(r * g.lda * 2 + ch * 16 + 8192 - u * 1024);
+        voffA[u] = (unsigned)((QF ? frame_row(wave * 64 + r) : r) * g.lda * 2 + ch * 16 + 8192 - u * 1024);
         voffW[u] = (unsigned)(r * g.ldw * 2 + ch * 16 + 8192 - u * 1024);
     }
-    auto a_base = [&](int tile) { return (const char*)g.A + ((long)((tile / g.ntiles_n) * 256 + wave * 64) + g.a_off) * g.lda * 2 - 4096; };
+    auto a_base = [&](int tile) { return (const char*)g.A + ((long)((tile / g.ntiles_n) * 256 + (QF ? 0 : wave * 64)) + g.a_off) * g.lda * 2 - 4096; };
     auto w_base = [&](int tile) { return (const char*)g.W + (long)((tile % g.ntiles_n) * 256 + wave * 64) * g.ldw * 2 - 4096; };
     const char* a_src = a_base(c_tile);
     const char* w_src = w_base(c_tile);
@@ -158,12 +189,20 @@
         f32x4 biasm[2][4];
         [[maybe_unused]] float ln_mean[8], ln_rstd[8];
         [[maybe_unused]] f32x4 lns[2][4];
+        [[maybe_unused]] f32x4 pl[4][2];
+        [[maybe_unused]] int ql15 = l15, qgrp = grp;
+        if constexpr (QF != 0) asm volatile("" : "+v"(ql15), "+v"(qgrp));
+        [[maybe_unused]] auto qf_p_request = [&](int mt, int h, int mh) __attribute__((always_inline)) {
+            const float* pp = g.attn_p + (((long)tm * 16 + wm * 8 + mh * 4 + mt) * (g.N >> 5) + (n0 >> 5) + h * 2) * 256 + (qgrp * 16 + ql15) * 4;
+#pragma unroll
+            for (int hd = 0; hd < 2; ++hd) pl[mt][hd] = *(const f32x4*)(pp + hd * 256);
+        };
         auto slab = [&](auto S_, auto FIRST_, auto LAST_, int j) __attribute__((always_inline)) {
             constexpr int S = decltype(S_)::value;
             constexpr bool FIRST = decltype(FIRST_)::value, LAST = decltype(LAST_)::value;
             g4_for<32>([&](auto i_) {
                 constexpr int i = decltype(i_)::value, m = i >> 3, nt = i & 7;
-                g4_mfma<((nt >> 2) * 8 + m) * 4 + (nt & 3), FIRST, i == 0, HF>(wf[0][nt], xf[0][m]);
+                g4_mm<QF == 2, ((nt >> 2) * 8 + m) * 4 + (nt & 3), FIRST, i == 0, HF>(wf[0][nt], xf[0][m]);
                 __builtin_amdgcn_sched_barrier(0);
                 if constexpr (!(MAGE4_ABL & 4) && i < 4) {
                     rd_x1(1, S, 0, 4 + i);
@@ -185,7 +224,7 @@
             if constexpr (!(MAGE4_ABL & 8) && !FIRST) w_src = (j == nk - 2) ? w_next : w_src + 128;
             g4_for<32>([&](auto i_) {
                 constexpr int i = decltype(i_)::value, m = i >> 3, nt = i & 7;
-                g4_mfma<((nt >> 2) * 8 + 4 + m) * 4 + (nt & 3), FIRST, i == 0, HF>(wf[0][nt], xf[1][m]);
+                g4_mm<QF == 2, ((nt >> 2) * 8 + 4 + m) * 4 + (nt & 3), FIRST, i == 0, HF>(wf[0][nt], xf[1][m]);
                 __builtin_amdgcn_sched_barrier(0);
                 if constexpr (!(MAGE4_ABL & 4) && i < 12) {
                     if constexpr (i < 4) rd_x1(0, S, 1, i);
@@ -196,6 +235,11 @@
             if constexpr (LAST) {
 #pragma unroll
                 for (int b = 0; b < 4; ++b) {
+                    if constexpr (QF == 2) {
+                        biasm[0][0][b] = g.bias[n0 + b * 16 + l15];
+                        lns[0][0][b] = g.ln_colsum[n0 + b * 16 + l15];
+                        continue;
+                    }
                     const int n = n0 + b * 16 + grp * 4;
                     biasm[0][b] = *(const f32x4*)(g.bias + n);
                     if constexpr (LN == LN_CONSUME) lns[0][b] = *(const f32x4*)(g.ln_colsum + n);
@@ -203,7 +247,8 @@
                 if constexpr (LN == LN_CONSUME) {
 #pragma unroll
                     for (int a = 0; a < 8; ++a) {
-                        const float2 st = *(const float2*)(g.ln_stats + 2 * (long)(m0 + a * 16 + l15));
+                        const long row = QF ? (long)tm * 256 + frame_row(wm * 128 + a * 16 + ql15) : (long)(m0 + a * 16 + l15);
+                        const float2 st = *(const float2*)(g.ln_stats + 2 * row);
                         ln_mean[a] = st.x;
                         ln_rstd[a] = st.y;
                     }
@@ -212,7 +257,7 @@
             }
             g4_for<32>([&](auto i_) {
                 constexpr int i = decltype(i_)::value, m = i >> 3, nt = i & 7;
-                g4_mfma<((nt >> 2) * 8 + m) * 4 + (nt & 3), false, i == 0, HF>(wf[1][nt], xf[0][m]);
+                g4_mm<QF == 2, ((nt >> 2) * 8 + m) * 4 + (nt & 3), false, i == 0, HF>(wf[1][nt], xf[0][m]);
                 __builtin_amdgcn_sched_barrier(0);
                 if constexpr (!(MAGE4_ABL & 4) && i < 4) {
                     rd_x1(1, S, 1, 4 + i);
@@ -220,13 +265,15 @@
                 }
             });
             if constexpr (MAGE4_ABL & 16) __builtin_amdgcn_s_waitcnt(0xC07F);
+            else if constexpr (FIRST && QF == 1) __builtin_amdgcn_s_waitcnt(0x007C);
+            else if constexpr (FIRST && QF == 2) __builtin_amdgcn_s_waitcnt(0x8070);
             else if constexpr (FIRST) __builtin_amdgcn_s_waitcnt(LN == LN_CONSUME ? 0x8074 : 0x8070);
             else __builtin_amdgcn_s_waitcnt(0x0070);
             ring_barrier();
             __builtin_amdgcn_sched_barrier(0);
             g4_for<32>([&](auto i_) {
                 constexpr int i = decltype(i_)::value, m = i >> 3, nt = i & 7;
-                g4_mfma<((nt >> 2) * 8 + 4 + m) * 4 + (nt & 3), false, i == 0, HF>(wf[1][nt], xf[1][m]);
+                g4_mm<QF == 2, ((nt >> 2) * 8 + 4 + m) * 4 + (nt & 3), false, i == 0, HF>(wf[1][nt], xf[1][m]);
                 __builtin_amdgcn_sched_barrier(0);
                 if constexpr (!(MAGE4_ABL & 4) && i < 12 && !LAST) {
                     if constexpr (i < 4) rd_x1(0, S ^ 1, 0, i);
@@ -244,6 +291,10 @@
                     if constexpr ((i & 1) == 1 && i < 16) g4_dma<(i >> 1)>(voffA[i >> 1], a_src);
                     if constexpr ((i & 1) == 1 && i > 16) g4_dma<((i - 16) >> 1)>(voffW[(i - 16) >> 1], w_src);
                     if constexpr (i == 0 || i == 16 || (i & 1) == 1) __builtin_amdgcn_sched_barrier(0);
+                }
+                if constexpr (QF == 2 && LAST && (i & 7) == 6) {
+                    qf_p_request(i >> 3, 0, 0);
+                    __builtin_amdgcn_sched_barrier(0);
                 }
             });
             if constexpr (!(MAGE4_ABL & 8)) a_src = (j == nk - 3) ? a_next : a_src + 128;
@@ -321,10 +372,112 @@
         char* win = smem + G4_RING + wave * 4096;
 #pragma unroll
         for (int b = 0; b < 4; ++b) {
+            if constexpr (QF == 2) {
+                biasm[1][0][b] = g.bias[n0 + 64 + b * 16 + l15];
+                lns[1][0][b] = g.ln_colsum[n0 + 64 + b * 16 + l15];
+                continue;
+            }
             const int n = n0 + 64 + b * 16 + grp * 4;
             biasm[1][b] = *(const f32x4*)(g.bias + n);
             if constexpr (LN == LN_CONSUME) lns[1][b] = *(const f32x4*)(g.ln_colsum + n);
         }
+        if constexpr (QF != 0) {
+            g4_for<4>([&](auto c_) {
+                constexpr int c = decltype(c_)::value, h = c >> 1, mh = c & 1;
+                __builtin_amdgcn_sched_barrier(0);
+                f32x4 t[4][4];
+                g4_for<16>([&](auto q_) {
+                    constexpr int q = decltype(q_)::value;
+                    t[q >> 2][q & 3] = g4_acc_read<(h * 8 + mh * 4 + (q >> 2)) * 4 + (q & 3), q == 0>();
+                });
+                if constexpr (QF == 1) {
+                    float* pp = g.attn_p + (((long)tm * 16 + wm * 8 + mh * 4) * (g.N >> 6) + (n0 >> 6) + h) * 256 + (qgrp * 16 + ql15) * 4;
+#pragma unroll
+                    for (int mt = 0; mt < 4; ++mt) {
+                        uint2 pk[4];
+#pragma unroll
+                        for (int nt = 0; nt < 4; ++nt) {
+                            const f32x4 v = (t[mt][nt] - lns[h][nt] * ln_mean[mh * 4 + mt]) * ln_rstd[mh * 4 + mt] + biasm[h][nt];
+                            pk[nt] = uint2{pack16x2<H16>(v[0], v[1]), pack16x2<H16>(v[2], v[3])};
+                        }
+                        f32x4 st = g4_epi_qk<HF>(u32x4{pk[2].x, pk[2].y, pk[3].x, pk[3].y}, u32x4{pk[0].x, pk[0].y, pk[1].x, pk[1].y});
+                        f32x4 p;
+                        {
+#pragma clang fp contract(off)
+                            float mx = -INFINITY;
+#pragma unroll
+                            for (int e = 0; e < 4; ++e) {
+                                st[e] = st[e] * g.attn_scale;
+                                mx = fmaxf(mx, st[e]);
+                            }
+                            mx = fmaxf(mx, __shfl_xor(mx, 16));
+                            mx = fmaxf(mx, __shfl_xor(mx, 32));
+#pragma unroll
+                            for (int e = 0; e < 4; ++e) p[e] = expf(st[e] - mx);
+                        }
+                        *(f32x4*)(pp + (long)mt * (g.N >> 6) * 256) = p;
+                    }
+                } else {
+                    const long shift = (long)(tm * 256 / g.out_w) * (g.y_img_stride - g.out_w) + g.y_off;
+                    const int srow = (qgrp * 16 + ql15) >> 3, scc = ql15 & 7;
+                    H16* op = (H16*)g.Y + n0 + h * 64 + scc * 8;
+                    const int wchunk = (qgrp & 1) * 2 + (qgrp >> 1);
+#pragma unroll
+                    for (int mt = 0; mt < 4; ++mt) {
+                        f32x4 mean4, rstd4;
+#pragma unroll
+                        for (int e = 0; e < 4; ++e) {
+                            mean4[e] = __shfl(ln_mean[mh * 4 + mt], 4 * grp + e);
+                            rstd4[e] = __shfl(ln_rstd[mh * 4 + mt], 4 * grp + e);
+                        }
+#pragma unroll
+                        for (int hd = 0; hd < 2; ++hd) {
+                            const f32x4 p = pl[mt][hd];
+                            float den = 0.f;
+                            ashort4 phi, plo;
+#pragma unroll
+                            for (int e = 0; e < 4; ++e) {
+                                den += p[e];
+                                short ph, pw;
+                                attn_p_split<H16>(p[e], ph, pw);
+                                phi[e] = ph;
+                                plo[e] = pw;
+                            }
+                            den += __shfl_xor(den, 16);
+                            den += __shfl_xor(den, 32);
+                            if constexpr (c < 3) {
+                                if (hd == 1) qf_p_request(mt, (c + 1) >> 1, (c + 1) & 1);
+                            }
+                            f32x4 o[2];
+                            ashort4 vt[2];
+#pragma unroll
+                            for (int b = 0; b < 2; ++b) {
+                                const int nt = hd * 2 + b;
+                                const f32x4 v = (t[mt][nt] - mean4 * lns[h][0][nt]) * rstd4 + biasm[h][0][nt];
+                                vt[b] = __builtin_bit_cast(ashort4, uint2{pack16x2<H16>(v[0], v[1]), pack16x2<H16>(v[2], v[3])});
+                            }
+                            g4_epi_pv<HF>(vt[0], vt[1], phi, plo, o[0], o[1]);
+                            const float inv = 1.0f / den;
+                            f32x4 v0, v1;
+#pragma unroll
+                            for (int e = 0; e < 4; ++e) {
+                                const auto sw = __builtin_amdgcn_permlane16_swap(__float_as_uint(o[0][e]), __float_as_uint(o[1][e]), false, false);
+                                v0[e] = __uint_as_float(sw[0]) * inv;
+                                v1[e] = __uint_as_float(sw[1]) * inv;
+                            }
+                            *(u32x4*)(win + ql15 * 128 + (((hd * 4 + wchunk) ^ ((ql15 >> 1) & 7)) << 4)) =
+                                u32x4{pack16x2<H16>(v0[0], v0[1]), pack16x2<H16>(v0[2], v0[3]), pack16x2<H16>(v1[0], v1[1]), pack16x2<H16>(v1[2], v1[3])};
+                        }
+#pragma unroll
+                        for (int i = 0; i < 2; ++i) {
+                            const int r = srow + 8 * i;
+                            const long yrow = (long)tm * 256 + frame_row(wm * 128 + mh * 64 + mt * 16 + r) + shift;
+                            *(u32x4*)(op + yrow * g.ldy) = *(const u32x4*)(win + r * 128 + ((scc ^ ((r >> 1) & 7)) << 4));
+                        }
+                    }
+                }
+            });
+        } else {
         mage_gemm_desc e = {};
         e.M = 0x7fffffff;
         e.N = LN == LN_PRODUCE ? g.N : 0x7fffffff;
@@ -365,6 +518,7 @@
                 else epilogue_lean<ACT, H16, 4, false, LN>(e, biasm[h], t, m0 + mh * 64, n0 + h * 64, lane, 1, win, 0);
             }
         });
+        }
 #endif
         G4_STAMP(it, 2);
         __builtin_amdgcn_sched_barrier(0);
@@ -383,8 +537,22 @@
 }
 
 template <int ACT, int EK, int LN, bool RB, bool HF = false>
-int launch4(const mage_gemm_desc* d, hipStream_t s, int n_cu) {
+__global__ __launch_bounds__(256) void gemm4_kernel(const Gemm4Args g) {
+    gemm4_body<ACT, EK, LN, RB, HF, 0>(g);
+}
+template <bool HF, int QF>
+__global__ __launch_bounds__(256) void gemm4_attn_kernel(const Gemm4Args g) {
+    gemm4_body<MAGE_ACT_NONE, EK_BIAS, LN_CONSUME, false, HF, QF>(g);
+}
+
+template <int ACT, int EK, int LN, bool RB, bool HF = false, int QF = 0>
+int launch4(const mage_gemm_desc* d, hipStream_t s, int n_cu, float* attn_p = nullptr, int attn_axis = 0, float attn_scale = 0.f) {
     Gemm4Args a;
+    a.attn_p = attn_p;
+    a.attn_axis = attn_axis;
+    a.attn_scale = attn_scale;
+    a.out_w = d->out_w;
+    a.y_img_stride = d->y_img_stride;
     a.A = d->A;
     a.W = d->W;
     a.Y = d->Y;
@@ -416,7 +584,9 @@
         a.stagger_groups = st_groups;
         a.stagger_sleeps = (int)(period * st_percent / 100 / st_groups / 1024);
     }
-    const int r = mage_gemm_launch<gemm4_kernel<ACT, EK, LN, RB, HF>>(grid, 256, G4_LDS, s, a);
+    int r;
+    if constexpr (QF != 0) r = mage_gemm_launch<gemm4_attn_kernel<HF, QF>>(grid, 256, G4_LDS, s, a);
+    else r = mage_gemm_launch<gemm4_kernel<ACT, EK, LN, RB, HF>>(grid, 256, G4_LDS, s, a);
     return r < 0 ? r : 1;
 }
 
@@ -672,6 +842,52 @@
     return launch4<MAGE_ACT_QUICKGELU, EK_BIAS, LN_NONE, false>(d, s, n_cu);
 }
 
+extern "C" int mage_gemm_attn_fused(const mage_gemm_desc* d, int32_t phase, int32_t axis, float scale, float* p, void* stream) {
+    MAGE_CHECK_ARG(d != nullptr, "mage_gemm_attn_fused: null descriptor");
+    MAGE_CHECK_ARG(phase == 1 || phase == 2, "mage_gemm_attn_fused: phase %d (1 = the Q K launch, 2 = the V launch)", (int)phase);
+    MAGE_CHECK_ARG(axis == 1 || axis == 2, "mage_gemm_attn_fused: axis %d (1 = H, 2 = W of 16 x 16 frames)", (int)axis);
+    MAGE_CHECK_ARG(d->dtype == MAGE_BF16 || d->dtype == MAGE_F16, "mage_gemm_attn_fused: bf16 or f16 operands");
+    MAGE_CHECK_ARG(d->A && d->W && p && d->bias && d->ln_stats && d->ln_colsum && (phase == 1 || d->Y),
+                   "mage_gemm_attn_fused: A, W, bias, ln_stats, ln_colsum, the P scratch%s must be given", phase == 2 ? " and Y" : "");
+    MAGE_CHECK_ARG(d->M > 0 && d->M % 256 == 0 && d->N % 256 == 0 && d->K % 128 == 0 && d->K >= 256 && d->K <= 1024,
+                   "mage_gemm_attn_fused: M=%d, N=%d multiples of 256 (whole 16 x 16 frames), K=%d a multiple of 128 in [256, 1024]", d->M, d->N, d->K);
+    MAGE_CHECK_ARG(d->taps_h * d->taps_w == 1 && d->stride == 1 && !d->dy0 && !d->dx0 && d->in_h == 1 && d->out_h == 1 && d->in_w == d->out_w && !d->a_half &&
+                       d->y_mul_x == 1 && (d->out_w >= d->M || (d->out_w % 256 == 0 && d->a_img_stride == d->out_w)) && d->a_off % 256 == 0 && d->a_off >= 0,
+                   "mage_gemm_attn_fused: plain rows in (a_off a multiple of 256), output rows regrouped whole frames at a time");
+    MAGE_CHECK_ARG(!d->scale && !d->shift && !d->rowadd && !d->residual && !d->post_relu && !d->res_half && !d->y2 && !d->ln_part && !d->head_w && !d->a_relu &&
+                       d->n_split <= 1 && d->act == MAGE_ACT_NONE,
+                   "mage_gemm_attn_fused: the LayerNorm-consuming bias epilogue only");
+    MAGE_CHECK_ARG(phase == 1 || (d->y_dtype == d->dtype && d->ldy % 8 == 0 && d->ldy >= d->N && (((uintptr_t)d->Y) & 15) == 0 && d->y_off >= 0),
+                   "mage_gemm_attn_fused: the V launch writes 16-bit rows of the operands' type, ldy a multiple of 8, Y 16-byte aligned");
+    const int ldw = d->ldw ? d->ldw : d->K;
+    MAGE_CHECK_ARG(ldw == d->K && d->lda % 8 == 0 && d->lda >= d->K, "mage_gemm_attn_fused: W packed [N][K], lda a multiple of 8");
+    MAGE_CHECK_ARG((((uintptr_t)d->A | (uintptr_t)d->W | (uintptr_t)d->bias | (uintptr_t)d->ln_colsum | (uintptr_t)p) & 15) == 0 && (((uintptr_t)d->ln_stats) & 7) == 0,
+                   "mage_gemm_attn_fused: operands must be 16-byte aligned");
+    MAGE_CHECK_ARG(((long)d->M + d->a_off) * d->lda * 2 + 16384 < (1L << 32) && (long)d->N * ldw * 2 + 16384 < (1L << 32),
+                   "mage_gemm_attn_fused: operands beyond the kernel's 32-bit lane offsets");
+    hipStream_t s = (hipStream_t)stream;
+    const int n_cu = mage_gemm_cu_count();
+    int r;
+    if (d->dtype == MAGE_F16)
+        r = phase == 1 ? launch4<MAGE_ACT_NONE, EK_BIAS, LN_CONSUME, false, true, 1>(d, s, n_cu, p, axis, scale)
+                       : launch4<MAGE_ACT_NONE, EK_BIAS, LN_CONSUME, false, true, 2>(d, s, n_cu, p, axis, scale);
+    else
+        r = phase == 1 ? launch4<MAGE_ACT_NONE, EK_BIAS, LN_CONSUME, false, false, 1>(d, s, n_cu, p, axis, scale)
+                       : launch4<MAGE_ACT_NONE, EK_BIAS, LN_CONSUME, false, false, 2>(d, s, n_cu, p, axis, scale);
+    return r < 0 ? r : MAGE_OK;
+}
+
+extern "C" int mage_gemm_attn_fused_kernel_name(const mage_gemm_desc* d, int32_t phase, int32_t axis, char* buf, int32_t len) {
+    MAGE_CHECK_ARG(buf != nullptr && len > 0, "mage_gemm_attn_fused_kernel_name: no buffer");
+    float dummy_p[4] __attribute__((aligned(16)));
+    const void* kernel = nullptr;
+    mage_gemm_plan = &kernel;
+    const int r = mage_gemm_attn_fused(d, phase, axis, 1.f, dummy_p, nullptr);
+    mage_gemm_plan = nullptr;
+    if (r != MAGE_OK) return r;
+    return mage_kernel_symbol_name(kernel, buf, len, "mage_gemm_attn_fused_kernel_name");
+}
+
 int mage_gemm_tn4_try(const void* dY, int64_t lda, const void* X, int64_t ldb, int64_t T, int32_t N, int32_t K, int32_t n_split, int64_t tps,
                       float* partials, float* db_partials, hipStream_t stream) {
     if (mage_options().gemm_no_4w) return 0;
diff --git a/mage_amd/csrc/norm_attn.hip b/mage_amd/csrc/norm_attn.hip
--- a/mage_amd/csrc/norm_attn.hip
+++ b/mage_amd/csrc/norm_attn.hip
@@ -2,6 +2,7 @@
 #include <type_traits>
 
 #include "common.h"
+#include "attn_mfma.h"
 
 namespace {
 
@@ -159,30 +160,6 @@
 #pragma unroll
         for (int c = 0; c < 4; ++c) store8(orow + c * 8, o[2 * c] * inv, o[2 * c + 1] * inv);
     }
-}
-
-typedef __attribute__((ext_vector_type(8))) __bf16 abf16x8;
-typedef __attribute__((ext_vector_type(4))) short ashort4;
-typedef __attribute__((ext_vector_type(4))) _Float16 ahalf4;
-template <typename HT> __device__ __forceinline__ void attn_p_split(float p, short& hi, short& lo) {
-    if constexpr (std::is_same<HT, f16_t>::value) {
-        const _Float16 h = (_Float16)p;
-        hi = __builtin_bit_cast(short, h);
-        lo = __builtin_bit_cast(short, (_Float16)(p - (float)h));
-    } else {
-        const unsigned hb = __float_as_uint(p) & 0xffff0000u;
-        hi = (short)(hb >> 16);
-        lo = (short)(__float_as_uint(p - __uint_as_float(hb)) >> 16);
-    }
-}
-template <typename HT> __device__ __forceinline__ f32x4 attn_mfma_pv(const ashort4& vt, const ashort4& p, const f32x4& o) {
-    if constexpr (std::is_same<HT, f16_t>::value)
-        return __builtin_amdgcn_mfma_f32_16x16x16f16(__builtin_bit_cast(ahalf4, vt), __builtin_bit_cast(ahalf4, p), o, 0, 0, 0);
-    else
-        return __builtin_amdgcn_mfma_f32_16x16x16bf16_1k(vt, p, o, 0, 0, 0);
-}
-template <typename HT> __device__ __forceinline__ f32x4 attn_mfma_qk(const uint4& k, const uint4& q) {
-    return mfma16x16x32<HT>(__builtin_bit_cast(u32x4, k), __builtin_bit_cast(u32x4, q), f32x4{0.f, 0.f, 0.f, 0.f});
 }
 
 template <int NKB, int MAXH, typename HT = unsigned short>
diff --git a/mage_amd/modules/mage_model.py b/mage_amd/modules/mage_model.py
--- a/mage_amd/modules/mage_model.py
+++ b/mage_amd/modules/mage_model.py
@@ -373,6 +373,7 @@
         self.compute_dtype = F32
         self.split_kind = 0
         self.stream_bf16 = True
+        self.qk_fuse_tiles = 4
         self._derived = _Derived(self)
 
     def initialize_parameters(self):
@@ -415,6 +416,8 @@
                 d[f"b{i}.{lin}.lnw"] = wq
                 d[f"b{i}.{lin}.lns"] = wq.float().sum(dim=1).contiguous()
                 d[f"b{i}.{lin}.lnc"] = ((w.double() * bt.double()[None, :]).sum(1) + d[f"b{i}.{lin}.b"].double()).float().contiguous()
+            if i % 3 and self.model_channels % 64 == 0:
+                self._qk_fuse_pack(d, f"b{i}", d[f"b{i}.in_proj.lnw"], d[f"b{i}.in_proj.lns"], "")
         return d
 
     def _fold(self, dt, B: int, hw: int) -> bool:
@@ -440,6 +443,31 @@
             wq = (d[f"{p}.{lin}.f32"] * d[f"{p}.{ln}.w"][None, :]).to(F16)
             d[kw_], d[ks_] = wq, wq.float().sum(dim=1).contiguous()
         return d[kw_], d[ks_]
+
+    def _qk_fuse(self, xb, M: int, hh: int, ww: int, stats_rows: bool, cache) -> bool:
+        Cc = self.model_channels
+        if not (stats_rows and cache is None and hh == 16 and ww == 16 and self.use_cids and config.get().qk_fuse):
+            return False
+        if Cc % 256 or not 256 <= Cc <= 1024 or M % 256 or (M + 8) * Cc * 2 >= 2 ** 32:
+            return False
+        return (M // 256) * (Cc // 256) >= getattr(self, "qk_fuse_tiles", 4) * torch.cuda.get_device_properties(xb.device).multi_processor_count
+
+    def _qk_fuse_w(self, d, p, dt):
+        sfx = ".f16" if dt == F16 else ""
+        if f"{p}.in_proj.qk.w{sfx}" not in d:
+            lnw, lns = self._ln_fold_w(d, p, "in_proj", dt)
+            self._qk_fuse_pack(d, p, lnw, lns, sfx)
+        q = f"{p}.in_proj."
+        return dict(wqk=d[q + "qk.w" + sfx], sqk=d[q + "qk.s" + sfx], cqk=d[q + "qk.c"],
+                    wv=d[q + "v.w" + sfx], sv=d[q + "v.s" + sfx], cv=d[q + "v.c"])
+
+    def _qk_fuse_pack(self, d, p, lnw, lns, sfx: str) -> None:
+        Cc = self.model_channels
+        idx = ops.qk_pack_rows(Cc, lnw.device)
+        lnc = d[f"{p}.in_proj.lnc"]
+        d[f"{p}.in_proj.qk.w{sfx}"], d[f"{p}.in_proj.qk.s{sfx}"] = lnw[idx].contiguous(), lns[idx].contiguous()
+        d[f"{p}.in_proj.v.w{sfx}"], d[f"{p}.in_proj.v.s{sfx}"] = lnw[2 * Cc:].contiguous(), lns[2 * Cc:].contiguous()
+        d[f"{p}.in_proj.qk.c"], d[f"{p}.in_proj.v.c"] = lnc[idx].contiguous(), lnc[2 * Cc:].contiguous()
 
     def _stats_inline(self, xb, M: int) -> bool:
         Cc = self.model_channels
@@ -541,12 +569,19 @@
         ao = torch.empty(M, Cc, device=dev, dtype=dt)
         hdn = torch.empty(M, 4 * Cc, device=dev, dtype=dt)
         geo = [self._axial_geo(a, B, hh, ww, P, p0, cached=cache is not None, q_cached=cache is not None) for a in range(3)]
+        fuse = self._qk_fuse(xb, M, hh, ww, fold and not inl, cache)
+        pscr = torch.empty(M, Cc // 32, 16, device=dev, dtype=F32) if fuse else None
         for i in range(self.layers):
             p = f"b{i}"
             ln1 = ln if i else ln0
             if ln1 is None:
                 ops.layernorm(x, d[p + ".ln_1.w"], d[p + ".ln_1.b"], xn, 1e-5)
-            if i % 3 == 0 and cache is not None:
+            if fuse and i % 3:
+                f = self._qk_fuse_w(d, p, dt)
+                kw = dict(axis=i % 3, M=M, K=Cc, lda=Cc, ln_stats=stats)
+                ops.gemm_attn_fused(xb, f["wqk"], None, pscr, phase=1, N=2 * Cc, bias=f["cqk"], ln_colsum=f["sqk"], **kw)
+                ops.gemm_attn_fused(xb, f["wv"], ao, pscr, phase=2, N=Cc, ldy=Cc, bias=f["cv"], ln_colsum=f["sv"], **kw)
+            elif i % 3 == 0 and cache is not None:
                 if p0 == 0:
                     cache[i] = torch.empty(B * L * hw, 3 * Cc, device=dev, dtype=dt)
                 kv = cache[i]
@@ -555,7 +590,8 @@
             else:
                 q = kv = qkv
                 self._ln_linear(d, p, "in_proj", xn, xb, ln1, qkv, M=M, N=3 * Cc)
-            ops.attention(q, kv[:, Cc:], kv[:, 2 * Cc:], ao, ldq=3 * Cc, ldk=3 * Cc, ldv=3 * Cc, ldo=Cc, **geo[i % 3])
+            if not (fuse and i % 3):
+                ops.attention(q, kv[:, Cc:], kv[:, 2 * Cc:], ao, ldq=3 * Cc, ldk=3 * Cc, ldv=3 * Cc, ldo=Cc, **geo[i % 3])
             _linear(ao, d, p + ".out_proj", x, dt, M=M, N=Cc, K=Cc, **res)
             if fold and not inl:
                 ops.ln_stats(part, Cc, 1e-5, stats)
diff --git a/mage_amd/ops.py b/mage_amd/ops.py
--- a/mage_amd/ops.py
+++ b/mage_amd/ops.py
@@ -265,6 +265,49 @@
     return y
 
 
+def qk_pack_rows(C_: int, device=None) -> torch.Tensor:
+    n = torch.arange(2 * C_, device=device)
+    head, part, j = n // 64, (n % 64) // 32, n % 32
+    dim = (j % 16 // 4) * 8 + (j // 16) * 4 + j % 4
+    return part * C_ + head * 32 + dim
+
+
+def gemm_attn_fused(a: torch.Tensor, w: torch.Tensor, y: Optional[torch.Tensor], p: torch.Tensor, *, phase: int, axis: int, M: int, N: int, K: int,
+                    lda: int, bias, ln_stats, ln_colsum, ldy: int = 0, scale: Optional[float] = None, a_off: int = 0, out_w: Optional[int] = None,
+                    y_img_stride: Optional[int] = None, y_off: int = 0):
+    l, s = _dev(a)
+    assert w.dtype == a.dtype and p.dtype == torch.float32 and p.is_contiguous() and p.numel() >= M * (N // (4 if phase == 1 else 2)), (w.dtype, p.shape)
+    out_w = M if out_w is None else out_w
+    d = GemmDesc()
+    d.dtype, d.M, d.N, d.K = code(a), M, N, K
+    d.A, d.W, d.Y = a.data_ptr(), w.data_ptr(), _p(y)
+    d.lda, d.ldy, d.y_dtype = lda, ldy, (code(y) if y is not None else code(a))
+    d.out_h, d.out_w, d.in_h, d.in_w = 1, out_w, 1, out_w
+    d.a_img_stride, d.a_off = out_w, a_off
+    d.taps_h, d.taps_w, d.cin, d.stride = 1, 1, K, 1
+    d.dys, d.dxs = 1, 1
+    d.y_img_stride = out_w if y_img_stride is None else y_img_stride
+    d.y_mul_y, d.y_mul_x, d.y_off = out_w, 1, y_off
+    d.bias, d.ln_stats, d.ln_colsum = _p(bias), _p(ln_stats), _p(ln_colsum)
+    d.n_split = 1
+    sc = float(32 ** -0.5 if scale is None else scale)
+    ev = None
+    if PROFILE.enabled:
+        buf = C.create_string_buffer(256)
+        _lib.check(l.mage_gemm_attn_fused_kernel_name(C.byref(d), phase, axis, buf, len(buf)), l)
+        key = buf.value.decode()
+        if PROFILE.wants(key):
+            ev = PROFILE.begin()
+    _lib.check(l.mage_gemm_attn_fused(C.byref(d), phase, axis, sc, p.data_ptr(), s), l)
+    if ev is not None:
+        es = a.element_size()
+        pb = float(M) * (N // (4 if phase == 1 else 2)) * 4
+        nb = float(M) * K * es + float(N) * K * es + pb + (float(M) * N * y.element_size() if phase == 2 else 0.0)
+        fl = 2.0 * M * N * K + (2.0 * M * 16 * (N // 2) if phase == 1 else 4.0 * M * 16 * N)
+        PROFILE.end(key, ev, fl, nb)
+    return p if phase == 1 else y
+
+
 def gemm_is_small(a: torch.Tensor, M: int, N: int, K: int) -> bool:
     l, _ = _dev(a)
     r = l.mage_gemm_is_small(M, N, K)
```

New measurement: 5917 (median of 6 runs). 1.02x the previous value.
